# blyssprivacy/sdk

Hardware: AMD Instinct MI355X
Metric: PIR queries/sec (full answer path) on 2^20 items x 256 B (higher is better)
Workload: dtype u64; 1 GPU; spiral-rs process_query, c2 = {"db_item_size": 256, "instances": 1, "n": 2, "nu_1": 9, "nu_2": 11, "p": 256, "q2_bits": 20, "t_conv": 4, "t_exp_left": 8, "t_exp_right": 56, "t_gsw": 8}, encoded DB 64.0 GiB (56.0 GiB resident per GPU), unsharded, one query per step

## Files before the change

include/spiral_hip.h:

```cpp
#ifndef SPIRAL_HIP_H
#define SPIRAL_HIP_H

#include <stddef.h>
#include <stdint.h>

#ifdef __cplusplus
extern "C" {
#endif

#define SP_OK 0
#define SP_E_ARG (-1)
#define SP_E_HIP (-2)
#define SP_E_OOM (-3)
#define SP_E_STATE (-4)
#define SP_E_NOTFOUND (-5)

#define SP_MAX_ROW_SHARDS 8

typedef struct sp_params sp_params_t;
typedef struct sp_pp sp_pp_t;
typedef struct sp_ppc sp_ppc_t;
typedef struct sp_db sp_db_t;
typedef struct sp_query sp_query_t;

const char* sp_last_error(void);
uint64_t sp_paths_taken(int reset);
const char* sp_path_name(int bit);
int sp_debug_set(const char* name, long value);
int sp_device_count(void);
int sp_set_device(int device);

sp_params_t* sp_params_from_json(const char* json);
void sp_params_free(sp_params_t*);
uint64_t sp_params_get(const sp_params_t*, const char* name);
int sp_params_ntt_table(const sp_params_t*, int crt, int which, uint64_t* out_n);

sp_db_t* sp_db_create(const sp_params_t*, int shard, int num_shards);
sp_db_t* sp_db_create_columns(const sp_params_t*, int shard, int num_shards);
sp_db_t* sp_db_create_sparse(const sp_params_t*);
sp_db_t* sp_db_create_sparse_shard(const sp_params_t*, int shard, int num_shards);
size_t sp_db_sparse_items(const sp_db_t*);
sp_db_t* sp_db_create_planar(const sp_params_t*);
sp_db_t* sp_db_create_planar_shard(const sp_params_t*, int shard, int num_shards);
const char* sp_db_format(const sp_db_t*);
void sp_db_free(sp_db_t*);
int sp_db_load_plane(sp_db_t*, int plane, int z0, int nz, const uint64_t* words);
int sp_db_load(sp_db_t*, const uint64_t* words, size_t n_words);
int sp_db_load_items(sp_db_t*, const uint8_t* file, size_t file_len);
int sp_db_update_item(sp_db_t*, size_t item_idx, const uint8_t* data, size_t len);
int sp_db_update_items(sp_db_t*, const size_t* item_idx, const uint8_t* const* data, const size_t* lens, size_t n);
int sp_db_update_rows(sp_db_t*, const uint8_t* body, size_t body_len, size_t* applied, size_t* largest_update);
int sp_db_fill_synthetic(sp_db_t*, uint64_t seed);
int sp_db_prepare_batch(sp_db_t*, int* built);
uint64_t sp_synth_word(uint64_t seed, uint64_t ref_index);
int sp_db_read_ref(const sp_db_t*, int plane, int z, int ii, int j0, int count, uint64_t* out);
int sp_db_read_items(const sp_db_t*, size_t item0, size_t count, uint8_t* out, size_t out_cap,
                     uint8_t* present , size_t* undecodable );
size_t sp_db_export_rows_bound(const sp_db_t*, size_t count);
int sp_db_export_rows(const sp_db_t*, size_t item0, size_t count, uint8_t* body, size_t body_cap,
                      size_t* body_len, size_t* records);
int sp_db_copy_items(sp_db_t* dst, const sp_db_t* src, size_t item0, size_t count, size_t* copied );
#define SP_DIGEST_RESIDENT 0
#define SP_DIGEST_BATCH_COPY 1
int sp_db_digest(const sp_db_t*, uint64_t seed, int which, int plane0, int nplanes, uint64_t* out );
int sp_db_digest_ref_words(const sp_params_t*, uint64_t seed, int plane, int z0, int nz, const uint64_t* words, uint64_t acc[2]);
int sp_db_item_digests(const sp_db_t*, uint64_t seed, int which, int plane0, int nplanes, size_t item0, size_t count,
                       uint64_t* out , uint8_t* present );
int sp_db_item_digests_ref_words(const sp_params_t*, uint64_t seed, int plane, int z0, int nz, const uint64_t* words,
                                 uint64_t* acc );
size_t sp_db_device_bytes(const sp_db_t*);
size_t sp_db_batch_copy_bytes(const sp_db_t*);

sp_pp_t* sp_pp_deserialize(const sp_params_t*, const uint8_t* data, size_t len);
void sp_pp_free(sp_pp_t*);
int sp_pp_export(const sp_pp_t*, uint64_t* out, size_t cap_words, size_t* n_words);
size_t sp_pp_device_bytes(const sp_pp_t*);

sp_ppc_t* sp_pp_compact(const sp_params_t*, const uint8_t* data, size_t len);
void sp_ppc_free(sp_ppc_t*);
size_t sp_ppc_device_bytes(const sp_ppc_t*);
sp_pp_t* sp_pp_expand(const sp_ppc_t*);
int sp_pp_expand_into(const sp_ppc_t*, sp_pp_t* slot);

int sp_process_query(const sp_params_t*, const sp_pp_t*, const uint8_t* query, size_t query_len,
                     const sp_db_t*, uint8_t* out, size_t out_cap, size_t* out_len);
int sp_process_query_batch(const sp_params_t*, const sp_pp_t* const* pps, const uint8_t* const* queries,
                           const size_t* query_lens, int batch, const sp_db_t*, uint8_t* out,
                           size_t out_stride, size_t* out_len);

int sp_query_sweep_scatter(sp_query_t*, const sp_db_t*, int G);
int sp_query_sweep_scatter_plane(sp_query_t*, const sp_db_t*, int G, int plane);
int sp_query_sweep_scatter_group(sp_query_t* const* qs, int batch, const sp_db_t* shard, int G);
int sp_query_fold_local(sp_query_t*, const void* reduced_chunk_dev, int G);
int sp_query_fold_local_plane(sp_query_t*, const void* reduced_plane_chunk_dev, int G, int plane);
int sp_query_fold_local_join(sp_query_t*);
void* sp_query_stream2(sp_query_t*);
void* sp_query_local_cts_ptr(sp_query_t*);
size_t sp_query_local_cts_words(const sp_query_t*);
int sp_query_finish_gathered(sp_query_t*, const void* gathered_dev, int G, uint8_t* out, size_t out_cap, size_t* out_len);
sp_query_t* sp_query_begin(const sp_params_t*, const sp_pp_t*, const uint8_t* query, size_t query_len);
sp_query_t* sp_query_begin_for_db(const sp_params_t*, const sp_pp_t*, const uint8_t* query, size_t query_len,
                                  const sp_db_t* db);
int sp_query_sweep(sp_query_t*, const sp_db_t*);
void* sp_query_partial_ptr(sp_query_t*);
size_t sp_query_partial_words(const sp_query_t*);
int sp_query_sync(sp_query_t*);
int sp_query_finish(sp_query_t*, uint8_t* out, size_t out_cap, size_t* out_len);
void sp_query_free(sp_query_t*);
void* sp_query_stream(sp_query_t*);
int sp_query_timings(const sp_query_t*, float* ms4);

typedef struct sp_comm sp_comm_t;
#define SP_COMM_ID_BYTES 128
int sp_comm_unique_id(uint8_t* id128);
sp_comm_t* sp_comm_create(int rank, int world, const uint8_t* id128);
typedef struct sp_comm_ops {
  int (*reduce_scatter_u32)(void* user, const void* send, void* recv, size_t recv_count, void* hip_stream);
  int (*all_gather_u64)(void* user, const void* send, void* recv, size_t send_count, void* hip_stream);
  void* user;
} sp_comm_ops_t;
sp_comm_t* sp_comm_create_custom(int rank, int world, const sp_comm_ops_t* ops);
void sp_comm_free(sp_comm_t*);
int sp_comm_rank(const sp_comm_t*);
int sp_comm_world(const sp_comm_t*);
void* sp_comm_stream(sp_comm_t*);
int sp_comm_barrier(sp_comm_t*);
int sp_process_query_sharded(sp_comm_t*, const sp_params_t*, const sp_pp_t*, const uint8_t* query, size_t query_len,
                             const sp_db_t* shard, uint8_t* out, size_t out_cap, size_t* out_len);
int sp_process_queries_sharded(sp_comm_t*, const sp_params_t*, const sp_pp_t* const* pps, const uint8_t* const* queries,
                               const size_t* query_lens, int n, const sp_db_t* shard, uint8_t* out, size_t out_stride,
                               size_t* out_len);
int sp_process_queries_sharded_batched(sp_comm_t*, const sp_params_t*, const sp_pp_t* const* pps, const uint8_t* const* queries,
                                       const size_t* query_lens, int n, const sp_db_t* shard, int group, uint8_t* out,
                                       size_t out_stride, size_t* out_len);
int sp_comm_reserve_batch(sp_comm_t*, const sp_params_t* params, int group);
int sp_comm_reserve_batch_for(sp_comm_t*, const sp_params_t* params, const sp_db_t* shard, int group);
int sp_comm_reserve(sp_comm_t*, const sp_params_t* params);
int sp_comm_timings(const sp_comm_t*, float* ms3);
int sp_comm_describe(const sp_comm_t*, char* buf, size_t cap);

typedef struct sp_server sp_server_t;
sp_server_t* sp_server_create(const sp_params_t* params, const sp_db_t* db);
void sp_server_free(sp_server_t*);
size_t sp_server_clients(const sp_server_t*);
int sp_server_setup(sp_server_t*, const uint8_t* pp_bytes, size_t len, char* uuid_out37);
int sp_server_setup_json(sp_server_t*, const char* body, size_t body_len, char* out, size_t out_cap, size_t* out_len);
int sp_server_forget(sp_server_t*, const char* uuid);
int sp_server_private_read(sp_server_t*, const uint8_t* const* requests, const size_t* request_lens, int n, uint8_t* out,
                           size_t out_stride, size_t* out_lens);
int sp_server_private_read_json(sp_server_t*, const char* body, size_t body_len, char* out, size_t out_cap, size_t* out_len);
size_t sp_server_private_read_json_bound(const sp_server_t*, int n_queries);
int sp_server_update_row(sp_server_t*, sp_db_t* db, const uint8_t* body, size_t body_len, char* out, size_t out_cap, size_t* out_len);
int sp_server_replace_db(sp_server_t*, const sp_db_t* new_db);
int sp_server_set_expanded_clients(sp_server_t*, size_t max_expanded);
int sp_server_client_stats(const sp_server_t*, uint64_t out[7]);

int sp_sweep_launches(const sp_params_t*, const sp_db_t*);
int sp_bench_sweep(sp_query_t* q, const sp_db_t* db, int iters, float* ms_per_launch);
int sp_bench_sweep_ex(sp_query_t* q, const sp_db_t* db, int iters, int per_plane_launches, float* ms_per_launch);
int sp_bench_sweep_batch(sp_query_t* const* qs, int batch, const sp_db_t* db, int iters, float* ms_per_pass);
int sp_bench_sweep_scatter_group(sp_query_t* const* qs, int batch, const sp_db_t* shard, int G, int layout, int iters,
                                 float* ms_per_pass);

int sp_debug_cu_probe(int bit_lo, int bit_hi, int blocks, uint32_t* out2);
int sp_debug_resident_check(const sp_params_t* params, const sp_pp_t* pp, uint64_t* out, int cap);
int sp_debug_chacha20_u64(const uint8_t seed[32], uint64_t* out, size_t count);
int sp_debug_chacha20_u64_device(const sp_params_t*, const uint8_t seed[32], size_t first_word, uint64_t* out, size_t count);

int sp_bench_ntt(const sp_params_t*, int M, int blocks, int reps, float* ns_per_ntt);


int sp_ntt_forward(const sp_params_t*, uint64_t* data, size_t count);
int sp_ntt_inverse(const sp_params_t*, uint64_t* data, size_t count);
int sp_to_ntt(const sp_params_t*, const uint64_t* raw, uint64_t* out, size_t count);
int sp_from_ntt(const sp_params_t*, const uint64_t* ntt, uint64_t* out, size_t count);
int sp_multiply(const sp_params_t*, const uint64_t* a, size_t ar, size_t ac, const uint64_t* b, size_t bc,
                uint64_t* res);
int sp_add(const sp_params_t*, const uint64_t* a, const uint64_t* b, size_t count, uint64_t* res);
int sp_add_into(const sp_params_t*, uint64_t* res, const uint64_t* a, size_t count);
int sp_scalar_multiply(const sp_params_t*, const uint64_t* scalar, const uint64_t* b, size_t count, uint64_t* res);
int sp_automorph(const sp_params_t*, const uint64_t* a, size_t count, size_t t, uint64_t* res);
int sp_gadget_invert_rdim(const sp_params_t*, const uint64_t* inp, size_t rows_in, size_t cols, uint64_t* out,
                          size_t rows_out, size_t rdim);
int sp_reorient_reg_ciphertexts(const sp_params_t*, const uint64_t* v_reg, uint64_t* out);
int sp_multiply_reg_by_database(const sp_params_t*, const uint64_t* db, const uint64_t* v_firstdim, size_t dim0,
                                size_t num_per, uint64_t* out);
int sp_coefficient_expansion(const sp_params_t*, const sp_pp_t*, uint64_t* v, size_t g, size_t stop_round,
                             size_t max_bits_to_gen_right);
int sp_regev_to_gsw(const sp_params_t*, const sp_pp_t*, const uint64_t* v_inp, uint64_t* v_gsw, size_t num_gsw);
int sp_get_v_folding_neg(const sp_params_t*, const uint64_t* v_folding, uint64_t* out);
int sp_expand_query(const sp_params_t*, const sp_pp_t*, const uint8_t* query, size_t query_len,
                    uint64_t* v_reg_reoriented, uint64_t* v_folding);
int sp_fold_ciphertexts(const sp_params_t*, uint64_t* cts, size_t num_per, const uint64_t* v_folding,
                        const uint64_t* v_folding_neg);
int sp_fold_ciphertexts_fused(const sp_params_t*, uint64_t* cts, size_t num_per, const uint64_t* v_folding,
                              long fused_min_pairs);
int sp_pack(const sp_params_t*, const sp_pp_t*, const uint64_t* v_ct, uint64_t* out);
int sp_encode(const sp_params_t*, const uint64_t* v_packed, uint8_t* out, size_t out_cap, size_t* out_len);

#ifdef __cplusplus
}
#endif
#endif
```

rust/src/hip.rs:

```rust
#![allow(non_camel_case_types, clippy::missing_safety_doc, clippy::too_many_arguments)]

use std::ffi::{CStr, CString};
use std::os::raw::{c_char, c_int, c_long, c_void};

pub mod sys {
    use super::*;

    pub const SP_OK: c_int = 0;
    pub const SP_E_ARG: c_int = -1;
    pub const SP_E_HIP: c_int = -2;
    pub const SP_E_OOM: c_int = -3;
    pub const SP_E_STATE: c_int = -4;
    pub const SP_E_NOTFOUND: c_int = -5;
    pub const SP_MAX_ROW_SHARDS: c_int = 8;
    pub const SP_COMM_ID_BYTES: usize = 128;

    #[repr(C)]
    pub struct sp_params_t {
        _p: [u8; 0],
    }
    #[repr(C)]
    pub struct sp_pp_t {
        _p: [u8; 0],
    }
// ... 7 lines not shown
    }
    #[repr(C)]
    pub struct sp_query_t {
        _p: [u8; 0],
    }
    #[repr(C)]
    pub struct sp_comm_t {
        _p: [u8; 0],
    }
    #[repr(C)]
    pub struct sp_server_t {
        _p: [u8; 0],
    }
    #[repr(C)]
    pub struct sp_comm_ops_t {
        pub reduce_scatter_u32: Option<
            unsafe extern "C" fn(user: *mut c_void, send: *const c_void, recv: *mut c_void, recv_count: usize, hip_stream: *mut c_void) -> c_int,
        >,
        pub all_gather_u64: Option<
            unsafe extern "C" fn(user: *mut c_void, send: *const c_void, recv: *mut c_void, send_count: usize, hip_stream: *mut c_void) -> c_int,
        >,
        pub user: *mut c_void,
    }

    extern "C" {
        pub fn sp_last_error() -> *const c_char;
        pub fn sp_paths_taken(reset: c_int) -> u64;
        pub fn sp_path_name(bit: c_int) -> *const c_char;
        pub fn sp_debug_set(name: *const c_char, value: c_long) -> c_int;
        pub fn sp_device_count() -> c_int;
        pub fn sp_set_device(device: c_int) -> c_int;
        pub fn sp_params_from_json(json: *const c_char) -> *mut sp_params_t;
        pub fn sp_params_free(p: *mut sp_params_t);
        pub fn sp_params_get(p: *const sp_params_t, name: *const c_char) -> u64;
        pub fn sp_params_ntt_table(p: *const sp_params_t, crt: c_int, which: c_int, out_n: *mut u64) -> c_int;
        pub fn sp_db_create(p: *const sp_params_t, shard: c_int, num_shards: c_int) -> *mut sp_db_t;
        pub fn sp_db_create_columns(p: *const sp_params_t, shard: c_int, num_shards: c_int) -> *mut sp_db_t;
        pub fn sp_db_create_sparse(p: *const sp_params_t) -> *mut sp_db_t;
        pub fn sp_db_create_sparse_shard(p: *const sp_params_t, shard: c_int, num_shards: c_int) -> *mut sp_db_t;
        pub fn sp_db_create_planar(p: *const sp_params_t) -> *mut sp_db_t;
        pub fn sp_db_create_planar_shard(p: *const sp_params_t, shard: c_int, num_shards: c_int) -> *mut sp_db_t;
        pub fn sp_db_format(db: *const sp_db_t) -> *const c_char;
        pub fn sp_db_sparse_items(db: *const sp_db_t) -> usize;
        pub fn sp_db_free(db: *mut sp_db_t);
        pub fn sp_db_load_plane(db: *mut sp_db_t, plane: c_int, z0: c_int, nz: c_int, words: *const u64) -> c_int;
        pub fn sp_db_load(db: *mut sp_db_t, words: *const u64, n_words: usize) -> c_int;
        pub fn sp_db_load_items(db: *mut sp_db_t, file: *const u8, file_len: usize) -> c_int;
        pub fn sp_db_update_item(db: *mut sp_db_t, item_idx: usize, data: *const u8, len: usize) -> c_int;
        pub fn sp_db_update_items(db: *mut sp_db_t, item_idx: *const usize, data: *const *const u8, lens: *const usize, n: usize) -> c_int;
        pub fn sp_db_update_rows(db: *mut sp_db_t, body: *const u8, body_len: usize, applied: *mut usize, largest_update: *mut usize) -> c_int;
        pub fn sp_db_fill_synthetic(db: *mut sp_db_t, seed: u64) -> c_int;
        pub fn sp_db_prepare_batch(db: *mut sp_db_t, built: *mut c_int) -> c_int;
        pub fn sp_db_batch_copy_bytes(db: *const sp_db_t) -> usize;
        pub fn sp_synth_word(seed: u64, ref_index: u64) -> u64;
        pub fn sp_db_read_ref(db: *const sp_db_t, plane: c_int, z: c_int, ii: c_int, j0: c_int, count: c_int, out: *mut u64) -> c_int;
        pub fn sp_db_read_items(db: *const sp_db_t, item0: usize, count: usize, out: *mut u8, out_cap: usize, present: *mut u8, undecodable: *mut usize) -> c_int;
        pub fn sp_db_export_rows_bound(db: *const sp_db_t, count: usize) -> usize;
        pub fn sp_db_export_rows(db: *const sp_db_t, item0: usize, count: usize, body: *mut u8, body_cap: usize, body_len: *mut usize, records: *mut usize) -> c_int;
        pub fn sp_db_copy_items(dst: *mut sp_db_t, src: *const sp_db_t, item0: usize, count: usize, copied: *mut usize) -> c_int;
        pub fn sp_db_digest(db: *const sp_db_t, seed: u64, which: c_int, plane0: c_int, nplanes: c_int, out: *mut u64) -> c_int;
        pub fn sp_db_digest_ref_words(p: *const sp_params_t, seed: u64, plane: c_int, z0: c_int, nz: c_int, words: *const u64, acc: *mut u64) -> c_int;
        pub fn sp_db_item_digests(db: *const sp_db_t, seed: u64, which: c_int, plane0: c_int, nplanes: c_int, item0: usize, count: usize, out: *mut u64, present: *mut u8) -> c_int;
        pub fn sp_db_item_digests_ref_words(p: *const sp_params_t, seed: u64, plane: c_int, z0: c_int, nz: c_int, words: *const u64, acc: *mut u64) -> c_int;
        pub fn sp_db_device_bytes(db: *const sp_db_t) -> usize;
        pub fn sp_pp_deserialize(p: *const sp_params_t, data: *const u8, len: usize) -> *mut sp_pp_t;
        pub fn sp_pp_free(pp: *mut sp_pp_t);
        pub fn sp_pp_export(pp: *const sp_pp_t, out: *mut u64, cap_words: usize, n_words: *mut usize) -> c_int;
        pub fn sp_pp_device_bytes(pp: *const sp_pp_t) -> usize;
        pub fn sp_pp_compact(p: *const sp_params_t, data: *const u8, len: usize) -> *mut sp_ppc_t;
        pub fn sp_ppc_free(c: *mut sp_ppc_t);
        pub fn sp_ppc_device_bytes(c: *const sp_ppc_t) -> usize;
        pub fn sp_pp_expand(c: *const sp_ppc_t) -> *mut sp_pp_t;
        pub fn sp_pp_expand_into(c: *const sp_ppc_t, slot: *mut sp_pp_t) -> c_int;
        pub fn sp_process_query(p: *const sp_params_t, pp: *const sp_pp_t, query: *const u8, query_len: usize, db: *const sp_db_t,
                                out: *mut u8, out_cap: usize, out_len: *mut usize) -> c_int;
        pub fn sp_process_query_batch(p: *const sp_params_t, pps: *const *const sp_pp_t, queries: *const *const u8,
                                      query_lens: *const usize, batch: c_int, db: *const sp_db_t, out: *mut u8,
                                      out_stride: usize, out_len: *mut usize) -> c_int;
        pub fn sp_query_sweep_scatter(q: *mut sp_query_t, db: *const sp_db_t, g: c_int) -> c_int;
        pub fn sp_query_sweep_scatter_plane(q: *mut sp_query_t, db: *const sp_db_t, g: c_int, plane: c_int) -> c_int;
        pub fn sp_query_sweep_scatter_group(qs: *const *mut sp_query_t, batch: c_int, shard: *const sp_db_t, g: c_int) -> c_int;
        pub fn sp_query_fold_local(q: *mut sp_query_t, reduced_chunk_dev: *const c_void, g: c_int) -> c_int;
        pub fn sp_query_fold_local_plane(q: *mut sp_query_t, reduced_plane_chunk_dev: *const c_void, g: c_int, plane: c_int) -> c_int;
        pub fn sp_query_fold_local_join(q: *mut sp_query_t) -> c_int;
        pub fn sp_query_stream2(q: *mut sp_query_t) -> *mut c_void;
        pub fn sp_query_local_cts_ptr(q: *mut sp_query_t) -> *mut c_void;
        pub fn sp_query_local_cts_words(q: *const sp_query_t) -> usize;
        pub fn sp_query_finish_gathered(q: *mut sp_query_t, gathered_dev: *const c_void, g: c_int, out: *mut u8, out_cap: usize,
                                        out_len: *mut usize) -> c_int;
        pub fn sp_query_begin(p: *const sp_params_t, pp: *const sp_pp_t, query: *const u8, query_len: usize) -> *mut sp_query_t;
        pub fn sp_query_begin_for_db(p: *const sp_params_t, pp: *const sp_pp_t, query: *const u8, query_len: usize,
                                     db: *const sp_db_t) -> *mut sp_query_t;
        pub fn sp_query_sweep(q: *mut sp_query_t, db: *const sp_db_t) -> c_int;
        pub fn sp_query_partial_ptr(q: *mut sp_query_t) -> *mut c_void;
        pub fn sp_query_partial_words(q: *const sp_query_t) -> usize;
        pub fn sp_query_sync(q: *mut sp_query_t) -> c_int;
        pub fn sp_query_finish(q: *mut sp_query_t, out: *mut u8, out_cap: usize, out_len: *mut usize) -> c_int;
        pub fn sp_query_free(q: *mut sp_query_t);
        pub fn sp_query_stream(q: *mut sp_query_t) -> *mut c_void;
        pub fn sp_query_timings(q: *const sp_query_t, ms4: *mut f32) -> c_int;
        pub fn sp_comm_unique_id(id128: *mut u8) -> c_int;
        pub fn sp_comm_create(rank: c_int, world: c_int, id128: *const u8) -> *mut sp_comm_t;
        pub fn sp_comm_create_custom(rank: c_int, world: c_int, ops: *const sp_comm_ops_t) -> *mut sp_comm_t;
        pub fn sp_comm_free(c: *mut sp_comm_t);
        pub fn sp_comm_rank(c: *const sp_comm_t) -> c_int;
        pub fn sp_comm_world(c: *const sp_comm_t) -> c_int;
        pub fn sp_comm_stream(c: *mut sp_comm_t) -> *mut c_void;
        pub fn sp_comm_barrier(c: *mut sp_comm_t) -> c_int;
        pub fn sp_process_query_sharded(c: *mut sp_comm_t, p: *const sp_params_t, pp: *const sp_pp_t, query: *const u8,
                                        query_len: usize, shard: *const sp_db_t, out: *mut u8, out_cap: usize,
                                        out_len: *mut usize) -> c_int;
        pub fn sp_process_queries_sharded(c: *mut sp_comm_t, p: *const sp_params_t, pps: *const *const sp_pp_t, queries: *const *const u8,
                                          query_lens: *const usize, n: c_int, shard: *const sp_db_t, out: *mut u8, out_stride: usize,
                                          out_len: *mut usize) -> c_int;
        pub fn sp_comm_reserve(c: *mut sp_comm_t, p: *const sp_params_t) -> c_int;
        pub fn sp_comm_reserve_batch(c: *mut sp_comm_t, p: *const sp_params_t, group: c_int) -> c_int;
        pub fn sp_comm_reserve_batch_for(c: *mut sp_comm_t, p: *const sp_params_t, shard: *const sp_db_t, group: c_int) -> c_int;
        pub fn sp_process_queries_sharded_batched(c: *mut sp_comm_t, p: *const sp_params_t, pps: *const *const sp_pp_t,
                                                  queries: *const *const u8, query_lens: *const usize, n: c_int,
                                                  shard: *const sp_db_t, group: c_int, out: *mut u8, out_stride: usize,
                                                  out_len: *mut usize) -> c_int;
        pub fn sp_comm_timings(c: *const sp_comm_t, ms3: *mut f32) -> c_int;
        pub fn sp_comm_describe(c: *const sp_comm_t, buf: *mut c_char, cap: usize) -> c_int;
        pub fn sp_server_create(params: *const sp_params_t, db: *const sp_db_t) -> *mut sp_server_t;
        pub fn sp_server_free(s: *mut sp_server_t);
        pub fn sp_server_clients(s: *const sp_server_t) -> usize;
        pub fn sp_server_setup(s: *mut sp_server_t, pp_bytes: *const u8, len: usize, uuid_out37: *mut c_char) -> c_int;
        pub fn sp_server_setup_json(s: *mut sp_server_t, body: *const c_char, body_len: usize, out: *mut c_char, out_cap: usize,
                                    out_len: *mut usize) -> c_int;
        pub fn sp_server_forget(s: *mut sp_server_t, uuid: *const c_char) -> c_int;
        pub fn sp_server_set_expanded_clients(s: *mut sp_server_t, max_expanded: usize) -> c_int;
        pub fn sp_server_client_stats(s: *const sp_server_t, out7: *mut u64) -> c_int;
        pub fn sp_server_private_read(s: *mut sp_server_t, requests: *const *const u8, request_lens: *const usize, n: c_int,
                                      out: *mut u8, out_stride: usize, out_lens: *mut usize) -> c_int;
        pub fn sp_server_private_read_json(s: *mut sp_server_t, body: *const c_char, body_len: usize, out: *mut c_char,
                                           out_cap: usize, out_len: *mut usize) -> c_int;
        pub fn sp_server_private_read_json_bound(s: *const sp_server_t, n_queries: c_int) -> usize;
        pub fn sp_server_update_row(s: *mut sp_server_t, db: *mut sp_db_t, body: *const u8, body_len: usize, out: *mut c_char,
                                    out_cap: usize, out_len: *mut usize) -> c_int;
        pub fn sp_server_replace_db(s: *mut sp_server_t, new_db: *const sp_db_t) -> c_int;
        pub fn sp_sweep_launches(p: *const sp_params_t, db: *const sp_db_t) -> c_int;
        pub fn sp_bench_sweep(q: *mut sp_query_t, db: *const sp_db_t, iters: c_int, ms_per_launch: *mut f32) -> c_int;
        pub fn sp_bench_sweep_ex(q: *mut sp_query_t, db: *const sp_db_t, iters: c_int, per_plane_launches: c_int,
                                 ms_per_launch: *mut f32) -> c_int;
        pub fn sp_bench_sweep_batch(qs: *const *mut sp_query_t, batch: c_int, db: *const sp_db_t, iters: c_int,
                                    ms_per_pass: *mut f32) -> c_int;
        pub fn sp_bench_sweep_scatter_group(qs: *const *mut sp_query_t, batch: c_int, shard: *const sp_db_t, g: c_int,
                                            layout: c_int, iters: c_int, ms_per_pass: *mut f32) -> c_int;
        pub fn sp_debug_cu_probe(bit_lo: c_int, bit_hi: c_int, blocks: c_int, out2: *mut u32) -> c_int;
        pub fn sp_debug_resident_check(params: *const sp_params_t, pp: *const sp_pp_t, out: *mut u64, cap: c_int) -> c_int;
        pub fn sp_debug_chacha20_u64(seed: *const u8, out: *mut u64, count: usize) -> c_int;
        pub fn sp_debug_chacha20_u64_device(p: *const sp_params_t, seed: *const u8, first_word: usize, out: *mut u64,
                                            count: usize) -> c_int;
        pub fn sp_bench_ntt(p: *const sp_params_t, m: c_int, blocks: c_int, reps: c_int, ns_per_ntt: *mut f32) -> c_int;
        pub fn sp_ntt_forward(p: *const sp_params_t, data: *mut u64, count: usize) -> c_int;
        pub fn sp_ntt_inverse(p: *const sp_params_t, data: *mut u64, count: usize) -> c_int;
        pub fn sp_to_ntt(p: *const sp_params_t, raw: *const u64, out: *mut u64, count: usize) -> c_int;
        pub fn sp_from_ntt(p: *const sp_params_t, ntt: *const u64, out: *mut u64, count: usize) -> c_int;
        pub fn sp_multiply(p: *const sp_params_t, a: *const u64, ar: usize, ac: usize, b: *const u64, bc: usize, res: *mut u64) -> c_int;
        pub fn sp_add(p: *const sp_params_t, a: *const u64, b: *const u64, count: usize, res: *mut u64) -> c_int;
        pub fn sp_add_into(p: *const sp_params_t, res: *mut u64, a: *const u64, count: usize) -> c_int;
        pub fn sp_scalar_multiply(p: *const sp_params_t, scalar: *const u64, b: *const u64, count: usize, res: *mut u64) -> c_int;
        pub fn sp_automorph(p: *const sp_params_t, a: *const u64, count: usize, t: usize, res: *mut u64) -> c_int;
        pub fn sp_gadget_invert_rdim(p: *const sp_params_t, inp: *const u64, rows_in: usize, cols: usize, out: *mut u64,
                                     rows_out: usize, rdim: usize) -> c_int;
        pub fn sp_reorient_reg_ciphertexts(p: *const sp_params_t, v_reg: *const u64, out: *mut u64) -> c_int;
        pub fn sp_multiply_reg_by_database(p: *const sp_params_t, db: *const u64, v_firstdim: *const u64, dim0: usize,
                                           num_per: usize, out: *mut u64) -> c_int;
        pub fn sp_coefficient_expansion(p: *const sp_params_t, pp: *const sp_pp_t, v: *mut u64, g: usize, stop_round: usize,
                                        max_bits_to_gen_right: usize) -> c_int;
        pub fn sp_regev_to_gsw(p: *const sp_params_t, pp: *const sp_pp_t, v_inp: *const u64, v_gsw: *mut u64, num_gsw: usize) -> c_int;
        pub fn sp_get_v_folding_neg(p: *const sp_params_t, v_folding: *const u64, out: *mut u64) -> c_int;
        pub fn sp_expand_query(p: *const sp_params_t, pp: *const sp_pp_t, query: *const u8, query_len: usize,
                               v_reg_reoriented: *mut u64, v_folding: *mut u64) -> c_int;
        pub fn sp_fold_ciphertexts(p: *const sp_params_t, cts: *mut u64, num_per: usize, v_folding: *const u64,
                                   v_folding_neg: *const u64) -> c_int;
        pub fn sp_fold_ciphertexts_fused(p: *const sp_params_t, cts: *mut u64, num_per: usize, v_folding: *const u64,
                                         fused_min_pairs: c_long) -> c_int;
        pub fn sp_pack(p: *const sp_params_t, pp: *const sp_pp_t, v_ct: *const u64, out: *mut u64) -> c_int;
        pub fn sp_encode(p: *const sp_params_t, v_packed: *const u64, out: *mut u8, out_cap: usize, out_len: *mut usize) -> c_int;
    }
}

#[derive(Debug, Clone)]
pub struct HipError {
    pub code: c_int,
    pub message: String,
}
impl std::fmt::Display for HipError {
    fn fmt(&self, f: &mut std::fmt::Formatter<'_>) -> std::fmt::Result {
        write!(f, "spiral_hip rc={}: {}", self.code, self.message)
    }
}
impl std::error::Error for HipError {}

fn last_error() -> String {
    unsafe { CStr::from_ptr(sys::sp_last_error()) }.to_string_lossy().into_owned()
}
fn check(rc: c_int) -> Result<(), HipError> {
    if rc == sys::SP_OK {
        Ok(())
    } else {
        Err(HipError { code: rc, message: last_error() })
    }
}
fn must<T>(r: Result<T, HipError>) -> T {
    r.unwrap_or_else(|e| panic!("{}", e))
}

const N: usize = 2048;
const CRT: usize = 2;

pub struct Params(*mut sys::sp_params_t);
pub struct PublicParameters(*mut sys::sp_pp_t);
pub struct CompactPublicParameters(*mut sys::sp_ppc_t);
unsafe impl Send for CompactPublicParameters {}
unsafe impl Sync for CompactPublicParameters {}
pub struct Database(*mut sys::sp_db_t);
pub struct Comm(*mut sys::sp_comm_t);
unsafe impl Send for Params {}
unsafe impl Sync for Params {}
unsafe impl Send for PublicParameters {}
unsafe impl Sync for PublicParameters {}
unsafe impl Send for Database {}
unsafe impl Sync for Database {}
unsafe impl Send for Comm {}

impl Params {
    pub fn try_from_json(cfg: &str) -> Result<Self, HipError> {
        let c = CString::new(cfg).map_err(|_| HipError { code: sys::SP_E_ARG, message: "NUL in JSON".into() })?;
        let p = unsafe { sys::sp_params_from_json(c.as_ptr()) };
        if p.is_null() {
            Err(HipError { code: sys::SP_E_ARG, message: last_error() })
        } else {
            Ok(Params(p))
        }
    }
    pub fn from_json(cfg: &str) -> Self {
        must(Self::try_from_json(cfg))
    }
    pub fn get(&self, name: &str) -> u64 {
        let c = CString::new(name).unwrap();
        let v = unsafe { sys::sp_params_get(self.0, c.as_ptr()) };
        assert!(v != u64::MAX, "unknown Params field {}", name);
        v
    }
    pub fn setup_bytes(&self) -> usize { self.get("setup_bytes") as usize }
    pub fn query_bytes(&self) -> usize { self.get("query_bytes") as usize }
    pub fn num_items(&self) -> usize { self.get("num_items") as usize }
    pub fn response_bytes(&self) -> usize { self.get("response_bytes") as usize }
    pub fn db_words(&self) -> usize { self.get("db_words") as usize }
    pub fn dim0(&self) -> usize { 1usize << self.get("db_dim_1") }
    pub fn num_per(&self) -> usize { 1usize << self.get("db_dim_2") }
    pub fn planes(&self) -> usize { (self.get("instances") * self.get("n") * self.get("n")) as usize }
    pub fn t_gsw(&self) -> usize { self.get("t_gsw") as usize }
    pub fn n(&self) -> usize { self.get("n") as usize }
    pub fn as_ptr(&self) -> *const sys::sp_params_t { self.0 }
}
impl Drop for Params {
    fn drop(&mut self) {
        unsafe { sys::sp_params_free(self.0) }
    }
}

impl PublicParameters {
    pub fn try_deserialize(params: &Params, data: &[u8]) -> Result<Self, HipError> {
        let h = unsafe { sys::sp_pp_deserialize(params.0, data.as_ptr(), data.len()) };
        if h.is_null() {
            Err(HipError { code: sys::SP_E_ARG, message: last_error() })
        } else {
            Ok(PublicParameters(h))
        }
    }
    pub fn deserialize(params: &Params, data: &[u8]) -> Self {
        must(Self::try_deserialize(params, data))
    }
}
impl Drop for PublicParameters {
    fn drop(&mut self) {
        unsafe { sys::sp_pp_free(self.0) }
    }
}
impl PublicParameters {
    pub fn device_bytes(&self) -> usize {
        unsafe { sys::sp_pp_device_bytes(self.0) }
    }
}

impl CompactPublicParameters {
    pub fn try_new(params: &Params, data: &[u8]) -> Result<Self, HipError> {
        let h = unsafe { sys::sp_pp_compact(params.0, data.as_ptr(), data.len()) };
        if h.is_null() {
            Err(HipError { code: sys::SP_E_ARG, message: last_error() })
        } else {
            Ok(CompactPublicParameters(h))
        }
    }
    pub fn device_bytes(&self) -> usize {
        unsafe { sys::sp_ppc_device_bytes(self.0) }
    }
    pub fn expand(&self) -> Result<PublicParameters, HipError> {
        let h = unsafe { sys::sp_pp_expand(self.0) };
        if h.is_null() {
            Err(HipError { code: sys::SP_E_ARG, message: last_error() })
        } else {
            Ok(PublicParameters(h))
// ... 348 lines not shown
```

sdk_amd/csrc/capi.cpp:

```cpp
#include <cstdlib>
#include <new>

#include "capi_internal.hpp"

using namespace spiral;

static thread_local std::string g_last_error;
static thread_local int g_last_rc = SP_OK;
static thread_local int g_shard_split_hint = 1;
int spiral::guarded_status(int rc, const char* what) {
  if (rc != SP_OK) g_last_error = what;
  g_last_rc = rc;
  return rc;
}
int spiral::null_handle_rc() { return g_last_rc != SP_OK ? g_last_rc : SP_E_ARG; }

void spiral::check_device(int dev) {
  int cur = 0;
  HIP_CHECK(hipGetDevice(&cur));
  if (cur != dev) throw ArgError("handle belongs to HIP device " + std::to_string(dev) + " but the current device is " + std::to_string(cur));
}

void spiral::download_ntt(Workspace& W, const u32* src, size_t words, uint64_t* host, DevBuf<u64>& tmp) {
  tmp.ensure(words);
// ... 1259 lines not shown
    need_shard_count(q->params->p, G, db);
    need_row_shard(db);
    need_begun_for(q, db);
    check_device(db->device);
    Workspace& W = *q->ws;
    if (db->sparse) {
      sweep_sparse_scatter(q, db, G, 0, (int)q->params->p.planes(), false);
    } else if (db->planar_resident) {
      sp_query_t* one[1] = {q};
      planar_shard_pass(one, 1, db, G, 0, (int)q->params->p.planes(), true);
    } else {
      ScatterLayout scatter(W, G);
      run_sweep(W, *db);
    }
    HIP_CHECK(hipEventRecord(W.ev[2], W.stream));
    q->state = 2;
  });
}

int sp_query_sweep_scatter_plane(sp_query_t* q, const sp_db_t* db, int G, int plane) {
  return guarded([&] {
    need(q && db, "null argument");
    refuse_planar_unsharded(db, "sp_query_sweep_scatter_plane");
    need(db->params == q->params, "db was created for different params");
    need_rows_of(q, db);
    const Params& p = q->params->p;
    need_shard_count(p, G, db);
    need_row_shard(db);
    need_begun_for(q, db);
    need(plane >= 0 && (size_t)plane < p.planes(), "plane out of range");
    need(q->state == 1 && q->next_plane == plane, "sp_query_sweep_scatter_plane: planes must be swept in order after begin");
    check_device(db->device);
    Workspace& W = *q->ws;
    W.ensure_sweep();
    if (db->sparse) {
      sweep_sparse_scatter(q, db, G, plane, 1, true);
    } else if (db->planar_resident) {
      sp_query_t* one[1] = {q};
      planar_shard_pass(one, 1, db, G, plane, 1, false);
    } else {
      ScatterLayout scatter(W, G);
      launch_plane_sweep(W, *db, (size_t)plane);
    }
    q->next_plane = plane + 1;
    if ((size_t)q->next_plane == p.planes()) {
      HIP_CHECK(hipEventRecord(W.ev[2], W.stream));
      q->state = 2;
    }
  });
}

int sp_query_sweep_scatter_group(sp_query_t* const* qs, int batch, const sp_db_t* db, int G) {
  return guarded([&] {
    scatter_group_check(qs, batch, db, G);
    for (int i = 0; i < batch; i++)
      need(qs[i]->state == 1 && qs[i]->next_plane == 0, "sp_query_sweep_scatter_group: every query must be in 'begun' state, no plane swept");
    const size_t planes = db->params->p.planes();
    SweepBatchDesc d{};
    if (db->sparse) {
      const int group_min = sparse_group_min();
      bool shared = batch >= 2 && group_min != 0 && batch >= group_min;
      for (int i = 1; i < batch; i++) shared = shared && qs[i]->sparse_index == qs[0]->sparse_index;
      for (int i = 0; i < batch; i++) qs[i]->ws->ensure_sweep();
      if (shared) {
        Workspace* Ws[SPARSE_GROUP_MAX];
        for (int i = 0; i < batch; i++) Ws[i] = qs[i]->ws.get();
        const sp_db::SparseIndex& idx = *qs[0]->sparse_index;
        Workspace& W0 = group_pass_stream(qs, batch);
        run_sweep_sparse_scatter_group(Ws, batch, *db, idx.col_ptr.p, idx.col_rows.p, idx.col_slots.p, G, W0.stream);
        for (int i = 0; i < batch; i++) {
          group_pass_done(qs, i);
          qs[i]->ws->zero_shortcuts = true;
        }
      } else {
        for (int i = 0; i < batch; i++) {
          sweep_sparse_scatter(qs[i], db, G, 0, (int)planes, true);
          HIP_CHECK(hipEventRecord(qs[i]->ws->ev[2], qs[i]->ws->stream));
        }
      }
    } else if (db->planar_resident) {
      planar_shard_pass(qs, batch, db, G, 0, (int)planes, false);
      for (int i = 0; i < batch; i++) group_pass_done(qs, i);
    } else if (scatter_group_desc(qs, batch, db, G, d)) {
      Workspace& W0 = group_pass_stream(qs, batch);
      sweep_batch_prepare(W0.D->T, d, W0.stream);
      launch_sweep_batch_scatter(W0.D->T, d, G, W0.stream);
      for (int i = 0; i < batch; i++) group_pass_done(qs, i);
    } else {
      for (int i = 0; i < batch; i++) {
        Workspace& W = *qs[i]->ws;
        ScatterLayout scatter(W, G);
        for (size_t pl = 0; pl < planes; pl++) launch_plane_sweep(W, *db, pl);
        HIP_CHECK(hipEventRecord(W.ev[2], W.stream));
      }
    }
    for (int i = 0; i < batch; i++) {
      qs[i]->next_plane = (int)planes;
      qs[i]->state = 2;
    }
  });
}

int sp_query_fold_local(sp_query_t* q, const void* reduced_chunk, int G) {
  return guarded([&] {
    need(q && reduced_chunk, "null argument");
    need(q->state == 2, "sp_query_fold_local: sweep has not run");
    need_shard_count(q->params->p, G);
    run_fold_local(*q->ws, (const u32*)reduced_chunk, G);
    q->state = 4;
  });
}
int sp_query_fold_local_plane(sp_query_t* q, const void* reduced_plane_chunk, int G, int plane) {
  return guarded([&] {
    need(q && reduced_plane_chunk, "null argument");
    const Params& p = q->params->p;
    need_shard_count(p, G);
    need(plane >= 0 && (size_t)plane < p.planes(), "plane out of range");
    need((q->state == 1 && plane < q->next_plane) || q->state == 2, "sp_query_fold_local_plane: plane has not been swept");
    need(plane == q->next_fold_plane, "sp_query_fold_local_plane: planes must be folded in order");
    run_fold_local_plane(*q->ws, (const u32*)reduced_plane_chunk, G, plane);
    q->next_fold_plane = plane + 1;
  });
}

int sp_query_fold_local_join(sp_query_t* q) {
  return guarded([&] {
    need(q, "null argument");
    need(q->state == 2 && (size_t)q->next_fold_plane == q->params->p.planes(),
         "sp_query_fold_local_join: every plane must have been swept and folded");
    run_fold_local_join(*q->ws);
    q->state = 4;
  });
}

void* sp_query_stream2(sp_query_t* q) { return q && q->ws ? (void*)q->ws->stream2 : nullptr; }

void* sp_query_local_cts_ptr(sp_query_t* q) { return q && q->ws ? (void*)q->ws->final_cts.p : nullptr; }
size_t sp_query_local_cts_words(const sp_query_t* q) { return q ? q->params->p.planes() * 2 * POLY_LEN : 0; }

int sp_query_finish_gathered(sp_query_t* q, const void* gathered, int G, uint8_t* out, size_t out_cap, size_t* out_len) {
  return guarded([&] {
    need(q && gathered && out && out_len, "null argument");
    need(q->state == 4, "sp_query_finish_gathered: local fold has not run");
    const Params& p = q->params->p;
    need(out_cap >= p.response_bytes(), "output buffer smaller than response_bytes");
    run_finish_gathered(*q->ws, *q->pp, (const u64*)gathered, G);
    collect_response(q, out, out_len);
    q->state = 3;
  });
}

void* sp_query_partial_ptr(sp_query_t* q) {
  if (!q || !q->ws) return nullptr;
  if (guarded([&] { q->ws->ensure_sweep(); }) != SP_OK) return nullptr;
  return (void*)q->ws->sweep_out.p;
}
size_t sp_query_partial_words(const sp_query_t* q) {
  if (!q) return 0;
  const Params& p = q->params->p;
  return p.planes() * 4 * POLY_LEN * p.num_per();
}
void* sp_query_stream(sp_query_t* q) { return q && q->ws ? (void*)q->ws->stream : nullptr; }

int sp_query_sync(sp_query_t* q) {
  return guarded([&] {
    need(q && q->ws, "null query");
    HIP_CHECK(hipStreamSynchronize(q->ws->stream));
    HIP_CHECK(hipStreamSynchronize(q->ws->stream2));
  });
}

int sp_query_finish(sp_query_t* q, uint8_t* out, size_t out_cap, size_t* out_len) {
  return guarded([&] { finish_impl(q, true, out, out_cap, out_len); });
}

int sp_query_timings(const sp_query_t* q, float* ms4) {
  if (!q || !ms4 || q->state != 3) {
    g_last_error = "timings are available after sp_query_finish";
    return SP_E_STATE;
  }
  memcpy(ms4, q->ms, sizeof(q->ms));
  return SP_OK;
}
void sp_query_free(sp_query_t* q) { delete q; }

int sp_process_query(const sp_params_t* h, const sp_pp_t* pp, const uint8_t* query, size_t query_len,
                     const sp_db_t* db, uint8_t* out, size_t out_cap, size_t* out_len) {
  if (db && (db->num_shards != 1 || db->col_G != 1)) {
    g_last_error = "sp_process_query needs an unsharded db; use sp_query_begin/sweep/finish for shards";
    return SP_E_ARG;
  }
  sp_query_t* q = sp_query_begin_for_db(h, pp, query, query_len, db);
  if (!q) return null_handle_rc();
  int rc = sp_query_sweep(q, db);
  if (rc == SP_OK) rc = guarded([&] { finish_impl(q, false, out, out_cap, out_len); });
  sp_query_free(q);
  return rc;
}

}

#include "capi_readback.hpp"
#include "capi_copy.hpp"
#include "capi_digest.hpp"
#include "capi_item_digest.hpp"
#include "capi_compact.hpp"

#ifndef SPIRAL_CAPI_SPLIT
#include "capi_batch.cpp"
#include "capi_stage.cpp"
#endif
```

sdk_amd/csrc/capi_internal.hpp:

```cpp
#pragma once
#include <cstring>
#include <memory>
#include <string>

#include "../../include/spiral_hip.h"
#include "pipeline.hpp"

struct sp_query {
  sp_params* params = nullptr;
  const sp_pp* pp = nullptr;
  std::unique_ptr<spiral::Workspace> ws;
  int state = 0;
  int next_plane = 0;
  int next_fold_plane = 0;
  int rows_j0 = 0, rows_nj = 0;
  const sp_db* for_sparse = nullptr;
  std::shared_ptr<const sp_db::SparseIndex> sparse_index;
  std::shared_ptr<const spiral::DevBuf<spiral::u64>> planar;
  float ms[4] = {0, 0, 0, 0};
  bool streams_idle = false;
  ~sp_query() {
    if (ws && params) {
      if (!streams_idle) {
        (void)hipStreamSynchronize(ws->stream);
        (void)hipStreamSynchronize(ws->stream2);
      }
      ws->pipelined = false;
      ws->have_sweep_span = false;
      ws->zero_shortcuts = false;
      ws->out_G = 1;
      params->release_ws(std::move(ws));
    }
  }
};

extern "C" void sp_set_last_error_(const char* msg);

namespace spiral {

int guarded_status(int rc, const char* what);
int null_handle_rc();

template <typename F>
int guarded(F&& f) {
  tunables_new_call();
  try {
    f();
    return guarded_status(SP_OK, nullptr);
  } catch (const ArgError& e) {
    return guarded_status(SP_E_ARG, e.what());
  } catch (const OomError& e) {
    return guarded_status(SP_E_OOM, e.what());
  } catch (const HipError& e) {
    return guarded_status(SP_E_HIP, e.what());
  } catch (const std::bad_alloc&) {
    return guarded_status(SP_E_OOM, "host allocation failed");
  } catch (const std::exception& e) {
    return guarded_status(SP_E_ARG, e.what());
  }
}
template <typename F>
auto guarded_handle(F&& make) -> decltype(make().release()) {
  decltype(make()) h;
  return guarded([&] { h = make(); }) == SP_OK ? h.release() : nullptr;
}

inline void need(bool c, const char* msg) {
  if (!c) throw ArgError(msg);
}
void check_device(int dev);

struct Scoped {
  sp_params* P;
  std::unique_ptr<Workspace> ws;
  explicit Scoped(const sp_params* p) : P(const_cast<sp_params*>(p)), ws(P->acquire_ws()) {}
  ~Scoped() {
    (void)hipStreamSynchronize(ws->stream);
    P->release_ws(std::move(ws));
  }
  Workspace& operator*() { return *ws; }
  Workspace* operator->() { return ws.get(); }
};
void download_ntt(Workspace& W, const u32* src, size_t words, uint64_t* host, DevBuf<u64>& tmp);

struct TimingEvents {
  hipEvent_t a = nullptr, b = nullptr;
  TimingEvents() {
    HIP_CHECK(hipEventCreate(&a));
    if (hipEventCreate(&b) != hipSuccess) {
      (void)hipEventDestroy(a);
      throw HipError("hipEventCreate failed");
    }
  }
  ~TimingEvents() {
    (void)hipEventDestroy(a);
    (void)hipEventDestroy(b);
  }
  TimingEvents(const TimingEvents&) = delete;
  TimingEvents& operator=(const TimingEvents&) = delete;
};
template <typename F>
float timed_reps(hipStream_t s, int iters, F&& once, float launches_per_rep = 1.0f) {
  struct Drain {
    hipStream_t s;
    ~Drain() { (void)hipStreamSynchronize(s); }
  } drain{s};
  TimingEvents ev;
  once();
  HIP_CHECK(hipEventRecord(ev.a, s));
  for (int i = 0; i < iters; i++) once();
  HIP_CHECK(hipEventRecord(ev.b, s));
  HIP_CHECK(hipStreamSynchronize(s));
  float t = 0;
  HIP_CHECK(hipEventElapsedTime(&t, ev.a, ev.b));
  return t / ((float)iters * launches_per_rep);
}

sp_query_t* query_open(const sp_params_t* h, const sp_pp_t* pp);
sp_query_t* query_open_sparse(const sp_params_t* h, const sp_pp_t* pp, const sp_db_t* db, std::shared_ptr<const sp_db::SparseIndex> snapshot);
void query_begin_opened(sp_query_t* q, const uint8_t* query, size_t query_len, const sp_db_t* db);
void finish_impl(sp_query_t* q, bool premod, uint8_t* out, size_t out_cap, size_t* out_len);

size_t group_ws_bytes(const Params& p, int np_local);

using PlanarPin = std::shared_ptr<const DevBuf<u64>>;
SweepBatchDesc group_pass(const sp_db& db, sp_query_t* const* qs, int B, bool use_planar, PlanarPin& pin);
void group_pass_launch(const sp_db& db, const DevTables& T, SweepBatchDesc& d, hipStream_t s);
void refuse_planar_resident(const sp_db_t* db, const char* what);
Workspace& group_pass_stream(sp_query_t* const* qs, int B);
void group_pass_done(sp_query_t* const* qs, int i);

void sparse_group_pass(const sp_db& db, sp_query_t* const* qs, int B, hipStream_t s);

void scatter_group_check(sp_query_t* const* qs, int batch, const sp_db_t* db, int G);
bool scatter_group_desc(sp_query_t* const* qs, int batch, const sp_db_t* db, int G, SweepBatchDesc& d);

}
```

sdk_amd/csrc/capi_stage.cpp:

```cpp
#include "capi_internal.hpp"

using namespace spiral;

namespace {

void upload_ntt(Workspace& W, const uint64_t* host, size_t words, DevBuf<u32>& dst, DevBuf<u64>& tmp) {
  tmp.ensure(words);
  dst.ensure(words);
  HIP_CHECK(hipMemcpyAsync(tmp.p, host, words * 8, hipMemcpyHostToDevice, W.stream));
  launch_u64_to_u32(dst.p, tmp.p, (long)words, W.stream);
}
void upload_raw(Workspace& W, const uint64_t* host, size_t words, DevBuf<u64>& dst) {
  dst.ensure(words);
  HIP_CHECK(hipMemcpyAsync(dst.p, host, words * 8, hipMemcpyHostToDevice, W.stream));
}
void download_raw(Workspace& W, const u64* src, size_t words, uint64_t* host) {
  HIP_CHECK(hipMemcpyAsync(host, src, words * 8, hipMemcpyDeviceToHost, W.stream));
  HIP_CHECK(hipStreamSynchronize(W.stream));
}

void ensure_stage_fold(Workspace& W, size_t num_per, size_t further) {
  const size_t two_t = 2 * W.P->t_gsw;
  W.ensure_expand();
  W.foldX.ensure(num_per * 2 * POLY_LEN);
  W.foldY.ensure(std::max<size_t>(num_per / 2, 1) * 2 * POLY_LEN);
  W.fold_dig.ensure(num_per * two_t * 2 * POLY_LEN);
  W.fold_ntt.ensure(std::max<size_t>(num_per / 2, 1) * 2 * 2 * POLY_LEN);
  W.fold_mats.ensure(further * 2 * 2 * two_t * 2 * POLY_LEN);
}

enum MatsCopy { TO_MATS, FROM_MATS };
void copy_mats_half(Workspace& W, MatsCopy dir, int half, size_t levels, u32* dense) {
  const size_t row = 2 * W.P->t_gsw * 2 * POLY_LEN;
  for (size_t k = 0; k < levels * 2; k++) {
    u32 *m = W.fold_mats.p + (k * 2 + half) * row, *d = dense + k * row;
    HIP_CHECK(hipMemcpyAsync(dir == TO_MATS ? m : d, dir == TO_MATS ? d : m, row * sizeof(u32), hipMemcpyDeviceToDevice, W.stream));
  }
}
size_t mats_half_words(const Params& p, size_t levels) { return levels * 2 * 2 * p.t_gsw * 2 * POLY_LEN; }

template <typename F>
void stage_fold(const sp_params_t* h, uint64_t* cts, size_t num_per, const uint64_t* v_folding, F&& prepare) {
  need(num_per >= 1 && (num_per & (num_per - 1)) == 0, "num_per must be a power of two");
  size_t further = 0;
  while (((size_t)1 << further) < num_per) further++;
  if (further == 0) return;
  Scoped W(h);
  ensure_stage_fold(*W, num_per, further);
  DevBuf<u64> tmp, tmp2;
  DevBuf<u32> dF, left;
  upload_ntt(*W, v_folding, mats_half_words(h->p, further), dF, tmp);
  copy_mats_half(*W, TO_MATS, 1, further, dF.p);
  const FoldOpts o = prepare(*W, further, left, tmp2);
  HIP_CHECK(hipMemcpyAsync(W->foldX.p, cts, num_per * 2 * POLY_LEN * 8, hipMemcpyHostToDevice, W->stream));
  u64* res = run_fold(*W, o, W->foldX.p, W->foldY.p, 1, (int)num_per, -1);
  download_raw(*W, res, 2 * POLY_LEN, cts);
}

}

extern "C" {

int sp_bench_sweep(sp_query_t* q, const sp_db_t* db, int iters, float* ms_per_launch) {
  return sp_bench_sweep_ex(q, db, iters, -1, ms_per_launch);
}

int sp_bench_sweep_ex(sp_query_t* q, const sp_db_t* db, int iters, int per_plane_launches, float* ms_per_launch) {
  return guarded([&] {
    need(q && db && ms_per_launch && iters > 0, "bad argument");
    refuse_planar_resident(db, "sp_bench_sweep");
    need(q->state >= 1, "query not begun");
    check_device(db->device);
    Workspace& W = *q->ws;
    const Params& p = q->params->p;
    const bool per_plane = per_plane_launches < 0 ? sweep_is_pipelined(p, *db) : per_plane_launches != 0;
    need(!per_plane || db->col_G == 1, "per-plane launches need a row-sharded or unsharded db");
    auto sweep_once = [&] {
      if (!per_plane) return run_sweep(W, *db);
      W.ensure_sweep();
      for (size_t pl = 0; pl < p.planes(); pl++) launch_plane_sweep(W, *db, pl);
    };
    *ms_per_launch = timed_reps(W.stream, iters, sweep_once, per_plane ? (float)p.planes() : 1.0f);
  });
}

int sp_bench_sweep_batch(sp_query_t* const* qs, int batch, const sp_db_t* db, int iters, float* ms_per_pass) {
  return guarded([&] {
    if (qs && db && db->sparse) {
      need(ms_per_pass && iters > 0 && batch >= 1 && batch <= SPARSE_GROUP_MAX, "bad argument");
      check_device(db->device);
      for (int i = 0; i < batch; i++) {
        need(qs[i] && qs[i]->state >= 1, "query not begun");
        need(qs[i]->params == db->params, "query and db were created for different params");
        qs[i]->ws->ensure_sweep();
        HIP_CHECK(hipStreamSynchronize(qs[i]->ws->stream));
        HIP_CHECK(hipStreamSynchronize(qs[i]->ws->stream2));
      }
      hipStream_t s = qs[0]->ws->stream;
      *ms_per_pass = timed_reps(s, iters, [&] { sparse_group_pass(*db, qs, batch, s); });
      return;
    }
    const int group_max = !db ? 0 : db->planar_resident ? planar_resident_group_max(db->nj) : sweep_batch_group_max(db->np_local, db->nj);
    need(qs && db && ms_per_pass && iters > 0 && batch >= 1 && batch <= group_max, "bad argument");
    const bool narrow = !db->packed && db->num_shards == 1 && db->col_G == 1 && batch >= 2 && sweep_narrow_batch_shape_ok(db->np_local, db->nj);
    need(narrow || (db->planar_resident && db->num_shards == 1) || (db->packed && db->num_shards == 1 && db->col_G == 1),
         "the batched pass needs an unsharded PACKED database");
    check_device(db->device);
    for (int i = 0; i < batch; i++) {
      need(qs[i] && qs[i]->state >= 1, "query not begun");
      need(qs[i]->params == db->params, "query and db were created for different params");
    }
    Workspace& W0 = *qs[0]->ws;
    for (int i = 0; i < batch; i++) {
      qs[i]->ws->ensure_sweep();
      HIP_CHECK(hipStreamSynchronize(qs[i]->ws->stream));
      HIP_CHECK(hipStreamSynchronize(qs[i]->ws->stream2));
    }
    PlanarPin pin;
    SweepBatchDesc d = group_pass(*db, qs, batch, true, pin);
    *ms_per_pass = timed_reps(W0.stream, iters, [&] { group_pass_launch(*db, W0.D->T, d, W0.stream); });
  });
}

int sp_bench_sweep_scatter_group(sp_query_t* const* qs, int batch, const sp_db_t* db, int G, int layout, int iters, float* ms_per_pass) {
  return guarded([&] {
    need(ms_per_pass && iters > 0 && (layout == 0 || layout == 1), "bad argument");
    scatter_group_check(qs, batch, db, G);
    for (int i = 0; i < batch; i++) {
      need(qs[i]->state >= 1, "query not begun");
      HIP_CHECK(hipStreamSynchronize(qs[i]->ws->stream));
      HIP_CHECK(hipStreamSynchronize(qs[i]->ws->stream2));
    }
    if (db->sparse) {
      Workspace* Ws[SPARSE_GROUP_MAX];
      for (int i = 0; i < batch; i++) {
        need(qs[i]->sparse_index == qs[0]->sparse_index, "the queries of a sparse bucket's group must have been begun on one snapshot of its index");
        qs[i]->ws->ensure_sweep();
        Ws[i] = qs[i]->ws.get();
      }
      const sp_db::SparseIndex& idx = *qs[0]->sparse_index;
      Workspace& W0 = *qs[0]->ws;
      const int planes = (int)db->params->p.planes();
      *ms_per_pass = timed_reps(W0.stream, iters, [&] {
        if (batch == 1 && layout == 1)
          run_sweep_sparse_scatter(W0, *db, idx.col_ptr.p, idx.col_rows.p, idx.col_slots.p, G, 0, planes, true);
        else if (batch == 1)
          run_sweep_sparse(W0, *db, idx.col_ptr.p, idx.col_rows.p, idx.col_slots.p);
        else if (layout == 1)
          run_sweep_sparse_scatter_group(Ws, batch, *db, idx.col_ptr.p, idx.col_rows.p, idx.col_slots.p, G, W0.stream);
        else
          run_sweep_sparse_group(Ws, batch, *db, idx.col_ptr.p, idx.col_rows.p, idx.col_slots.p, W0.stream);
      });
      return;
    }
    if (db->planar_resident) {
      need(layout == 1, "a planar row shard has the scatter-form pass only (layout 1)");
      for (int i = 0; i < batch; i++) qs[i]->ws->ensure_sweep();
      PlanarPin none;
      SweepBatchDesc pd = group_pass(*db, qs, batch, false, none);
      Workspace& Wp = *qs[0]->ws;
      const int planes = (int)db->params->p.planes();
      *ms_per_pass = timed_reps(Wp.stream, iters, [&] {
        sweep_planar_resident_prepare(Wp.D->T, pd, Wp.stream);
        launch_sweep_planar_scatter(Wp.D->T, pd, G, 0, planes, false, Wp.stream);
      });
      return;
    }
    SweepBatchDesc d{};
    need(scatter_group_desc(qs, batch, db, G, d), "this group / shard does not take the scatter-form pass (sp_query_sweep_scatter_group would sweep per query)");
    Workspace& W0 = *qs[0]->ws;
    *ms_per_pass = timed_reps(W0.stream, iters, [&] {
      sweep_batch_prepare(W0.D->T, d, W0.stream);
      if (layout == 1)
        launch_sweep_batch_scatter(W0.D->T, d, G, W0.stream);
      else
        launch_sweep_batch(W0.D->T, d, W0.stream);
    });
  });
}

int sp_sweep_launches(const sp_params_t* h, const sp_db_t* db) {
  if (!h || !db) return 0;
  return sweep_is_pipelined(h->p, *db) ? (int)h->p.planes() : 1;
}

int sp_debug_cu_probe(int bit_lo, int bit_hi, int blocks, uint32_t* out2) {
  return guarded([&] {
    need(out2 && blocks > 0 && blocks <= 65536, "bad argument");
    hipStream_t s = nullptr;
    if (bit_hi > bit_lo) {
      hipDeviceProp_t prop;
      int dev = 0;
      HIP_CHECK(hipGetDevice(&dev));
      HIP_CHECK(hipGetDeviceProperties(&prop, dev));
      std::vector<uint32_t> m((prop.multiProcessorCount + 31) / 32, 0u);
      for (int k = bit_lo; k < bit_hi && k < prop.multiProcessorCount; k++) m[k / 32] |= 1u << (k % 32);
      HIP_CHECK(hipExtStreamCreateWithCUMask(&s, (uint32_t)m.size(), m.data()));
    } else {
      HIP_CHECK(hipStreamCreateWithFlags(&s, hipStreamNonBlocking));
    }
    DevBuf<u32> d((size_t)blocks * 2);
    launch_cu_probe(d.p, blocks, s);
    HIP_CHECK(hipMemcpyAsync(out2, d.p, (size_t)blocks * 8, hipMemcpyDeviceToHost, s));
    HIP_CHECK(hipStreamSynchronize(s));
    (void)hipStreamDestroy(s);
  });
}

int sp_debug_chacha20_u64(const uint8_t seed[32], uint64_t* out, size_t count) {
  if (!seed || (!out && count)) {
    sp_set_last_error_("null argument");
    return SP_E_ARG;
  }
  chacha20_keystream_u64(seed, out, count);
  return SP_OK;
}

int sp_debug_resident_check(const sp_params_t* h, const sp_pp_t* pp, uint64_t* out, int cap) {
  return guarded([&] {
    need(h && pp && out && cap >= 24, "bad argument");
    DeviceState& D = const_cast<sp_params*>(h)->device_state();
    struct Item { const u32* p; size_t n; const u32* host; };
    const Item items[6] = {{D.tw.p, D.tw.n, h->p.ntt_tables.data()}, {D.neg1.p, D.neg1.n, nullptr},
                           {D.gadget_gsw.p, D.gadget_gsw.n, nullptr}, {(const u32*)D.lists.p, D.lists.n, nullptr},
                           {pp->all.p, pp->all.n, nullptr}, {pp->pack_cat.p, pp->pack_cat.n, nullptr}};
    hipStream_t s = nullptr;
    HIP_CHECK(hipStreamCreateWithFlags(&s, hipStreamNonBlocking));
    DevBuf<unsigned long long> acc(12);
    DevBuf<u32> sink(1);
    auto host_sum = [](const u32* p, size_t n) {
      unsigned long long a = 0;
      for (size_t i = 0; i < n; i++) a += (unsigned long long)p[i] * (unsigned long long)((i << 1) | 1);
      return a;
    };
    HIP_CHECK(hipMemsetAsync(acc.p, 0, 12 * 8, s));
    for (int i = 0; i < 6; i++) launch_checksum(items[i].p, items[i].n, acc.p + i, s);
    launch_cache_sync(sink.p, s);
    for (int i = 0; i < 6; i++) launch_checksum(items[i].p, items[i].n, acc.p + 6 + i, s);
    unsigned long long k[12];
    HIP_CHECK(hipMemcpyAsync(k, acc.p, sizeof(k), hipMemcpyDeviceToHost, s));
    HIP_CHECK(hipStreamSynchronize(s));
    for (int i = 0; i < 6; i++) {
      std::vector<u32> hostcopy(items[i].n);
      if (items[i].n) HIP_CHECK(hipMemcpy(hostcopy.data(), items[i].p, items[i].n * 4, hipMemcpyDeviceToHost));
      out[4 * i + 0] = k[i];
      out[4 * i + 1] = host_sum(hostcopy.data(), items[i].n);
      out[4 * i + 2] = k[6 + i];
      out[4 * i + 3] = items[i].host ? host_sum(items[i].host, items[i].n) : 0;
    }
    (void)hipStreamDestroy(s);
  });
}

int sp_bench_ntt(const sp_params_t* h, int M, int blocks, int reps, float* ns_per_ntt) {
  return guarded([&] {
    need(h && ns_per_ntt && blocks > 0 && reps > 0, "bad argument");
    Scoped W(h);
    DevBuf<u32> scratch((size_t)blocks * 256);
    const float ms = bench_ntt_core(W->D->T, M, blocks, reps, scratch.p, W->stream);
    *ns_per_ntt = ms * 1e6f / ((float)blocks * reps * (M == 1 || M == 2 ? M : 4));
  });
}

int sp_to_ntt(const sp_params_t* h, const uint64_t* raw, uint64_t* out, size_t count) {
  return guarded([&] {
    need(h && raw && out, "null argument");
    if (count == 0) return;
    Scoped W(h);
    DevBuf<u64> d_raw, tmp;
    DevBuf<u32> d_ntt(count * 2 * POLY_LEN);
    upload_raw(*W, raw, count * POLY_LEN, d_raw);
    FwdDesc f{d_raw.p, nullptr, d_ntt.p, (int)count, 1, 1, 1, 64, 1, 0, 1};
    launch_ntt_fwd(W->D->T, f, W->stream);
    download_ntt(*W, d_ntt.p, count * 2 * POLY_LEN, out, tmp);
  });
}

int sp_from_ntt(const sp_params_t* h, const uint64_t* ntt, uint64_t* out, size_t count) {
  return guarded([&] {
    need(h && ntt && out, "null argument");
    if (count == 0) return;
    Scoped W(h);
    DevBuf<u64> tmp, d_raw(count * POLY_LEN);
    DevBuf<u32> d_ntt;
    upload_ntt(*W, ntt, count * 2 * POLY_LEN, d_ntt, tmp);
    InvDesc inv{};
    inv.src = d_ntt.p;
    inv.poly_stride = 2 * POLY_LEN;
    inv.crt_stride = POLY_LEN;
    inv.z_stride = 1;
    inv.dst = d_raw.p;
    inv.n_polys = (int)count;
    launch_ntt_inv(W->D->T, inv, W->stream);
    download_raw(*W, d_raw.p, count * POLY_LEN, out);
  });
}

int sp_ntt_forward(const sp_params_t* h, uint64_t* data, size_t count) {
  return guarded([&] {
    need(h && data, "null argument");
    if (count == 0) return;
    std::vector<u64> full(count * 2 * 2 * POLY_LEN);
    int rc = sp_to_ntt(h, data, full.data(), count * 2);
    if (rc != SP_OK) throw HipError(sp_last_error());
    for (size_t i = 0; i < count; i++)
      for (size_t c = 0; c < 2; c++)
        memcpy(data + (i * 2 + c) * POLY_LEN, full.data() + ((i * 2 + c) * 2 + c) * POLY_LEN, POLY_LEN * 8);
  });
}

int sp_ntt_inverse(const sp_params_t* h, uint64_t* data, size_t count) {
  return guarded([&] {
    need(h && data, "null argument");
    if (count == 0) return;
    std::vector<u64> raw(count * POLY_LEN);
    int rc = sp_from_ntt(h, data, raw.data(), count);
    if (rc != SP_OK) throw HipError(sp_last_error());
    for (size_t i = 0; i < count; i++)
      for (size_t z = 0; z < POLY_LEN; z++) {
        data[(i * 2 + 0) * POLY_LEN + z] = raw[i * POLY_LEN + z] % h->p.moduli[0];
        data[(i * 2 + 1) * POLY_LEN + z] = raw[i * POLY_LEN + z] % h->p.moduli[1];
      }
  });
}

int sp_multiply(const sp_params_t* h, const uint64_t* a, size_t ar, size_t ac, const uint64_t* b, size_t bc,
                uint64_t* res) {
  return guarded([&] {
    need(h && a && b && res && ar && ac && bc, "bad argument");
    Scoped W(h);
    DevBuf<u64> tmp;
    DevBuf<u32> dA, dBt, dR(ar * bc * 2 * POLY_LEN);
    upload_ntt(*W, a, ar * ac * 2 * POLY_LEN, dA, tmp);
    std::vector<u64> bt(ac * bc * 2 * POLY_LEN);
    for (size_t k = 0; k < ac; k++)
      for (size_t j = 0; j < bc; j++)
        memcpy(bt.data() + (j * ac + k) * 2 * POLY_LEN, b + (k * bc + j) * 2 * POLY_LEN, 2 * POLY_LEN * 8);
    DevBuf<u64> tmp2;
    upload_ntt(*W, bt.data(), bt.size(), dBt, tmp2);
    MacDesc m{};
    m.A = dA.p;
    m.B = dBt.p;
    m.out = dR.p;
    m.R = (int)ar;
    m.K = (int)ac;
    m.batch_inner = (int)bc;
    m.batch_outer = 1;
    m.B_inner_stride = (long)ac;
    m.split_k = (int)ac;
    m.out_batch_stride = 1;
    m.out_row_stride = (int)bc;
    launch_mac(W->D->T, m, W->stream);
    download_ntt(*W, dR.p, ar * bc * 2 * POLY_LEN, res, tmp);
  });
}

int sp_add(const sp_params_t* h, const uint64_t* a, const uint64_t* b, size_t count, uint64_t* res) {
  return guarded([&] {
    need(h && a && b && res && count, "bad argument");
    Scoped W(h);
    DevBuf<u64> tmp, tmp2;
    DevBuf<u32> dA, dB, dR(count * 2 * POLY_LEN);
    upload_ntt(*W, a, count * 2 * POLY_LEN, dA, tmp);
    upload_ntt(*W, b, count * 2 * POLY_LEN, dB, tmp2);
    launch_add(W->D->T, dR.p, dA.p, dB.p, (int)count, W->stream);
    download_ntt(*W, dR.p, count * 2 * POLY_LEN, res, tmp);
  });
}
// ... 223 lines not shown
```

sdk_amd/csrc/db.hip:

```cpp
#include "device_common.hpp"

namespace spiral {

__global__ __launch_bounds__(256) void k_db_relayout(u64* dst_plane, const u64* src, int z0, int num_per, int dim0,
                                                     int j0, int nj, ColMap cm) {
  __shared__ u64 tile[32][33];
  const int zl = blockIdx.z;
  const int tx = threadIdx.x & 31, ty = threadIdx.x >> 5;
  const int jt = blockIdx.x * 32, it = blockIdx.y * 32;
  const u64* s = src + (size_t)zl * cm.np_global * dim0;
  u64* dpl = dst_plane + (size_t)(z0 + zl) * nj * num_per;
#pragma unroll
  for (int i = 0; i < 4; i++) {
    int ii = it + ty + 8 * i, j = jt + tx;
    if (ii < num_per && j < nj) tile[ty + 8 * i][tx] = canon_word(s[(size_t)(cm.off + cm.stride * ii) * dim0 + j0 + j]);
  }
  __syncthreads();
#pragma unroll
  for (int i = 0; i < 4; i++) {
    int j = jt + ty + 8 * i, ii = it + tx;
    if (ii < num_per && j < nj) dpl[(size_t)j * num_per + ii] = tile[tx][ty + 8 * i];
  }
}
__global__ __launch_bounds__(256) void k_db_relayout_packed(u32* dst, int plane, const u64* src, int z0, int nz,
// ... 184 lines not shown
  for (int k = 0; k < 8; k++) {
    const int z = 8 * tau + k;
    if (d.packed) {
      const int chunks = d.num_per >> 7, npairs = d.nj >> 1;
      u32* unit = reinterpret_cast<u32*>(d.db) +
                  packed_unit_offset((size_t)plane * N + z, jp, ii0 >> 7, npairs, chunks);
      pack_unit_lane(unit, (ii0 & 127) >> 1, w[0][k], w[1][k], w[2][k], w[3][k]);
    } else {
#pragma unroll
      for (int ab = 0; ab < 4; ab++) {
        const int jl = jl0 + (ab >> 1), ii = ii0 + (ab & 1);
        if (jl < d.nj && ii < d.num_per) d.db[(((size_t)plane * N + z) * d.nj + jl) * d.num_per + ii] = w[ab][k];
      }
    }
  }
}
void launch_db_encode(const DevTables& T, const DbEncodeDesc& d, hipStream_t s) {
  if (d.njp <= 0) return;
  const unsigned gx = d.only_item >= 0 ? 1u : (unsigned)((d.num_per + 1) / 2);
  hipLaunchKernelGGL(k_db_encode, dim3(gx * (unsigned)d.njp, 1, d.planes), dim3(256), 0, s, T, d);
  launched(0, "k_db_encode");
}

__device__ __forceinline__ u32 quad_item_coeff(const DbEncodeDesc& d, const uint8_t* bytes, int len, int chunk_idx, int z) {
  const int pos = chunk_idx * d.bytes_per_chunk;
  if (pos >= d.db_item_size) return 0u;
  const int avail = d.db_item_size - pos;
  const int bytes_read = avail < d.bytes_per_chunk ? avail : d.bytes_per_chunk;
  const int words_read = (bytes_read * 8 + d.logp - 1) / d.logp;
  if (z >= words_read) return 0u;
  const int bit = z * d.logp;
  const int b0 = bit >> 3, sh = bit & 7;
  u64 acc = 0;
  const int nb = (sh + d.logp + 7) >> 3;
  for (int i = 0; i < nb; i++) {
    const int bi = b0 + i;
    const u64 byte = (bi < bytes_read && pos + bi < len) ? (u64)bytes[pos + bi] : 0ULL;
    acc |= byte << (8 * i);
  }
  return (u32)((acc >> sh) & ((1ULL << d.logp) - 1ULL));
}
__global__ __launch_bounds__(256) void k_db_encode_quads(DevTables T, DbEncodeDesc d, const DbQuadRec* quads) {
  __shared__ u32 lds0[LDS_WORDS];
  __shared__ u32 lds1[LDS_WORDS];
  const int tau = threadIdx.x;
  const int plane = (int)(blockIdx.x % (unsigned)d.planes);
  const DbQuadRec* qr = quads + blockIdx.x / (unsigned)d.planes;
  const int jp = qr->jp, qd = qr->q;
  const int chunks = d.num_per >> 7, npairs = d.nj >> 1;
  u64 w[4][8];
#pragma unroll
  for (int t = 0; t < 4; t++)
#pragma unroll
    for (int k = 0; k < 8; k++) w[t][k] = 0;
  u32* la = lds0;
  u32* lb = lds1;
#pragma unroll 1
  for (int ab = 0; ab < 4; ab++) {
    const int a = ab >> 1, b = ab & 1;
    const int jl = 2 * jp + a, ii = 2 * qd + b;
    const bool valid = jl < d.nj && ii < d.num_per;
    const long long src = qr->src[ab];
    u64 cur[8];
    if (src < 0 || !valid) {
#pragma unroll
      for (int k = 0; k < 8; k++) {
        cur[k] = 0;
        if (valid && d.packed) {
          const u32* unit = reinterpret_cast<const u32*>(d.db) + packed_unit_offset((size_t)plane * N + 8 * tau + k, jp, ii >> 7, npairs, chunks);
          cur[k] = unpack_word(unit, (ii & 127) >> 1, ab);
        }
      }
    } else {
      const uint8_t* bytes = d.win + src;
      const int len = qr->len[ab];
      u32 lo[8];
#pragma unroll 1
      for (int c = 0; c < 2; c++) {
        const ModConst m = T.c.mod[c];
        u32 v[8];
#pragma unroll
        for (int k = 0; k < 8; k++) {
          const u32 x = quad_item_coeff(d, bytes, len, plane, tau + 256 * k);
          v[k] = x > d.pt_modulus / 2 ? m.q - (d.pt_modulus - x) : x;
        }
        const u32* fw = T.tw + (size_t)c * 4 * N;
        ntt_fwd_block(v, tau, la, lb, fw, fw + N, m.q, m.two_q);
        {
          u32* tmp = la;
          la = lb;
          lb = tmp;
        }
#pragma unroll
        for (int k = 0; k < 8; k++) {
          if (c == 0)
            lo[k] = v[k];
          else
            cur[k] = (u64)lo[k] | ((u64)v[k] << 32);
        }
      }
    }
#pragma unroll
    for (int t = 0; t < 4; t++)
#pragma unroll
      for (int k = 0; k < 8; k++) w[t][k] = t == ab ? cur[k] : w[t][k];
  }
  const int jl0 = 2 * jp, ii0 = 2 * qd;
#pragma unroll
  for (int k = 0; k < 8; k++) {
    const int z = 8 * tau + k;
    if (d.packed) {
      u32* unit = reinterpret_cast<u32*>(d.db) + packed_unit_offset((size_t)plane * N + z, jp, ii0 >> 7, npairs, chunks);
      pack_unit_lane(unit, (ii0 & 127) >> 1, w[0][k], w[1][k], w[2][k], w[3][k]);
    } else {
#pragma unroll
      for (int ab = 0; ab < 4; ab++) {
        const int jl = jl0 + (ab >> 1), ii = ii0 + (ab & 1);
        if (qr->src[ab] >= 0 && jl < d.nj && ii < d.num_per) d.db[(((size_t)plane * N + z) * d.nj + jl) * d.num_per + ii] = w[ab][k];
      }
    }
  }
}
void launch_db_encode_quads(const DevTables& T, const DbEncodeDesc& d, const DbQuadRec* quads, size_t n_quads, hipStream_t s) {
  if (n_quads == 0) return;
  hipLaunchKernelGGL(k_db_encode_quads, dim3((unsigned)(n_quads * (size_t)d.planes)), dim3(256), 0, s, T, d, quads);
  launched(0, "k_db_encode_quads");
}

__global__ __launch_bounds__(256) void k_canon_words(u64* w, size_t total) {
  const size_t i = (size_t)blockIdx.x * 256 + threadIdx.x;
  if (i < total) w[i] = canon_word(w[i]);
}
void launch_canon_words(u64* w, size_t total, hipStream_t s) {
  if (total == 0) return;
  hipLaunchKernelGGL(k_canon_words, dim3((unsigned)((total + 255) / 256)), dim3(256), 0, s, w, total);
  launched(0, "k_canon_words");
}

__global__ __launch_bounds__(256) void k_sweep_out_to_ref(u64* out, const u32* in, int num_per) {
  size_t i = (size_t)blockIdx.x * 256 + threadIdx.x;
  size_t total = (size_t)4 * N * num_per;
  if (i >= total) return;
  size_t z = i & (N - 1);
  size_t rc = (i >> POLY_LEN_LOG2) & 3;
  size_t ii = i >> (POLY_LEN_LOG2 + 2);
  out[i] = (u64)in[(rc * N + z) * num_per + ii];
}
void launch_sweep_out_to_ref(u64* out, const u32* in, int num_per, hipStream_t s) {
  size_t total = (size_t)4 * N * num_per;
  hipLaunchKernelGGL(k_sweep_out_to_ref, dim3((unsigned)((total + 255) / 256)), dim3(256), 0, s, out, in, num_per);
  launched(0, "k_sweep_out_to_ref");
}

}

#include "item_readback.hpp"
#include "db_digest.hpp"
#include "db_item_digest.hpp"
#include "db_copy.hpp"
```

sdk_amd/csrc/kernels.hpp:

```cpp
#pragma once
#include <hip/hip_runtime.h>

#include <vector>

#include "params.hpp"

namespace spiral {

constexpr int N = (int)POLY_LEN;

struct DevTables {
  const u32* tw;
  DevConsts c;
};
__host__ __device__ inline const u32* inv_tables(const u32* tw, int c) { return tw + (size_t)8 * N + (size_t)c * 2 * N; }
__host__ __device__ inline const u32* wave_fwd_image(const u32* tw, int c) { return tw + (size_t)12 * N + (size_t)c * 2 * N; }
__host__ __device__ inline int wtw_phys(int idx) {
  if (idx >= 1024) {
    const int L = (idx - 1024) >> 4, r = (idx - 1024) & 15;
    return 1024 + 16 * L + 4 * (((r >> 2) + (L >> 2)) & 3) + (r & 3);
  }
  if (idx >= 512) {
    const int L = (idx - 512) >> 3, r = (idx - 512) & 7;
    return 512 + 8 * L + 4 * (((r >> 2) + (L >> 3)) & 1) + (r & 3);
  }
  return idx;
}

enum PathBit : u64 {
  PATH_SWEEP_PERSIST = 1ull << 0,
  PATH_SWEEP_PACKED = 1ull << 1,
  PATH_SWEEP_WIDE = 1ull << 2,
  PATH_SWEEP_NARROW = 1ull << 3,
  PATH_SWEEP_BATCH = 1ull << 4,
  PATH_FROM_SWEEP4 = 1ull << 5,
  PATH_FROM_SWEEP1 = 1ull << 6,
  PATH_FOLD_FUSED = 1ull << 7,
  PATH_FOLD_TAIL = 1ull << 8,
  PATH_FOLD_TAIL_LITERAL = 1ull << 9,
  PATH_PIPELINED = 1ull << 10,
  PATH_EXPAND_PRUNED = 1ull << 11,
  PATH_PACK_V1 = 1ull << 12,
  PATH_DIRECT_UPLOAD = 1ull << 13,
  PATH_SCATTER_OUT = 1ull << 14,
  PATH_SWEEP_XCD_FROM = 1ull << 15,
  PATH_FOLD_TAIL_PERSIST = 1ull << 16,
  PATH_EXPAND_FUSED = 1ull << 17,
  PATH_SWEEP_SPARSE = 1ull << 18,
  PATH_RCCL = 1ull << 19,
  PATH_FOLD_WAVE = 1ull << 20,
  PATH_CU_SPLIT = 1ull << 21,
  PATH_EXPAND_SPLIT = 1ull << 22,
  PATH_PIPE_CLASS_SPLIT = 1ull << 23,
  PATH_SWEEP_MFMA = 1ull << 24,
  PATH_CUSTOM_TRANSPORT = 1ull << 25,
  PATH_FROM_SWEEP_WAVE = 1ull << 26,
  PATH_FOLD_TAIL_BATCHED = 1ull << 27,
  PATH_SWEEP_RING = 1ull << 28,
  PATH_SWEEP_MFMA2 = 1ull << 29,
  PATH_FOLD_WAVE8 = 1ull << 30,
  PATH_SWEEP_PLANAR = 1ull << 31,
  PATH_EXPAND_GROUP = 1ull << 32,
  PATH_EXPAND_WAVE = 1ull << 33,
  PATH_SWEEP_BATCH_SCATTER = 1ull << 34,
  PATH_SWEEP_SPARSE_GROUP = 1ull << 35,
  PATH_SWEEP_NARROW_GROUP = 1ull << 36
};
long tunable(const char* name, long dflt);
void launched(u64 path_bits, const char* kernel);
void note_path(u64 path_bits);
void launch_checksum(const u32* p, size_t n_words, unsigned long long* out, hipStream_t s);
void launch_cache_sync(u32* sink, hipStream_t s);
void launch_copy_words(u32* dst, const u32* src, size_t n_words, hipStream_t s);
void debug_stage(int stage);

struct FwdDesc {
  const u64* src;
  const int* src_idx;
  u32* dst;
  int n_out;
  int rdim, cols, t, bits;
  int src_batch_stride;
  int src_row0, src_cols;
  long delta_off;
  int delta_inner, delta_outer_stride;
};
void launch_ntt_fwd(const DevTables& T, const FwdDesc& d, hipStream_t s);
void launch_ntt_fwd3(const DevTables& T, const FwdDesc& d0, const FwdDesc& d1, const FwdDesc& d2, hipStream_t s);

float bench_ntt_core(const DevTables& T, int M, int blocks, int reps, u32* scratch, hipStream_t s);

struct InvDesc {
  const u32* src;
  const int* idx;
  int polys_per_idx;
  long idx_stride, poly_stride, crt_stride, z_stride;
  u64* dst;
  int n_polys;
  int premod;
  int sweep_np;
  int automorph_t;
  const u32* scal;
  u32* scal_dst;
  int scal_thresh;
  const int* scal_only_idx;
  int n_scalar_only;
  const u64* addend;
  int add_inner2, add_outer_stride;
};
void launch_ntt_inv(const DevTables& T, const InvDesc& d, hipStream_t s);
void launch_from_sweep4(const DevTables& T, const u32* src, int np, int n_planes, int premod, u64* dst, hipStream_t s);

struct MacDesc {
  const u32* A;
  const u32* B;
  u32* out;
  const u32* addend;
  const int* out_idx;
  int R, K;
  int A_row_stride;
  int batch_inner, batch_outer;
  long B_inner_stride, B_outer_stride;
  int split_k;
  long split_off;
  int out_batch_stride, out_row_stride;
  const u32* extra;
  const int* extra_idx;
  int extra_row;
};
void launch_mac(const DevTables& T, const MacDesc& d, hipStream_t s);
void launch_mac2(const DevTables& T, const MacDesc& d0, const MacDesc& d1, hipStream_t s);

struct ExpandSideDesc {
  const u64* raw;
  const int* pos;
  const int* out_idx;
  const u32* A;
  u32* v;
  int cnt, t, bits;
};
void launch_expand_round(const DevTables& T, const ExpandSideDesc& left, const ExpandSideDesc& right, hipStream_t s);
constexpr long EXPAND_ROUND_MIN_DEFAULT = 2048;

constexpr int GROUP_MAX = 16;
struct GroupOff {
  long long v[GROUP_MAX], raw[GROUP_MAX], dig[GROUP_MAX], ct1[GROUP_MAX], pp[GROUP_MAX];
};
void launch_ntt_inv_group(const DevTables& T, const InvDesc& d, const GroupOff& g, int B, hipStream_t s);
void launch_ntt_fwd3_group(const DevTables& T, const FwdDesc& d0, const FwdDesc& d1, const FwdDesc& d2, const GroupOff& g, int B,
                           hipStream_t s);
void launch_mac2_group(const DevTables& T, const MacDesc& d0, const MacDesc& d1, const GroupOff& g, int B, hipStream_t s);
void launch_expand_round_group(const DevTables& T, const ExpandSideDesc& left, const ExpandSideDesc& right, const GroupOff& g, int B,
                               hipStream_t s);
void launch_reorient_group(u64* out, const u32* v, int first, int step, int dim0, const GroupOff& g, int B, hipStream_t s);
void launch_copy_polys_group(u32* dst, const int* dst_idx, int dst_row_stride, const u32* src, const int* src_idx, int src_row_stride,
                             int R, int batch, const GroupOff& g, int B, hipStream_t s);
void launch_folding_neg_group(const DevTables& T, u32* mats, const u32* gadget_ntt, int nu2, int two_t, const GroupOff& g, int B,
                              hipStream_t s);
void launch_mats_to_wave_group(u32* dst, const u32* src, size_t n_words, int half_polys, const GroupOff& g, int B, hipStream_t s);
struct ExpandWaveDesc {
  const u64* raw;
  const int* pos;
  const int* out_idx;
  const u32* A_w;
  const u32* const_w;
  u32* v;
  int cnt, t, bits;
};
void launch_expand_wave(const DevTables& T, const ExpandWaveDesc& d, const GroupOff& g, int B, hipStream_t s);
constexpr long EXPAND_WAVE_MIN_DIGITS_DEFAULT = 16;
constexpr long EXPAND_GROUP_ROUND_MIN_DEFAULT = 4096;

struct FoldDesc {
  const u64* X;
  u64* Y;
  const u32* mats;
  int cur, half, planes;
  int t, bits;
  int t_live;
  int zero_shortcuts;
  const u32* mats_w;
};
void launch_mats_to_wave(u32* dst, const u32* src, size_t n_words, hipStream_t s, int half_polys = 0);
constexpr long FOLD_VARIANT_DEFAULT = 5;
void launch_fold_fused(const DevTables& T, const FoldDesc& d, hipStream_t s);

void launch_add_poly_into(const DevTables& T, u32* dst, const int* idx, const u32* src, int batch, hipStream_t s);
void launch_scalar_mul(const DevTables& T, u32* base, long dst_off, long src_off, const u32* scalar, int n_polys,
                       hipStream_t s);
void launch_add_polys_idx(const DevTables& T, u32* dst, const int* di, const u32* a, const int* ai, const u32* b,
                          const int* bi, int count, hipStream_t s);
void launch_interleave_query(u64* qv, const u32* row0_ntt, const u64* wire, int dim0, hipStream_t s);
void launch_copy_polys(u32* dst, const int* dst_idx, int dst_row_stride, const u32* src, const int* src_idx,
                       int src_row_stride, int R, int batch, hipStream_t s);
void launch_folding_neg(const DevTables& T, u32* mats, const u32* gadget_ntt, int nu2, int two_t, hipStream_t s);
void launch_add(const DevTables& T, u32* out, const u32* a, const u32* b, int n_polys, hipStream_t s);
void launch_invert_raw(const DevTables& T, u64* out, const u64* a, long n_words, hipStream_t s);
void launch_automorph(const DevTables& T, u64* out, const u64* a, int n_polys, int t, hipStream_t s);
void launch_gadget_raw(u64* out, const u64* inp, int rows_in, int cols, int rows_out, int rdim, int bits,
                       hipStream_t s);
void launch_u64_to_u32(u32* out, const u64* in, long n, hipStream_t s);
void launch_u32_to_u64(u64* out, const u32* in, long n, hipStream_t s);

void launch_cu_probe(u32* out, int blocks, hipStream_t s);

struct EncodeDesc {
  const u64* packed;
  unsigned long long* out;
  int instances, n;
  u64 Q, q1, q2;
  int q1_bits, q2_bits;
};
void launch_encode(const EncodeDesc& d, hipStream_t s);

void launch_reorient(u64* out, const u32* v, int first, int step, int dim0, hipStream_t s);

struct CopyPolysDesc {
  u32* dst;
  const int* dst_idx;
  int dst_row_stride;
  const u32* src;
  const int* src_idx;
  int src_row_stride, R, batch;
};
struct FoldingNegDesc {
  u32* mats;
  const u32* gadget_ntt;
  int two_t, nu2;
};
struct ReorientDesc {
  u64* out;
  const u32* v;
  int first, step, dim0;
};
struct MatsToWaveDesc {
  u32* dst;
  const u32* src;
  size_t n_words;
  int half_polys;
};
struct AddPolyIntoDesc {
  u32* dst;
  const int* idx;
  const u32* src;
  int batch;
};
struct CopyWordsDesc {
  u32* dst;
  const u32* src;
  size_t n_words;
};
constexpr u64 PP_RAW_WIRE = 1ull << 63;
struct PpRawDesc {
  u64* dst;
  const u64* wire;
  const u64* table;
  u64 n_words;
  u64 modulus, modulus_inv;
};
void launch_pp_raw_image(const PpRawDesc& d, int n_polys, hipStream_t s);

struct SweepDesc {
  const u64* db;
  const u64* qv;
  u32* out;
  int planes, num_per, dim0, j0, nj;
  int packed;
  int out_G;
  int nt_store;
};
struct ColMap {
  int off = 0, stride = 1, np_global = 0;
};
inline bool db_can_pack(int num_per, int nj) { return num_per >= 128 && (nj % 2) == 0; }
inline size_t db_bytes(int planes, int num_per, int nj, bool packed) {
  return (size_t)planes * N * nj * num_per * (packed ? 7 : 8);
}
void launch_sweep(const DevTables& T, const SweepDesc& d, hipStream_t s);
void launch_sweep_persist(const DevTables& T, const SweepDesc& d, int wgs_per_cu, hipStream_t s, int n_cus = 256);
constexpr int SWEEP_BATCH_MAX = 8;
constexpr int SWEEP_GROUP_MAX = 16;
struct SweepBatchDesc {
  const u64* db;
  const u64* qv[SWEEP_GROUP_MAX];
  u32* out[SWEEP_GROUP_MAX];
  int batch;
  int planes, num_per, dim0, j0, nj;
  u32* rq;
  int use_mfma;
  const unsigned char* planar;
  int narrow;
  int fold_every;
};
bool sweep_narrow_batch_shape_ok(int num_per, int nj);
constexpr long NARROW_BATCH_MIN_DEFAULT = 0;
void launch_sweep_narrow_batch(const DevTables& T, const SweepBatchDesc& d, hipStream_t s);
bool sweep_planar_shape_ok(int num_per, int nj);
size_t sweep_planar_bytes(int planes, int num_per, int nj);
void launch_packed_to_planar(unsigned char* planar, const u64* packed, int planes, int num_per, int nj, hipStream_t s);
void launch_planar_patch_item(unsigned char* planar, const u64* packed, int planes, int num_per, int nj, int j, int ii, hipStream_t s);
constexpr size_t UPSERT_MAX_GROUP_PLANES = (size_t)1 << 23;
struct PlanarPatchCell {
  int j, ii;
};
void launch_planar_patch_items(unsigned char* planar, const u64* packed, int planes, int num_per, int nj, const PlanarPatchCell* cells,
                               size_t n_cells, hipStream_t s);
void launch_sweep_planar(const DevTables& T, const SweepBatchDesc& d, hipStream_t s);
bool planar_resident_shape_ok(int num_per, int nj);
int planar_resident_group_max(int nj);
struct PlanarShardShape {
  int dim0 = 0;
  int j0 = 0;
  int G = 1;
};
void launch_planar_from_ref(unsigned char* planar, const u64* src, int plane, int z0, int nz, int num_per, int nj, PlanarShardShape sh,
                            hipStream_t s);
void launch_planar_synth(unsigned char* planar, u64 seed, int planes, int num_per, int nj, PlanarShardShape sh, hipStream_t s);
void launch_planar_from_stage(unsigned char* planar, const u64* stage, int planes, int jg, int ii0, int ncols, int num_per, int nj,
                              PlanarShardShape sh, hipStream_t s);
void launch_planar_put_items(unsigned char* planar, const u64* stage, int planes, size_t np_s, const PlanarPatchCell* cells, size_t n_items,
                             int num_per, int nj, PlanarShardShape sh, hipStream_t s);
void launch_planar_read(u64* out, const unsigned char* planar, int plane, int z, int ii, int jl0, int count, int num_per, int nj,
                        PlanarShardShape sh, hipStream_t s);
void sweep_planar_resident_prepare(const DevTables& T, SweepBatchDesc& d, hipStream_t s);
void launch_sweep_planar_resident(const DevTables& T, const SweepBatchDesc& d, hipStream_t s);
void launch_sweep_planar_scatter(const DevTables& T, const SweepBatchDesc& d, int G, int plane0, int total_planes, bool all_planes,
                                 hipStream_t s);
bool sweep_batch_wants_mfma(const SweepBatchDesc& d);
int sweep_batch_group_max(int num_per, int nj);
inline int sweep_batch_tiles(int batch) { return batch > SWEEP_BATCH_MAX ? 2 : 1; }
inline size_t sweep_batch_rq_words(int nj, int tiles = 1) {
  return (size_t)tiles * ((size_t)N * (size_t)(nj / 16) * 128 * 4 + (size_t)N * 32);
}
void sweep_batch_prepare(const DevTables& T, SweepBatchDesc& d, hipStream_t s);
void launch_sweep_batch(const DevTables& T, const SweepBatchDesc& d, hipStream_t s);
constexpr long BATCH_SCATTER_STORE_DEFAULT = 2;
constexpr long BATCH_SCATTER_MAX_G_DEFAULT = 8;
bool sweep_batch_scatter_ok(const SweepBatchDesc& d, int G);
void launch_sweep_batch_scatter(const DevTables& T, const SweepBatchDesc& d, int G, hipStream_t s);
void launch_db_relayout(u64* dst, int plane, const u64* src, int z0, int nz, int num_per, int dim0, int j0, int nj,
                        int packed, ColMap cm, hipStream_t s);
void launch_canon_words(u64* w, size_t total, hipStream_t s);
void launch_db_synth(u64* dst, u64 seed, int planes, int num_per, int dim0, int j0, int nj, int packed, ColMap cm,
                     hipStream_t s);
void launch_db_read(u64* out, const u64* db, int plane, int z, int ii, int jl0, int count, int num_per, int nj,
                    int packed, hipStream_t s);
struct DbEncodeDesc {
  const uint8_t* win;
  size_t win_item0;
  size_t win_bytes;
  size_t file_len;
  u64* db;
  int db_item_size, bytes_per_chunk, logp;
  u32 pt_modulus;
  int planes, num_per, dim0, j0, nj, packed;
  int jp0, njp;
  long only_item;
  int only_q;
  ColMap cm;
};
void launch_db_encode(const DevTables& T, const DbEncodeDesc& d, hipStream_t s);
struct DbQuadRec {
  int jp, q;
  int len[4];
  long long src[4];
};
void launch_db_encode_quads(const DevTables& T, const DbEncodeDesc& d, const DbQuadRec* quads, size_t n_quads, hipStream_t s);

void launch_items_gather(u64* dst, const u64* db, size_t L0, size_t nL, int np_local, int nj, int planes, int packed, hipStream_t s);
void launch_planar_gather(u64* dst, const unsigned char* planar, size_t L0, size_t nL, int num_per, int nj, int planes, PlanarShardShape sh,
                          hipStream_t s);
struct ItemDecodeRec {
  int src, pos;
};
struct ItemDecodeDesc {
  const u64* src;
  const ItemDecodeRec* list;
  uint8_t* out;
  unsigned long long* undecodable;
  int planes, db_item_size, bytes_per_chunk, logp;
  u32 pt_modulus;
};
void launch_items_decode(const DevTables& T, const ItemDecodeDesc& d, size_t n_items, hipStream_t s);

void launch_items_scatter_words8(u64* db, const u64* stage, const int* src_of, size_t D0, size_t nD, int np_local, int nj, int planes,
                                 hipStream_t s);
struct CopyQuadRec {
  int jp, q;
  int src[4];
};
void launch_items_scatter_packed(u64* db, const u64* stage, const CopyQuadRec* quads, size_t n_quads, int np_local, int nj, int planes,
                                 hipStream_t s);
struct CopyCellRec {
  int j, ii;
  int src[16];
};
void launch_planar_scatter_items(unsigned char* planar, const u64* stage, const CopyCellRec* cells, size_t n_cells, int num_per, int nj,
                                 int planes, PlanarShardShape sh, hipStream_t s);
struct CopySlotRec {
  int src, slot;
};
void launch_items_copy_slots(u64* polys, const u64* stage, const CopySlotRec* recs, size_t n_recs, int planes, hipStream_t s);

void launch_sparse_item_encode(const DevTables& T, const uint8_t* bytes, int item_bytes, int bytes_per_chunk, int logp,
                               u32 pt_modulus, u64* slot_polys, int planes, hipStream_t s);
struct SparseItemRec {
  unsigned long long off;
  int len, slot;
};
void launch_sparse_items_encode(const DevTables& T, const uint8_t* win, const SparseItemRec* items, size_t n_items, int item_bytes,
                                int bytes_per_chunk, int logp, u32 pt_modulus, u64* polys, int planes, hipStream_t s);
void launch_sweep_sparse(const DevTables& T, const int* col_ptr, const int* col_rows, const int* col_slots, const u64* polys,
                         int planes, const u32* v, int first, int step, u32* out, int num_per, hipStream_t s);
constexpr int SPARSE_GROUP_MAX = 8;
constexpr long SPARSE_BATCH_MIN_DEFAULT = 2;
struct SparseGroup {
  const u32* v[SPARSE_GROUP_MAX];
  u32* out[SPARSE_GROUP_MAX];
};
void launch_sweep_sparse_batch(const DevTables& T, const int* col_ptr, const int* col_rows, const int* col_slots, const u64* polys,
                               int planes, const SparseGroup& members, int nq, int first, int step, int num_per, hipStream_t s);
void launch_sweep_sparse_scatter(const DevTables& T, const int* col_ptr, const int* col_rows, const int* col_slots, const u64* polys,
                                 int planes, int plane0, int n_planes, const u32* v, int first, int step, u32* out, int num_per, int G,
                                 bool per_plane, hipStream_t s);
void launch_sweep_sparse_scatter_batch(const DevTables& T, const int* col_ptr, const int* col_rows, const int* col_slots, const u64* polys,
                                       int planes, const SparseGroup& members, int nq, int first, int step, int num_per, int G,
                                       hipStream_t s);

void launch_sweep_out_to_ref(u64* out, const u32* in, int num_per, hipStream_t s);

__host__ __device__ inline u64 synth_word(u64 seed, u64 idx) {
  u64 z = seed + 0x9E3779B97F4A7C15ULL * (idx + 1);
  z = (z ^ (z >> 30)) * 0xBF58476D1CE4E5B9ULL;
  z = (z ^ (z >> 27)) * 0x94D049BB133111EBULL;
  z ^= z >> 31;
  u64 lo = (u32)z % (u32)MODULUS_0;
  u64 hi = (u32)(z >> 32) % (u32)MODULUS_1;
  return lo | (hi << 32);
}

__host__ __device__ inline u64 digest_mix(u64 x) {
  x += 0x9E3779B97F4A7C15ULL;
  x = (x ^ (x >> 30)) * 0xBF58476D1CE4E5B9ULL;
  x = (x ^ (x >> 27)) * 0x94D049BB133111EBULL;
  return x ^ (x >> 31);
}
__host__ __device__ inline u64 digest_col_key(u64 s, u64 c) { return digest_mix(s ^ c) | 1ULL; }
__host__ __device__ inline u64 digest_row_key(u64 s, u64 j) { return digest_mix(~s ^ j) | 1ULL; }
constexpr int DIGEST_ROWS = 1024;
struct DigestDesc {
  unsigned long long* sums;
  const u64* R;
  u64 s[2];
  int plane0, nplanes;
  int num_per;
  int nj;
};
void launch_digest_keys(unsigned long long* sums, u64* R, u64 seed, int nplanes, int j0, int nj, hipStream_t s);
void launch_digest_words(const DigestDesc& d, const u64* db, int np_local, int packed, ColMap cm, hipStream_t s);
struct DigestSlotRec {
  unsigned long long slot, item;
};
void launch_digest_sparse(const DigestDesc& d, const u64* polys, int planes, const DigestSlotRec* list, size_t n, hipStream_t s);
void launch_digest_planar(const DigestDesc& d, const unsigned char* planar, PlanarShardShape sh, hipStream_t s);

constexpr int ITEM_DIGEST_Z = 64;
struct ItemDigestDesc {
  unsigned long long* table;
  const u64* R;
  u64 s[2];
  int plane0, nplanes;
  int num_per;
  int nj;
  int jl0, nrows;
};
void launch_item_digest_words(const ItemDigestDesc& d, const u64* db, int np_local, int packed, ColMap cm, hipStream_t s);
void launch_item_digest_sparse(const ItemDigestDesc& d, const u64* polys, int planes, const DigestSlotRec* list, size_t n,
                               unsigned long long item_base, uint8_t* present, hipStream_t s);
void launch_item_digest_planar(const ItemDigestDesc& d, const unsigned char* planar, PlanarShardShape sh, hipStream_t s);

}
```

sdk_amd/csrc/ntt.hip:

```cpp
#include "device_common.hpp"
#include "bodies.hpp"

namespace spiral {

template <int M>
__global__ __launch_bounds__(256) void k_ntt_core_bench(DevTables T, u32* out, int reps) {
  __shared__ u32 lds0[M * LDS_WORDS];
  __shared__ u32 lds1[M * LDS_WORDS];
  const int tau = threadIdx.x;
  const ModConst m = T.c.mod[blockIdx.x & 1];
  const u32* fw = T.tw + (size_t)(blockIdx.x & 1) * 4 * N;
  u32 v[M][8];
#pragma unroll
  for (int mm = 0; mm < M; mm++)
#pragma unroll
    for (int k = 0; k < 8; k++) v[mm][k] = (tau * 2654435761u + k * 40503u + mm + blockIdx.x) % m.q;
  u32* la = lds0;
  u32* lb = lds1;
  for (int r = 0; r < reps; r++) {
    const u32* fwk = fw;
    int tk = tau;
    asm volatile("" : "+s"(fwk));
    asm volatile("" : "+v"(tk));
    ntt_fwd_block_m<M>(v, tk, la, lb, fwk, fwk + N, m.q, m.two_q);
    u32* t = la;
    la = lb;
    lb = t;
  }
  u32 acc = 0;
#pragma unroll
  for (int mm = 0; mm < M; mm++)
#pragma unroll
    for (int k = 0; k < 8; k++) acc ^= v[mm][k];
  out[blockIdx.x * 256 + tau] = acc;
}
float bench_ntt_core(const DevTables& T, int M, int blocks, int reps, u32* scratch, hipStream_t s) {
  hipEvent_t a, b;
  (void)hipEventCreate(&a);
  (void)hipEventCreate(&b);
  auto go = [&] {
    switch (M) {
      case 1: hipLaunchKernelGGL(k_ntt_core_bench<1>, dim3(blocks), dim3(256), 0, s, T, scratch, reps); break;
      case 2: hipLaunchKernelGGL(k_ntt_core_bench<2>, dim3(blocks), dim3(256), 0, s, T, scratch, reps); break;
      default: hipLaunchKernelGGL(k_ntt_core_bench<4>, dim3(blocks), dim3(256), 0, s, T, scratch, reps); break;
    }
  };
  go();
  (void)hipEventRecord(a, s);
  go();
  (void)hipEventRecord(b, s);
  (void)hipEventSynchronize(b);
  float ms = 0;
  (void)hipEventElapsedTime(&ms, a, b);
  (void)hipEventDestroy(a);
  (void)hipEventDestroy(b);
  return ms;
}

__global__ __launch_bounds__(256) void k_ntt_fwd(DevTables T, FwdDesc d) {
  __shared__ u32 ldsA[LDS_WORDS];
  __shared__ u32 ldsB[LDS_WORDS];
  ntt_fwd_body(T, d, blockIdx.x, blockIdx.y, ldsA, ldsB);
}
__global__ __launch_bounds__(256) void k_ntt_fwd3(DevTables T, FwdDesc d0, FwdDesc d1, FwdDesc d2) {
  __shared__ u32 ldsA[LDS_WORDS];
  __shared__ u32 ldsB[LDS_WORDS];
  int o = blockIdx.x;
  if (o < d0.n_out) {
    ntt_fwd_body(T, d0, o, blockIdx.y, ldsA, ldsB);
  } else if (o < d0.n_out + d1.n_out) {
    ntt_fwd_body(T, d1, o - d0.n_out, blockIdx.y, ldsA, ldsB);
  } else {
    ntt_fwd_body(T, d2, o - d0.n_out - d1.n_out, blockIdx.y, ldsA, ldsB);
  }
}
__global__ __launch_bounds__(256) void k_ntt_fwd3_group(DevTables T, FwdDesc d0, FwdDesc d1, FwdDesc d2, GroupOff g) {
  __shared__ u32 ldsA[LDS_WORDS];
  __shared__ u32 ldsB[LDS_WORDS];
  const int qi = blockIdx.z;
  int o = blockIdx.x;
  FwdDesc d = d0;
  long long dst_off = g.dig[qi];
  if (o >= d0.n_out + d1.n_out) {
    d = d2;
    o -= d0.n_out + d1.n_out;
    dst_off = g.ct1[qi];
  } else if (o >= d0.n_out) {
    d = d1;
    o -= d0.n_out;
  }
  d.src = group_rebase(d.src, g.raw[qi]);
  d.dst = group_rebase(d.dst, dst_off);
  ntt_fwd_body(T, d, o, blockIdx.y, ldsA, ldsB);
}
void launch_ntt_fwd3_group(const DevTables& T, const FwdDesc& d0, const FwdDesc& d1, const FwdDesc& d2, const GroupOff& g, int B,
                           hipStream_t s) {
  const int total = std::max(d0.n_out, 0) + std::max(d1.n_out, 0) + std::max(d2.n_out, 0);
  if (total <= 0 || B <= 0) return;
  FwdDesc a = d0, b = d1, c = d2;
  a.n_out = std::max(a.n_out, 0);
  b.n_out = std::max(b.n_out, 0);
  c.n_out = std::max(c.n_out, 0);
  hipLaunchKernelGGL(k_ntt_fwd3_group, dim3(total, 2, B), dim3(256), 0, s, T, a, b, c, g);
  launched(PATH_EXPAND_GROUP, "k_ntt_fwd3_group");
}
void launch_ntt_fwd(const DevTables& T, const FwdDesc& d, hipStream_t s) {
  if (d.n_out <= 0) return;
  hipLaunchKernelGGL(k_ntt_fwd, dim3(d.n_out, 2), dim3(256), 0, s, T, d);
  launched(0, "k_ntt_fwd");
}
void launch_ntt_fwd3(const DevTables& T, const FwdDesc& d0, const FwdDesc& d1, const FwdDesc& d2, hipStream_t s) {
  const int total = std::max(d0.n_out, 0) + std::max(d1.n_out, 0) + std::max(d2.n_out, 0);
  if (total <= 0) return;
  FwdDesc a = d0, b = d1, c = d2;
  a.n_out = std::max(a.n_out, 0);
  b.n_out = std::max(b.n_out, 0);
  c.n_out = std::max(c.n_out, 0);
  hipLaunchKernelGGL(k_ntt_fwd3, dim3(total, 2), dim3(256), 0, s, T, a, b, c);
  launched(0, "k_ntt_fwd3");
}

constexpr int EXPAND_GD = 4;
static __device__ __forceinline__ void expand_round_body(const DevTables& T, const ExpandSideDesc& d, int b, int c, u32* lds0, u32* lds1) {
  constexpr int GD = EXPAND_GD;
  const int tau = threadIdx.x;
  const ModConst m = T.c.mod[c];
  const u32* fw = T.tw + (size_t)c * 4 * N;
  const u64* src = d.raw + (size_t)d.pos[b] * 2 * N;
  u64 x[8];
#pragma unroll
  for (int k = 0; k < 8; k++) x[k] = src[tau + 256 * k];
  const u64 mask = (1ULL << d.bits) - 1ULL;
  u64 acc0[8], acc1[8];
#pragma unroll
  for (int k = 0; k < 8; k++) acc0[k] = acc1[k] = 0;
#pragma unroll 1
  for (int k0 = 0; k0 < d.t; k0 += GD) {
    u32 v[GD][8];
#pragma unroll
    for (int mm = 0; mm < GD; mm++) {
      const int sh = (k0 + mm) * d.bits;
      const bool live = k0 + mm < d.t && sh < 64;
#pragma unroll
      for (int k = 0; k < 8; k++) v[mm][k] = live ? (u32)((x[k] >> (sh & 63)) & mask) : 0u;
    }
    int tk = tau;
    const u32* fwk = fw;
    asm volatile("" : "+v"(tk));
    asm volatile("" : "+s"(fwk));
    ntt_fwd_block_m<GD>(v, tk, lds0, lds1, fwk, fwk + N, m.q, m.two_q);
#pragma unroll
    for (int mm = 0; mm < GD; mm++) {
      const int kk = k0 + mm;
      if (kk < d.t) {
        const uint4* a0 = reinterpret_cast<const uint4*>(d.A + ((size_t)kk * 2 + c) * N + 8 * tk);
        const uint4* a1 = reinterpret_cast<const uint4*>(d.A + ((size_t)(d.t + kk) * 2 + c) * N + 8 * tk);
        const uint4 p0 = a0[0], p1 = a0[1], r0 = a1[0], r1 = a1[1];
        acc0[0] += (u64)p0.x * v[mm][0]; acc0[1] += (u64)p0.y * v[mm][1]; acc0[2] += (u64)p0.z * v[mm][2]; acc0[3] += (u64)p0.w * v[mm][3];
        acc0[4] += (u64)p1.x * v[mm][4]; acc0[5] += (u64)p1.y * v[mm][5]; acc0[6] += (u64)p1.z * v[mm][6]; acc0[7] += (u64)p1.w * v[mm][7];
        acc1[0] += (u64)r0.x * v[mm][0]; acc1[1] += (u64)r0.y * v[mm][1]; acc1[2] += (u64)r0.z * v[mm][2]; acc1[3] += (u64)r0.w * v[mm][3];
        acc1[4] += (u64)r1.x * v[mm][4]; acc1[5] += (u64)r1.y * v[mm][5]; acc1[6] += (u64)r1.z * v[mm][6]; acc1[7] += (u64)r1.w * v[mm][7];
      }
    }
    if (((k0 / GD) & 7) == 7) {
#pragma unroll
      for (int k = 0; k < 8; k++) {
        acc0[k] = reduce64(acc0[k], m);
        acc1[k] = reduce64(acc1[k], m);
      }
    }
    __syncthreads();
  }
  u32 e1[8];
#pragma unroll
  for (int k = 0; k < 8; k++) e1[k] = reduce64(src[(size_t)N + tau + 256 * k], m);
  ntt_fwd_block(e1, tau, lds0, lds1, fw, fw + N, m.q, m.two_q);
  u32* o0 = d.v + ((size_t)d.out_idx[b] * 2 + c) * N + 8 * tau;
  u32* o1 = o0 + (size_t)2 * N;
  const uint4 g0 = reinterpret_cast<const uint4*>(o0)[0], g1 = reinterpret_cast<const uint4*>(o0)[1];
  const uint4 h0 = reinterpret_cast<const uint4*>(o1)[0], h1 = reinterpret_cast<const uint4*>(o1)[1];
  const u32 ga[8] = {g0.x, g0.y, g0.z, g0.w, g1.x, g1.y, g1.z, g1.w};
  const u32 ha[8] = {h0.x, h0.y, h0.z, h0.w, h1.x, h1.y, h1.z, h1.w};
  u32 w0[8], w1[8];
#pragma unroll
  for (int k = 0; k < 8; k++) {
    w0[k] = reduce64(acc0[k] + ga[k], m);
    w1[k] = reduce64(acc1[k] + (u64)ha[k] + e1[k], m);
  }
  reinterpret_cast<uint4*>(o0)[0] = make_uint4(w0[0], w0[1], w0[2], w0[3]);
  reinterpret_cast<uint4*>(o0)[1] = make_uint4(w0[4], w0[5], w0[6], w0[7]);
  reinterpret_cast<uint4*>(o1)[0] = make_uint4(w1[0], w1[1], w1[2], w1[3]);
  reinterpret_cast<uint4*>(o1)[1] = make_uint4(w1[4], w1[5], w1[6], w1[7]);
}
__global__ __launch_bounds__(256) void k_expand_round(DevTables T, ExpandSideDesc dl, ExpandSideDesc dr) {
  __shared__ u32 lds0[EXPAND_GD * LDS_WORDS];
  __shared__ u32 lds1[EXPAND_GD * LDS_WORDS];
  const bool right = (int)blockIdx.x >= dl.cnt;
  expand_round_body(T, right ? dr : dl, (int)blockIdx.x - (right ? dl.cnt : 0), blockIdx.y, lds0, lds1);
}
__global__ __launch_bounds__(256) void k_expand_round_group(DevTables T, ExpandSideDesc dl, ExpandSideDesc dr, GroupOff g) {
  __shared__ u32 lds0[EXPAND_GD * LDS_WORDS];
  __shared__ u32 lds1[EXPAND_GD * LDS_WORDS];
  const int qi = blockIdx.z;
  const bool right = (int)blockIdx.x < dr.cnt;
  ExpandSideDesc d = right ? dr : dl;
  d.raw = group_rebase(d.raw, g.raw[qi]);
  d.A = group_rebase(d.A, g.pp[qi]);
  d.v = group_rebase(d.v, g.v[qi]);
  expand_round_body(T, d, (int)blockIdx.x - (right ? 0 : dr.cnt), blockIdx.y, lds0, lds1);
}
void launch_expand_round_group(const DevTables& T, const ExpandSideDesc& left, const ExpandSideDesc& right, const GroupOff& g, int B,
                               hipStream_t s) {
  const int total = std::max(left.cnt, 0) + std::max(right.cnt, 0);
  if (total <= 0 || B <= 0) return;
  ExpandSideDesc a = left, b = right;
  a.cnt = std::max(a.cnt, 0);
  b.cnt = std::max(b.cnt, 0);
  hipLaunchKernelGGL(k_expand_round_group, dim3(total, 2, B), dim3(256), 0, s, T, a, b, g);
  launched(PATH_EXPAND_FUSED | PATH_EXPAND_GROUP, "k_expand_round_group");
}
void launch_expand_round(const DevTables& T, const ExpandSideDesc& left, const ExpandSideDesc& right, hipStream_t s) {
  const int total = std::max(left.cnt, 0) + std::max(right.cnt, 0);
  if (total <= 0) return;
  ExpandSideDesc a = left, b = right;
  a.cnt = std::max(a.cnt, 0);
  b.cnt = std::max(b.cnt, 0);
  hipLaunchKernelGGL(k_expand_round, dim3(total, 2), dim3(256), 0, s, T, a, b);
  launched(PATH_EXPAND_FUSED, "k_expand_round");
}

__global__ __launch_bounds__(256) void k_ntt_inv(DevTables T, InvDesc d) {
  __shared__ u32 ldsA[LDS_WORDS];
  __shared__ u32 ldsB[LDS_WORDS];
  ntt_inv_body(T, d, blockIdx.x, ldsA, ldsB);
}
__global__ __launch_bounds__(256) void k_ntt_inv_group(DevTables T, InvDesc d, GroupOff g) {
  __shared__ u32 ldsA[LDS_WORDS];
  __shared__ u32 ldsB[LDS_WORDS];
  const int qi = blockIdx.y;
  d.src = group_rebase(d.src, g.v[qi]);
  d.scal_dst = group_rebase(d.scal_dst, g.v[qi]);
  d.dst = group_rebase(d.dst, g.raw[qi]);
  ntt_inv_body(T, d, blockIdx.x, ldsA, ldsB);
}
void launch_ntt_inv_group(const DevTables& T, const InvDesc& d, const GroupOff& g, int B, hipStream_t s) {
  const int blocks = d.n_polys + (d.scal ? 2 * d.n_scalar_only : 0);
  if (blocks <= 0 || B <= 0) return;
  hipLaunchKernelGGL(k_ntt_inv_group, dim3(blocks, B), dim3(256), 0, s, T, d, g);
  launched(PATH_EXPAND_GROUP, "k_ntt_inv_group");
}
void launch_ntt_inv(const DevTables& T, const InvDesc& d, hipStream_t s) {
  const int blocks = d.n_polys + (d.scal ? 2 * d.n_scalar_only : 0);
  if (blocks <= 0) return;
  hipLaunchKernelGGL(k_ntt_inv, dim3(blocks), dim3(256), 0, s, T, d);
  launched(d.sweep_np > 0 ? PATH_FROM_SWEEP1 : 0, "k_ntt_inv");
}

__global__ __launch_bounds__(256, 2) void k_from_sweep4(DevTables T, const u32* src, int np, int premod, u64* dst, int xcd_map) {
  __shared__ u32 lds0[4 * LDS_WORDS];
  __shared__ u32 lds1[4 * LDS_WORDS];
  const int tau = threadIdx.x;
  int g = blockIdx.x;
  if (xcd_map & 1) {
    const int xcd = g & 7, t = g >> 3;
    g = ((t >> 3) * 8 + xcd) * 8 + (t & 7);
  }
  const int gpr = np / 4;
  const int groups_per_plane = gpr * 2;
  const int plane = g / groups_per_plane, rem = g % groups_per_plane;
  const int r = rem / gpr, gl = rem % gpr;
  const int ii0 = gl * 4;
  const size_t base = ((size_t)plane * 4 + r * 2) * N * np + ii0;
  u32 res0[4][8];
  uint4 xin[2][8];
#pragma unroll
  for (int c = 0; c < 2; c++)
#pragma unroll
    for (int k = 0; k < 8; k++)
      xin[c][k] = *reinterpret_cast<const uint4*>(src + base + (size_t)c * N * np + (size_t)(8 * tau + k) * np);
#pragma unroll
  for (int c = 0; c < 2; c++) {
    const ModConst m = T.c.mod[c];
    u32 v[4][8];
#pragma unroll
    for (int k = 0; k < 8; k++) {
      uint4 x = xin[c][k];
      if (premod) {
        x.x %= m.q; x.y %= m.q; x.z %= m.q; x.w %= m.q;
      }
      v[0][k] = x.x; v[1][k] = x.y; v[2][k] = x.z; v[3][k] = x.w;
    }
    const u32* iw = inv_tables(T.tw, c);
    if (c == 1) __syncthreads();
    ntt_inv_block_m<4>(v, tau, lds0, lds1, iw, iw + N, m.q, m.two_q);
    if (c == 0) {
#pragma unroll
      for (int mm = 0; mm < 4; mm++)
#pragma unroll
        for (int k = 0; k < 8; k++) res0[mm][k] = v[mm][k];
    } else {
      const u32 q0 = T.c.mod[0].q, q1 = T.c.mod[1].q;
#pragma unroll
      for (int mm = 0; mm < 4; mm++) {
        u64* out = dst + (((size_t)plane * np + ii0 + mm) * 2 + r) * N;
#pragma unroll
        for (int k = 0; k < 8; k++) {
          u32 x = res0[mm][k], y = v[mm][k];
          u32 xm = x >= q1 ? x - q1 : x;
          u32 dd = y >= xm ? y - xm : y + q1 - xm;
          u32 qt = __umulhi(dd, T.c.q0_inv_q1_sh);
          u32 e = dd * T.c.q0_inv_q1 - qt * q1;
          e = e >= q1 ? e - q1 : e;
          const u64 val = (u64)x + (u64)q0 * (u64)e;
          out[tau + 256 * k] = val;
        }
      }
    }
  }
}
void launch_from_sweep4(const DevTables& T, const u32* src, int np, int n_planes, int premod, u64* dst, hipStream_t s) {
  if (n_planes <= 0) return;
  const unsigned groups = (unsigned)((np / 4) * 2 * n_planes);
  const int xcd_map = tunable("from_sweep_xcd", 1) != 0 && (np % 32) == 0 && (groups % 64) == 0;
  hipLaunchKernelGGL(k_from_sweep4, dim3(groups), dim3(256), 0, s, T, src, np, premod, dst, xcd_map);
  launched(PATH_FROM_SWEEP4 | (xcd_map ? PATH_SWEEP_XCD_FROM : 0), "k_from_sweep4");
}

}
```

sdk_amd/csrc/pipeline.hpp:

```cpp
#pragma once
#include <vector>

#include "server.hpp"

namespace spiral {

struct Workspace {
  const Params* P;
  DeviceState* D;
  int device = -1;
  hipStream_t stream = nullptr;
  hipStream_t stream2 = nullptr;
  std::vector<hipEvent_t> ev_plane;
  hipEvent_t ev_fold = nullptr;
  hipEvent_t ev_round0 = nullptr, ev_right = nullptr;
  bool right_pending = false;
  bool long_sweep_follows = false;
  hipEvent_t ev_sw[2] = {nullptr, nullptr};
  bool have_sweep_span = false;
  bool pipelined = false;
  hipEvent_t ev[5] = {nullptr, nullptr, nullptr, nullptr, nullptr};
  DevBuf<u64> q_raw;
  DevBuf<u32> v;
  DevBuf<u64> exp_raw;
  DevBuf<u32> exp_dig;
  DevBuf<u32> exp_ct1;
  DevBuf<u64> exp_raw_r;
  DevBuf<u32> exp_dig_r, exp_ct1_r;
  DevBuf<u64> qv;
  DevBuf<u32> fold_mats;
  DevBuf<u32> fold_mats_w;
  bool mats_w_ready = false;
  DevBuf<u64> gsw_raw;
  DevBuf<u32> gsw_dig;
  DevBuf<u32> sweep_out;
  DevBuf<u64> fold_tail;
  DevBuf<u32> batch_rq;
  DevBuf<u64> foldX, foldY, final_cts, pack_raw;
  DevBuf<u32> fold_dig, fold_ntt, pack_dig, pack_ct2, pack_res, pack_v1_P, pack_v1_P2;
  DevBuf<u64> pack_v1_raw, du_raw, du_wire;
  DevBuf<u32> du_ntt;
  u64* h_query = nullptr;
  u64* h_group_query = nullptr;
  DevBuf<u64> group_q_raw;
  u64* h_packed = nullptr;
  size_t h_packed_words = 0;
  DevBuf<u64> enc_out;
  uint8_t* h_response = nullptr;
  bool host_pinned = true;
  int out_G = 1;
  bool zero_shortcuts = false;
  long fused_min_pairs = 256;

  Workspace(const Params& P, DeviceState& D);
  ~Workspace();
  Workspace(const Workspace&) = delete;
  Workspace& operator=(const Workspace&) = delete;
  void ensure_expand();
  void ensure_sweep();
  void ensure_finish();
  size_t plane_group() const;
};

void run_coefficient_expansion(Workspace& W, const sp_pp& pp, size_t g_rounds, const DeviceState::PrunedPlan* plan = nullptr,
                               int tree = 0, size_t r_begin = 0);
void join_right(Workspace& W);
void run_regev_to_gsw(Workspace& W, const sp_pp& pp, const u32* v_src, const int* src_ct, const int* src_poly);
void run_folding_neg(Workspace& W);
void run_mats_to_wave(Workspace& W, size_t levels, bool c_only = false);
void run_fold_operands(Workspace& W);
void run_begin_direct(Workspace& W, const uint8_t* query);
void run_begin_group(Workspace* const* Ws, const sp_pp* const* pps, const uint8_t* const* queries, const size_t* query_lens, int B);
void run_begin(Workspace& W, const sp_pp& pp, const uint8_t* query, size_t query_len, int j0 = 0, int nj = 0,
               const DeviceState::PrunedPlan* plan = nullptr);
void run_sweep_sparse(Workspace& W, const sp_db& db, const int* col_ptr, const int* col_rows, const int* col_slots);
void run_sweep_sparse_group(Workspace* const* Ws, int B, const sp_db& db, const int* col_ptr, const int* col_rows, const int* col_slots,
                            hipStream_t s);
void run_sweep_sparse_scatter(Workspace& W, const sp_db& db, const int* col_ptr, const int* col_rows, const int* col_slots, int G,
                              int plane0, int n_planes, bool per_plane);
void run_sweep_sparse_scatter_group(Workspace* const* Ws, int B, const sp_db& db, const int* col_ptr, const int* col_rows,
                                    const int* col_slots, int G, hipStream_t s);
std::unique_ptr<DeviceState::PrunedPlan> build_pruned_plan_rows(const Params& P, const std::vector<char>& rows);
void run_sweep(Workspace& W, const sp_db& db);
void run_sweep_pipelined(Workspace& W, const sp_db& db);
bool sweep_is_pipelined(const Params& p, const sp_db& db);
void launch_plane_sweep(Workspace& W, const sp_db& db, size_t plane);
bool fused_fold_supported(const Params& p);
struct FoldOpts {
  long fused_min_pairs;
  bool delta_tail;
  bool inputs_below_q;
};
u64* run_fold(Workspace& W, const FoldOpts& o, u64* X, u64* Y, int np, int num_cts, int top, int d_begin = 0, int d_end = -1);
void run_fold_local(Workspace& W, const u32* reduced_chunk, int G);
void run_fold_local_plane(Workspace& W, const u32* reduced_plane_chunk, int G, int plane);
void run_fold_local_join(Workspace& W);
void run_finish_gathered(Workspace& W, const sp_pp& pp, const u64* gathered, int G);
void run_fold_all(Workspace& W, bool premod);
void run_pack(Workspace& W, const sp_pp& pp);
void run_finish(Workspace& W, const sp_pp& pp, bool premod);
size_t encode_response(const Params& p, const u64* packed, uint8_t* out);
void run_encode_device(Workspace& W);

}
```

sdk_amd/csrc/server.cpp:

```cpp
#include "server.hpp"

#include <algorithm>
#include <atomic>
#include <cstdlib>
#include <cstring>
#include <functional>

#include "pipeline.hpp"

namespace spiral {

void hip_check(hipError_t e, const char* what, const char* file, int line) {
  if (e != hipSuccess) {
    (void)hipGetLastError();
    throw HipError(std::string(what) + " failed at " + file + ":" + std::to_string(line) + ": " + hipGetErrorString(e));
  }
}

static std::mutex g_tun_mu;
static std::vector<std::pair<std::string, long>> g_tun;
static std::atomic<unsigned> g_tun_epoch{1};
static std::atomic<long> g_fresh_allocs{0};
void tunables_new_call() { g_tun_epoch.fetch_add(1, std::memory_order_relaxed); }
void set_tunable(const char* name, long v) {
// ... 968 lines not shown
    const long long dv = off(W.v.p, W0.v.p), dm = off(W.fold_mats.p, W0.fold_mats.p);
    g_reo.v[i] = dv;   g_reo.raw[i] = off(W.qv.p, W0.qv.p);
    g_copy.v[i] = dv;  g_copy.raw[i] = dm;
    g_inv.v[i] = dv;   g_inv.raw[i] = off(W.gsw_raw.p, W0.gsw_raw.p);
    g_fwd.raw[i] = g_inv.raw[i];  g_fwd.dig[i] = off(W.gsw_dig.p, W0.gsw_dig.p);
    g_mac.pp[i] = off(pps[i]->all.p, pps[0]->all.p);  g_mac.dig[i] = g_fwd.dig[i];  g_mac.v[i] = dm;
    g_neg.v[i] = dm;
    g_wave.v[i] = dm;  g_wave.raw[i] = off(W.fold_mats_w.p, W0.fold_mats_w.p);
    if (pps[i]->off_conv != pps[0]->off_conv) throw ArgError("a group's public parameters must have one layout");
  }
  launch_reorient_group(W0.qv.p, W0.v.p, 0, 2, (int)p.dim0(), g_reo, B, s);
  if (nb > 0) {
    launch_copy_polys_group(W0.fold_mats.p, L + D.gsw_out_odd, four_t, W0.v.p, L + D.gsw_src_poly, 1, 2, nb, g_copy, B, s);
    InvDesc inv{};
    inv.src = W0.v.p;
    inv.idx = L + D.gsw_src_ct;
    inv.polys_per_idx = 2;
    inv.idx_stride = 4 * POLY_LEN;
    inv.poly_stride = 2 * POLY_LEN;
    inv.crt_stride = POLY_LEN;
    inv.z_stride = 1;
    inv.dst = W0.gsw_raw.p;
    inv.n_polys = nb * 2;
    launch_ntt_inv_group(D.T, inv, g_inv, B, s);
    FwdDesc f{};
    f.src = W0.gsw_raw.p;
    f.dst = W0.gsw_dig.p;
    f.n_out = nb * 2 * (int)p.t_conv;
    f.rdim = 2;
    f.cols = 1;
    f.t = (int)p.t_conv;
    f.bits = (int)p.bits_per(p.t_conv);
    f.src_batch_stride = 2;
    f.src_row0 = 0;
    f.src_cols = 1;
    FwdDesc none{};
    launch_ntt_fwd3_group(D.T, f, none, none, g_fwd, B, s);
    MacDesc m{};
    m.A = pps[0]->all.p + pps[0]->off_conv * 2 * POLY_LEN;
    m.B = W0.gsw_dig.p;
    m.out = W0.fold_mats.p;
    m.out_idx = L + D.gsw_out_even;
    m.R = 2;
    m.K = 2 * (int)p.t_conv;
    m.batch_inner = nb;
    m.batch_outer = 1;
    m.B_inner_stride = 2 * p.t_conv;
    m.split_k = m.K;
    m.out_row_stride = four_t;
    MacDesc none_m{};
    launch_mac2_group(D.T, m, none_m, g_mac, B, s);
  }
  const bool neg = tunable("fold_neg_materialise", 0) != 0;
  if (neg) launch_folding_neg_group(D.T, W0.fold_mats.p, D.gadget_gsw.p, (int)p.db_dim_2, (int)(2 * p.t_gsw), g_neg, B, s);
  launch_mats_to_wave_group(W0.fold_mats_w.p, W0.fold_mats.p, mats_words, neg ? 0 : (int)(2 * p.t_gsw), g_wave, B, s);
  for (int i = 0; i < B; i++) Ws[i]->mats_w_ready = true;
}

void run_begin_group(Workspace* const* Ws, const sp_pp* const* pps, const uint8_t* const* queries, const size_t* query_lens, int B) {
  Workspace& W0 = *Ws[0];
  const Params& p = *W0.P;
  if (!p.expand_queries) throw ArgError("run_begin_group: direct-upload queries have no expansion to share");
  if (!W0.h_group_query) {
    if (W0.host_pinned)
      HIP_CHECK(hipHostMalloc((void**)&W0.h_group_query, (size_t)GROUP_MAX * 2 * POLY_LEN * sizeof(u64), hipHostMallocDefault));
    else if (!(W0.h_group_query = (u64*)malloc((size_t)GROUP_MAX * 2 * POLY_LEN * sizeof(u64))))
      throw OomError("host staging allocation failed");
  }
  W0.group_q_raw.ensure((size_t)GROUP_MAX * 2 * POLY_LEN);
  GroupOff gq{};
  for (int i = 0; i < B; i++) {
    Workspace& W = *Ws[i];
    query_ct_host(W, queries[i], query_lens[i], W0.h_group_query + (size_t)i * 2 * POLY_LEN);
    W.ensure_expand();
    if (W.right_pending) {
      HIP_CHECK(hipStreamWaitEvent(W0.stream, W.ev_right, 0));
      W.right_pending = false;
    }
    gq.raw[i] = (long long)((size_t)i * 2 * POLY_LEN * sizeof(u64));
    gq.dig[i] = (long long)((uintptr_t)W.v.p - (uintptr_t)W0.v.p);
  }
  HIP_CHECK(hipMemcpyAsync(W0.group_q_raw.p, W0.h_group_query, (size_t)B * 2 * POLY_LEN * sizeof(u64), hipMemcpyHostToDevice, W0.stream));
  {
    FwdDesc f{W0.group_q_raw.p, nullptr, W0.v.p, 2, 1, 1, 1, 64, 1, 0, 1};
    FwdDesc none{};
    launch_ntt_fwd3_group(W0.D->T, f, none, none, gq, B, W0.stream);
  }
  note_path(PATH_EXPAND_GROUP);
  run_group_expansion(Ws, pps, B, p.g());
  if (tunable("expand_group_tail", 1) != 0 && fused_fold_supported(p) && tunable("fold_variant", FOLD_VARIANT_DEFAULT) == 5 && p.db_dim_2 > 0)
    run_group_after_rounds(Ws, pps, B);
  else
    for (int i = 0; i < B; i++) {
      Workspace& W = *Ws[i];
      hipStream_t own = W.stream;
      W.stream = W0.stream;
      try {
        run_begin_after_rounds(W, *pps[i]);
      } catch (...) {
        W.stream = own;
        throw;
      }
      W.stream = own;
    }
  HIP_CHECK(hipEventRecord(W0.ev_round0, W0.stream));
  for (int i = 1; i < B; i++) HIP_CHECK(hipStreamWaitEvent(Ws[i]->stream, W0.ev_round0, 0));
}

void run_begin(Workspace& W, const sp_pp& pp, const uint8_t* query, size_t query_len, int j0, int nj,
               const DeviceState::PrunedPlan* plan) {
  const Params& p = *W.P;
  DeviceState& D = *W.D;
  if (query_len != p.query_bytes()) throw ArgError("query length " + std::to_string(query_len) + " != query_bytes " + std::to_string(p.query_bytes()));
  if (!p.expand_queries) {
    run_begin_direct(W, query);
    return;
  }
  run_begin_query_ct(W, query, query_len);
  hipStream_t s = W.stream;
  const size_t g = p.g();
  const bool prune = p.db_dim_2 > 0 && nj > 0 && (j0 != 0 || nj != (int)p.dim0());
  if (prune || (plan && p.db_dim_2 > 0)) note_path(PATH_EXPAND_PRUNED);
  const DeviceState::PrunedPlan* pl = plan && p.db_dim_2 > 0 ? plan : (prune ? &D.pruned_plan(p, j0, nj) : nullptr);
  const int* L = D.lists.p;
  const long split_mode = tunable("expand_split", -1);
  if (p.db_dim_2 > 0 && g >= 2 && (split_mode > 0 || (split_mode < 0 && W.long_sweep_follows))) {
    note_path(PATH_EXPAND_SPLIT);
    run_coefficient_expansion(W, pp, 1, pl, 0, 0);
    HIP_CHECK(hipEventRecord(W.ev_round0, s));
    HIP_CHECK(hipStreamWaitEvent(W.stream2, W.ev_round0, 0));
    on_stream(W, W.stream2, [&] {
      run_coefficient_expansion(W, pp, g, pl, 2, 1);
      run_regev_to_gsw(W, pp, W.v.p, L + D.gsw_src_ct, L + D.gsw_src_poly);
      run_fold_operands(W);
    });
    HIP_CHECK(hipEventRecord(W.ev_right, W.stream2));
    W.right_pending = true;
    run_coefficient_expansion(W, pp, g, pl, 1, 1);
    launch_reorient(W.qv.p, W.v.p, 0, 2, (int)p.dim0(), s);
    return;
  }
  run_coefficient_expansion(W, pp, g, pl);
  run_begin_after_rounds(W, pp);
}

void join_right(Workspace& W) {
  if (W.right_pending) HIP_CHECK(hipStreamWaitEvent(W.stream, W.ev_right, 0));
}

void run_sweep(Workspace& W, const sp_db& db) {
  if (db.planar_resident) throw ArgError("the single-query sweep kernels do not read a planar-resident database (sp_db_create_planar)");
  const Params& p = *W.P;
  W.ensure_sweep();
  SweepDesc d{db.words.p, W.qv.p, W.sweep_out.p, (int)p.planes(), db.np_local, (int)p.dim0(), db.j0, db.nj, db.packed, W.out_G};
  d.nt_store = (int)tunable("sweep_nt_store", 1);
  launch_sweep(W.D->T, d, W.stream);
}

void run_sweep_sparse(Workspace& W, const sp_db& db, const int* col_ptr, const int* col_rows, const int* col_slots) {
  const Params& p = *W.P;
  W.ensure_sweep();
  launch_sweep_sparse(W.D->T, col_ptr, col_rows, col_slots, db.polys.p, (int)p.planes(), W.v.p, 0,
                      p.db_dim_2 > 0 ? 2 : 1, W.sweep_out.p, (int)p.num_per(), W.stream);
}

void run_sweep_sparse_group(Workspace* const* Ws, int B, const sp_db& db, const int* col_ptr, const int* col_rows, const int* col_slots,
                            hipStream_t s) {
  const Params& p = *Ws[0]->P;
  SparseGroup g{};
  for (int b = 0; b < B; b++) {
    Ws[b]->ensure_sweep();
    g.v[b] = Ws[b]->v.p;
    g.out[b] = Ws[b]->sweep_out.p;
  }
  launch_sweep_sparse_batch(Ws[0]->D->T, col_ptr, col_rows, col_slots, db.polys.p, (int)p.planes(), g, B, 0, p.db_dim_2 > 0 ? 2 : 1,
                            (int)p.num_per(), s);
}

void run_sweep_sparse_scatter(Workspace& W, const sp_db& db, const int* col_ptr, const int* col_rows, const int* col_slots, int G,
                              int plane0, int n_planes, bool per_plane) {
  const Params& p = *W.P;
  W.ensure_sweep();
  launch_sweep_sparse_scatter(W.D->T, col_ptr, col_rows, col_slots, db.polys.p, (int)p.planes(), plane0, n_planes, W.v.p, 0,
                              p.db_dim_2 > 0 ? 2 : 1, W.sweep_out.p, (int)p.num_per(), G, per_plane, W.stream);
}
void run_sweep_sparse_scatter_group(Workspace* const* Ws, int B, const sp_db& db, const int* col_ptr, const int* col_rows,
                                    const int* col_slots, int G, hipStream_t s) {
  const Params& p = *Ws[0]->P;
  SparseGroup g{};
  for (int b = 0; b < B; b++) {
    Ws[b]->ensure_sweep();
    g.v[b] = Ws[b]->v.p;
    g.out[b] = Ws[b]->sweep_out.p;
  }
  launch_sweep_sparse_scatter_batch(Ws[0]->D->T, col_ptr, col_rows, col_slots, db.polys.p, (int)p.planes(), g, B, 0,
                                    p.db_dim_2 > 0 ? 2 : 1, (int)p.num_per(), G, s);
}

static FoldOpts query_fold_opts(const Workspace& W, bool below_q) {
  return FoldOpts{std::min(W.fused_min_pairs, tunable("fused_min_pairs_cap", 1L << 62)), true, below_q};
}

static void fold_planes(Workspace& W, size_t pg0, int np, bool premod) {
  const Params& p = *W.P;
  DeviceState& D = *W.D;
  hipStream_t s = W.stream;
  if (p.num_per() % 4 == 0 && !tunable("from_sweep1", 0)) {
    launch_from_sweep4(D.T, W.sweep_out.p + pg0 * 4 * POLY_LEN * p.num_per(), (int)p.num_per(), np, premod ? 1 : 0,
                       W.foldX.p, s);
  } else {
    InvDesc inv{};
    inv.src = W.sweep_out.p + pg0 * 4 * POLY_LEN * p.num_per();
    inv.sweep_np = (int)p.num_per();
    inv.dst = W.foldX.p;
    inv.n_polys = np * (int)p.num_per() * 2;
    inv.premod = premod ? 1 : 0;
    launch_ntt_inv(D.T, inv, s);
  }
  u64* res = run_fold(W, query_fold_opts(W, true), W.foldX.p, W.foldY.p, np, (int)p.num_per(), -1);
  HIP_CHECK(hipMemcpyAsync(W.final_cts.p + pg0 * 2 * POLY_LEN, res, (size_t)np * 2 * POLY_LEN * sizeof(u64), hipMemcpyDeviceToDevice, s));
}

static int tail_defer_levels(const Params& p, long stop) {
  if (stop <= 0 || !fused_fold_supported(p) || p.planes() < 2) return 0;
  int lv = 0;
  size_t cur = p.num_per();
  while (cur > (size_t)stop && cur / 2 >= 1 && (cur & 1) == 0) { cur >>= 1; lv++; }
  return cur == (size_t)stop && lv > 0 && stop >= 2 ? lv : 0;
}
static void fold_plane_head(Workspace& W, size_t pl, int levels) {
  const Params& p = *W.P;
  launch_from_sweep4(W.D->T, W.sweep_out.p + pl * 4 * POLY_LEN * p.num_per(), (int)p.num_per(), 1, 0, W.foldX.p, W.stream);
  u64* res = run_fold(W, query_fold_opts(W, true), W.foldX.p, W.foldY.p, 1, (int)p.num_per(), -1, 0, levels);
  const size_t cts = p.num_per() >> levels;
  HIP_CHECK(hipMemcpyAsync(W.fold_tail.p + pl * cts * 2 * POLY_LEN, res, cts * 2 * POLY_LEN * sizeof(u64), hipMemcpyDeviceToDevice, W.stream));
}
static void fold_tails(Workspace& W, int levels) {
  const Params& p = *W.P;
  const size_t cts = p.num_per() >> levels;
  u64* other = W.fold_tail.p + p.planes() * cts * 2 * POLY_LEN;
  u64* res = run_fold(W, query_fold_opts(W, true), W.fold_tail.p, other, (int)p.planes(), (int)p.num_per(), -1, levels, -1);
  HIP_CHECK(hipMemcpyAsync(W.final_cts.p, res, p.planes() * 2 * POLY_LEN * sizeof(u64), hipMemcpyDeviceToDevice, W.stream));
}

bool sweep_is_pipelined(const Params& p, const sp_db& db) {
  const bool enabled = tunable("pipeline", 1) != 0;
  return enabled && db.packed && db.num_shards == 1 && db.col_G == 1 && p.planes() > 1 && p.num_per() >= 1024;
}

void launch_plane_sweep(Workspace& W, const sp_db& db, size_t pl) {
  if (db.planar_resident) throw ArgError("the single-query sweep kernels do not read a planar-resident database (sp_db_create_planar)");
  const Params& p = *W.P;
  const size_t np_ = (size_t)db.np_local;
  const size_t plane_db_words = db_bytes(1, db.np_local, db.nj, db.packed) / 8;
  SweepDesc d{db.words.p + pl * plane_db_words, W.qv.p, W.sweep_out.p + pl * 4 * POLY_LEN * np_, 1, db.np_local,
              (int)p.dim0(), db.j0, db.nj, db.packed, W.out_G};
  d.nt_store = (int)tunable("sweep_nt_store", 1);
  const int wgs = (int)tunable("pipe_wgs", 4);
  if (db.packed && wgs > 0)
    launch_sweep_persist(W.D->T, d, wgs, W.stream);
  else
    launch_sweep(W.D->T, d, W.stream);
}

void run_sweep_pipelined(Workspace& W, const sp_db& db) {
  const Params& p = *W.P;
  W.ensure_sweep();
  W.ensure_finish();
  const size_t planes = p.planes();
  HIP_CHECK(hipEventRecord(W.ev_sw[0], W.stream));
  const int defer_levels = tail_defer_levels(p, tunable("pipe_tail_defer", 256));
  if (defer_levels > 0) {
    W.fold_tail.ensure(2 * planes * (p.num_per() >> defer_levels) * 2 * POLY_LEN);
    note_path(PATH_FOLD_TAIL_BATCHED);
  }
  for (size_t pl = 0; pl < planes; pl++) {
    launch_plane_sweep(W, db, pl);
    HIP_CHECK(hipEventRecord(W.ev_plane[pl], W.stream));
    HIP_CHECK(hipStreamWaitEvent(W.stream2, W.ev_plane[pl], 0));
    if (defer_levels > 0) {
      on_stream(W, W.stream2, [&] {
        fold_plane_head(W, pl, defer_levels);
        if (pl + 1 == planes) fold_tails(W, defer_levels);
      });
      continue;
    }
    on_stream(W, W.stream2, [&] { fold_planes(W, pl, 1, false); });
  }
  HIP_CHECK(hipEventRecord(W.ev_sw[1], W.stream));
  HIP_CHECK(hipEventRecord(W.ev_fold, W.stream2));
  W.have_sweep_span = true;
  W.pipelined = true;
  note_path(PATH_PIPELINED);
}

bool fused_fold_supported(const Params& p) { return 4 * p.t_gsw <= 128 && p.bits_per(p.t_gsw) <= 28; }

u64* run_fold(Workspace& W, const FoldOpts& o, u64* X, u64* Y, int np, int num_cts, int top, int d_begin, int d_end) {
  const Params& p = *W.P;
  DeviceState& D = *W.D;
  hipStream_t s = W.stream;
  const int two_t = (int)(2 * p.t_gsw);
  join_right(W);
  int further = 0;
  while (((int)1 << further) < num_cts) further++;
  const int top_idx = top < 0 ? further - 1 : top;
  if (d_end < 0) d_end = further;
  int cur = num_cts >> d_begin;
  for (int d = d_begin; d < d_end; d++) {
    const int half = cur / 2;
    if (W.zero_shortcuts && !fused_fold_supported(p))
      throw ArgError("sparse buckets need gadget parameters the fused fold supports (3 <= t_gsw <= 32)");
    if (W.zero_shortcuts || ((long)np * half >= o.fused_min_pairs && fused_fold_supported(p))) {
      FoldDesc fd{};
      fd.zero_shortcuts = W.zero_shortcuts ? 1 : 0;
      fd.mats_w = W.mats_w_ready ? W.fold_mats_w.p + (size_t)(top_idx - d) * 2 * 2 * two_t * 2 * POLY_LEN : nullptr;
      fd.X = X;
      fd.Y = Y;
      fd.mats = W.fold_mats.p + (size_t)(top_idx - d) * 2 * 2 * two_t * 2 * POLY_LEN;
      fd.cur = cur;
      fd.half = half;
      fd.planes = np;
      fd.t = (int)p.t_gsw;
      fd.bits = (int)p.bits_per(p.t_gsw);
      fd.t_live = o.inputs_below_q && tunable("fold_skip_dead_digits", 1)
                      ? (int)std::min<size_t>(p.t_gsw, (p.modulus_log2 + fd.bits - 1) / fd.bits) : fd.t;
      launch_fold_fused(D.T, fd, s);
      std::swap(X, Y);
      cur = half;
      continue;
    }
    if (o.delta_tail) {
      FwdDesc f{};
      f.src = X;
      f.dst = W.fold_dig.p;
      f.n_out = np * half * two_t;
      f.rdim = 2;
      f.cols = 1;
      f.t = (int)p.t_gsw;
      f.bits = (int)p.bits_per(p.t_gsw);
      f.src_batch_stride = 2;
      f.src_row0 = 0;
      f.src_cols = 1;
      f.delta_off = (long)half * 2;
      f.delta_inner = half;
      f.delta_outer_stride = cur;
      launch_ntt_fwd(D.T, f, s);
      MacDesc m{};
      m.A = W.fold_mats.p + ((size_t)(top_idx - d) * 2 * 2 * two_t + two_t) * 2 * POLY_LEN;
      m.A_row_stride = 2 * two_t;
      m.B = W.fold_dig.p;
      m.out = W.fold_ntt.p;
      m.R = 2;
      m.K = two_t;
      m.batch_inner = np * half;
      m.batch_outer = 1;
      m.B_inner_stride = two_t;
      m.split_k = two_t;
      m.out_batch_stride = 2;
      m.out_row_stride = 1;
      launch_mac(D.T, m, s);
      InvDesc inv{};
      inv.src = W.fold_ntt.p;
      inv.poly_stride = 2 * POLY_LEN;
      inv.crt_stride = POLY_LEN;
      inv.z_stride = 1;
      inv.dst = Y;
      inv.n_polys = np * half * 2;
      inv.addend = X;
      inv.add_inner2 = half * 2;
      inv.add_outer_stride = cur * 2;
      launch_ntt_inv(D.T, inv, s);
      note_path(PATH_FOLD_TAIL);
      std::swap(X, Y);
      cur = half;
      continue;
    }
    FwdDesc f{};
    f.src = X;
    f.dst = W.fold_dig.p;
    f.n_out = np * cur * two_t;
    f.rdim = 2;
    f.cols = 1;
    f.t = (int)p.t_gsw;
    f.bits = (int)p.bits_per(p.t_gsw);
    f.src_batch_stride = 2;
    f.src_row0 = 0;
    f.src_cols = 1;
    launch_ntt_fwd(D.T, f, s);
    MacDesc m{};
    m.A = W.fold_mats.p + (size_t)(top_idx - d) * 2 * 2 * two_t * 2 * POLY_LEN;
    m.B = W.fold_dig.p;
    m.out = W.fold_ntt.p;
    m.R = 2;
    m.K = 2 * two_t;
    m.batch_inner = half;
    m.batch_outer = np;
    m.B_inner_stride = two_t;
    m.B_outer_stride = (long)cur * two_t;
    m.split_k = two_t;
    m.split_off = (long)half * two_t;
    m.out_batch_stride = 2;
    m.out_row_stride = 1;
    launch_mac(D.T, m, s);
    InvDesc inv{};
    inv.src = W.fold_ntt.p;
    inv.poly_stride = 2 * POLY_LEN;
    inv.crt_stride = POLY_LEN;
    inv.z_stride = 1;
    inv.dst = Y;
    inv.n_polys = np * half * 2;
    launch_ntt_inv(D.T, inv, s);
    note_path(PATH_FOLD_TAIL_LITERAL);
    std::swap(X, Y);
    cur = half;
  }
  return X;
}

static void run_pack_v1(Workspace& W, const sp_pp& pp) {
  const Params& p = *W.P;
  DeviceState& D = *W.D;
  hipStream_t s = W.stream;
  const int* L = D.lists.p;
  const int tc = (int)p.t_conv;
  note_path(PATH_PACK_V1);
  const int nb = (int)p.planes();
  const int ne = (int)p.instances * 2;
  const size_t PW = 2 * POLY_LEN;
  W.pack_v1_P.ensure((size_t)nb * 3 * PW);
  W.pack_v1_P2.ensure((size_t)ne * 3 * PW);
  W.pack_v1_raw.ensure((size_t)ne * POLY_LEN);
  const u32* w_key = pp.all.p + (pp.off_packing + 0 * 3 * tc) * PW;
  const u32* w_shift = pp.all.p + (pp.off_packing + 1 * 3 * tc) * PW;
  FwdDesc f{};
  f.src = W.final_cts.p;
  f.src_idx = L + D.pack_src_ct;
  f.dst = W.pack_dig.p;
  f.n_out = nb * tc;
  f.rdim = 1; f.cols = 1; f.t = tc; f.bits = (int)p.bits_per(tc);
// ... 242 lines not shown
```

sdk_amd/csrc/sweep.hip:

```cpp
#include "device_common.hpp"
#include "sweep_mfma.hpp"
#include "server.hpp"

namespace spiral {

__device__ __forceinline__ size_t sweep_out_index(const SweepDesc& d, int plane, int rc, int z, int ii) {
  const int G = d.out_G > 1 ? d.out_G : 1;
  const int npl = d.num_per / G;
  const size_t chunk_words = (size_t)d.planes * 4 * N * npl;
  return (size_t)(ii % G) * chunk_words + (((size_t)plane * 4 + rc) * N + z) * npl + (ii / G);
}
__device__ __forceinline__ void sweep_store_pair(const SweepDesc& d, int plane, int z, int ii0, u32 r0c0_a, u32 r0c0_b,
                                                 u32 r0c1_a, u32 r0c1_b, u32 r1c0_a, u32 r1c0_b, u32 r1c1_a,
                                                 u32 r1c1_b) {
  if (d.out_G <= 1 && d.nt_store) {
    const size_t rc = (size_t)N * d.num_per;
    u32* o = d.out + (size_t)plane * 4 * rc + (size_t)z * d.num_per + ii0;
    __builtin_nontemporal_store(mf_u32x2_t{r0c0_a, r0c0_b}, reinterpret_cast<mf_u32x2_t*>(o + 0 * rc));
    __builtin_nontemporal_store(mf_u32x2_t{r0c1_a, r0c1_b}, reinterpret_cast<mf_u32x2_t*>(o + 1 * rc));
    __builtin_nontemporal_store(mf_u32x2_t{r1c0_a, r1c0_b}, reinterpret_cast<mf_u32x2_t*>(o + 2 * rc));
    __builtin_nontemporal_store(mf_u32x2_t{r1c1_a, r1c1_b}, reinterpret_cast<mf_u32x2_t*>(o + 3 * rc));
  } else if (d.out_G <= 1) {
    const size_t rc = (size_t)N * d.num_per;
    u32* o = d.out + (size_t)plane * 4 * rc + (size_t)z * d.num_per + ii0;
    *reinterpret_cast<uint2*>(o + 0 * rc) = make_uint2(r0c0_a, r0c0_b);
    *reinterpret_cast<uint2*>(o + 1 * rc) = make_uint2(r0c1_a, r0c1_b);
    *reinterpret_cast<uint2*>(o + 2 * rc) = make_uint2(r1c0_a, r1c0_b);
    *reinterpret_cast<uint2*>(o + 3 * rc) = make_uint2(r1c1_a, r1c1_b);
  } else {
    d.out[sweep_out_index(d, plane, 0, z, ii0)] = r0c0_a;
    d.out[sweep_out_index(d, plane, 0, z, ii0 + 1)] = r0c0_b;
    d.out[sweep_out_index(d, plane, 1, z, ii0)] = r0c1_a;
    d.out[sweep_out_index(d, plane, 1, z, ii0 + 1)] = r0c1_b;
    d.out[sweep_out_index(d, plane, 2, z, ii0)] = r1c0_a;
    d.out[sweep_out_index(d, plane, 2, z, ii0 + 1)] = r1c0_b;
    d.out[sweep_out_index(d, plane, 3, z, ii0)] = r1c1_a;
    d.out[sweep_out_index(d, plane, 3, z, ii0 + 1)] = r1c1_b;
  }
}

__global__ __launch_bounds__(256) void k_sweep_wide(DevTables T, SweepDesc d) {
  const int lane = threadIdx.x & 63;
  const int unit = __builtin_amdgcn_readfirstlane(blockIdx.x * 4 + (threadIdx.x >> 6));
  const int chunks = d.num_per >> 7;
  const int chunk = unit % chunks;
  const int zp = unit / chunks;
  const int z = zp & (N - 1);
  const int plane = zp >> POLY_LEN_LOG2;
  if (plane >= d.planes) return;
  const ulonglong2* p =
      reinterpret_cast<const ulonglong2*>(d.db + ((size_t)zp * d.nj) * d.num_per + (size_t)chunk * 128) + lane;
  const size_t stride = (size_t)(d.num_per >> 1);
  const uint4* __restrict__ qrow = reinterpret_cast<const uint4*>(d.qv) + ((size_t)z * d.dim0 + d.j0);
  const ModConst m0 = T.c.mod[0], m1 = T.c.mod[1];

  u64 a00 = 0, a01 = 0, a02 = 0, a03 = 0;
  u64 a10 = 0, a11 = 0, a12 = 0, a13 = 0;
  for (int jb = 0; jb < d.nj; jb += 256) {
    const int je = min(jb + 256, d.nj);
    for (int j = jb; j < je; j++) {
      const ulonglong2* a = p + (size_t)j * stride;
      ulonglong2 w;
      w.x = __builtin_nontemporal_load(&a->x);
      w.y = __builtin_nontemporal_load(&a->y);
      const uint4 qa = qrow[j];
      const u32 b0l = (u32)w.x, b0h = (u32)(w.x >> 32);
      const u32 b1l = (u32)w.y, b1h = (u32)(w.y >> 32);
      a00 += (u64)qa.x * b0l;
      a01 += (u64)qa.z * b0l;
      a02 += (u64)qa.y * b0h;
      a03 += (u64)qa.w * b0h;
      a10 += (u64)qa.x * b1l;
      a11 += (u64)qa.z * b1l;
      a12 += (u64)qa.y * b1h;
      a13 += (u64)qa.w * b1h;
    }
    a00 = reduce64(a00, m0);
    a01 = reduce64(a01, m0);
    a02 = reduce64(a02, m1);
    a03 = reduce64(a03, m1);
    a10 = reduce64(a10, m0);
    a11 = reduce64(a11, m0);
    a12 = reduce64(a12, m1);
    a13 = reduce64(a13, m1);
  }
  sweep_store_pair(d, plane, z, chunk * 128 + 2 * lane, (u32)a00, (u32)a10, (u32)a02, (u32)a12, (u32)a01, (u32)a11,
                   (u32)a03, (u32)a13);
}

typedef u32 u32x4_t __attribute__((ext_vector_type(4)));
typedef u32 u32x3_t __attribute__((ext_vector_type(3), aligned(4)));

__global__ __launch_bounds__(256) void k_sweep_packed_persist(DevTables T, SweepDesc d, int units, int hi_prio) {
  if (hi_prio) __builtin_amdgcn_s_setprio(3);
  constexpr int U = 4;
  const int lane = threadIdx.x & 63;
  const int wave0 = __builtin_amdgcn_readfirstlane(blockIdx.x * 4 + (threadIdx.x >> 6));
  const int nwaves = gridDim.x * 4;
  const int chunks = d.num_per >> 7;
  const int npairs = d.nj >> 1;
  const size_t ustride = 448;
  const ModConst m0 = T.c.mod[0], m1 = T.c.mod[1];
  const u32 M = 0x0FFFFFFFu;
  for (int unit = wave0; unit < units; unit += nwaves) {
    const int chunk = unit % chunks;
    const int zp = unit / chunks;
    const int z = zp & (N - 1);
    const int plane = zp >> POLY_LEN_LOG2;
    const u32* base = reinterpret_cast<const u32*>(d.db) + packed_unit_offset((size_t)zp, 0, chunk, npairs, chunks);
    const uint4* __restrict__ qrow = reinterpret_cast<const uint4*>(d.qv) + ((size_t)z * d.dim0 + d.j0);
    u64 a00 = 0, a01 = 0, a02 = 0, a03 = 0, a10 = 0, a11 = 0, a12 = 0, a13 = 0;
    for (int jb = 0; jb < npairs; jb += 128) {
      const int je = min(jb + 128, npairs);
      for (int jp0 = jb; jp0 < je; jp0 += U) {
        u32x4_t va[U];
        u32x3_t vb[U];
#pragma unroll
        for (int u = 0; u < U; u++) {
          const int jp = min(jp0 + u, je - 1);
          const u32* uu = base + (size_t)jp * ustride;
          va[u] = __builtin_nontemporal_load(reinterpret_cast<const u32x4_t*>(uu + lane * 4));
          vb[u] = __builtin_nontemporal_load(reinterpret_cast<const u32x3_t*>(uu + 256 + lane * 3));
        }
#pragma unroll
        for (int u = 0; u < U; u++) {
          const int jp = jp0 + u;
          if (jp < je) {
            const u32 d0 = va[u].x, d1 = va[u].y, d2 = va[u].z, d3 = va[u].w, d4 = vb[u].x, d5 = vb[u].y, d6 = vb[u].z;
            const uint4 qa = qrow[2 * jp];
            const uint4 qb = qrow[2 * jp + 1];
            const u32 f0 = d0 & M;
            const u32 f1 = __builtin_amdgcn_alignbit(d1, d0, 28) & M;
            const u32 f2 = __builtin_amdgcn_alignbit(d2, d1, 24) & M;
            const u32 f3 = __builtin_amdgcn_alignbit(d3, d2, 20) & M;
            const u32 f4 = __builtin_amdgcn_alignbit(d4, d3, 16) & M;
            const u32 f5 = __builtin_amdgcn_alignbit(d5, d4, 12) & M;
            const u32 f6 = __builtin_amdgcn_alignbit(d6, d5, 8) & M;
            const u32 f7 = d6 >> 4;
            a00 += (u64)qa.x * f0; a01 += (u64)qa.z * f0; a02 += (u64)qa.y * f1; a03 += (u64)qa.w * f1;
            a10 += (u64)qa.x * f2; a11 += (u64)qa.z * f2; a12 += (u64)qa.y * f3; a13 += (u64)qa.w * f3;
            a00 += (u64)qb.x * f4; a01 += (u64)qb.z * f4; a02 += (u64)qb.y * f5; a03 += (u64)qb.w * f5;
            a10 += (u64)qb.x * f6; a11 += (u64)qb.z * f6; a12 += (u64)qb.y * f7; a13 += (u64)qb.w * f7;
          }
        }
      }
      a00 = reduce64(a00, m0); a01 = reduce64(a01, m0); a02 = reduce64(a02, m1); a03 = reduce64(a03, m1);
      a10 = reduce64(a10, m0); a11 = reduce64(a11, m0); a12 = reduce64(a12, m1); a13 = reduce64(a13, m1);
    }
    sweep_store_pair(d, plane, z, chunk * 128 + 2 * lane, (u32)a00, (u32)a10, (u32)a02, (u32)a12, (u32)a01, (u32)a11,
                     (u32)a03, (u32)a13);
  }
}
typedef __attribute__((address_space(4))) const u32x4_t sweep_const_uint4;
template <int U>
__global__ __launch_bounds__(256) void k_sweep_packed_ring(DevTables T, SweepDesc d, int units, int hi_prio) {
  if (hi_prio) __builtin_amdgcn_s_setprio(3);
  const int lane = threadIdx.x & 63;
  const int wave0 = __builtin_amdgcn_readfirstlane(blockIdx.x * 4 + (threadIdx.x >> 6));
  const int nwaves = gridDim.x * 4;
  const int chunks = d.num_per >> 7;
  const int npairs = d.nj >> 1;
  const size_t ustride = 448;
  const ModConst m0 = T.c.mod[0], m1 = T.c.mod[1];
  const u32 M = 0x0FFFFFFFu;
  if (wave0 >= units) return;
  u32x4_t va[U], na[U];
  u32x3_t vb[U], nb[U];
#define SPR_BASE(UNIT) \
  (reinterpret_cast<const u32*>(d.db) + packed_unit_offset((size_t)((UNIT) / chunks), 0, (UNIT) % chunks, npairs, chunks))
#define SPR_LOAD(VA, VB, BASE, JP0)                                                                       \
  _Pragma("unroll") for (int uu = 0; uu < U; uu++) {                                                      \
    const u32* u = (BASE) + (size_t)((JP0) + uu) * ustride;                                               \
    VA[uu] = __builtin_nontemporal_load(reinterpret_cast<const u32x4_t*>(u + lane * 4));                  \
    VB[uu] = __builtin_nontemporal_load(reinterpret_cast<const u32x3_t*>(u + 256 + lane * 3));            \
  }
#define SPR_MAC(VA, VB, JP0)                                                                                              \
  _Pragma("unroll") for (int uu = 0; uu < U; uu++) {                                                                      \
    const int jp = (JP0) + uu;                                                                                            \
    const u32 d0 = VA[uu].x, d1 = VA[uu].y, d2 = VA[uu].z, d3 = VA[uu].w, d4 = VB[uu].x, d5 = VB[uu].y, d6 = VB[uu].z;    \
    const u32x4_t qa = qrow[2 * jp];                                                                                      \
    const u32x4_t qb = qrow[2 * jp + 1];                                                                                  \
    const u32 f0 = d0 & M;                                                                                                \
    const u32 f1 = __builtin_amdgcn_alignbit(d1, d0, 28) & M;                                                             \
    const u32 f2 = __builtin_amdgcn_alignbit(d2, d1, 24) & M;                                                             \
    const u32 f3 = __builtin_amdgcn_alignbit(d3, d2, 20) & M;                                                             \
    const u32 f4 = __builtin_amdgcn_alignbit(d4, d3, 16) & M;                                                             \
    const u32 f5 = __builtin_amdgcn_alignbit(d5, d4, 12) & M;                                                             \
    const u32 f6 = __builtin_amdgcn_alignbit(d6, d5, 8) & M;                                                              \
    const u32 f7 = d6 >> 4;                                                                                               \
    a00 += (u64)qa.x * f0; a01 += (u64)qa.z * f0; a02 += (u64)qa.y * f1; a03 += (u64)qa.w * f1;                           \
    a10 += (u64)qa.x * f2; a11 += (u64)qa.z * f2; a12 += (u64)qa.y * f3; a13 += (u64)qa.w * f3;                           \
    a00 += (u64)qb.x * f4; a01 += (u64)qb.z * f4; a02 += (u64)qb.y * f5; a03 += (u64)qb.w * f5;                           \
    a10 += (u64)qb.x * f6; a11 += (u64)qb.z * f6; a12 += (u64)qb.y * f7; a13 += (u64)qb.w * f7;                           \
  }
#define SPR_FOLD                                                                                          \
  a00 = reduce64(a00, m0); a01 = reduce64(a01, m0); a02 = reduce64(a02, m1); a03 = reduce64(a03, m1);     \
  a10 = reduce64(a10, m0); a11 = reduce64(a11, m0); a12 = reduce64(a12, m1); a13 = reduce64(a13, m1);
  const u32* base = SPR_BASE(wave0);
  SPR_LOAD(va, vb, base, 0)
  for (int unit = wave0; unit < units;) {
    const int chunk = unit % chunks;
    const int zp = unit / chunks;
    const int z = zp & (N - 1);
    const int plane = zp >> POLY_LEN_LOG2;
    const sweep_const_uint4* qrow =
        (const sweep_const_uint4*)(uintptr_t)(reinterpret_cast<const uint4*>(d.qv) + ((size_t)z * d.dim0 + d.j0));
    u64 a00 = 0, a01 = 0, a02 = 0, a03 = 0, a10 = 0, a11 = 0, a12 = 0, a13 = 0;
    int next_unit = units;
    const u32* next_base = base;
    for (int jb = 0; jb < npairs; jb += 128) {
      const int len = min(128, npairs - jb);
      int j = jb;
      for (; j + 2 * U < jb + len; j += 2 * U) {
        SPR_LOAD(na, nb, base, j + U)
        __builtin_amdgcn_sched_barrier(0);
        SPR_MAC(va, vb, j)
        SPR_LOAD(va, vb, base, j + 2 * U)
        __builtin_amdgcn_sched_barrier(0);
        SPR_MAC(na, nb, j + U)
      }
      SPR_LOAD(na, nb, base, j + U)
      __builtin_amdgcn_sched_barrier(0);
      SPR_MAC(va, vb, j)
      const bool more = jb + 128 < npairs;
      next_unit = unit + nwaves;
      next_base = next_unit < units ? SPR_BASE(next_unit) : base;
      const u32* nb_base = more ? base : next_base;
      const int nb_jp = more ? jb + 128 : 0;
      SPR_LOAD(va, vb, nb_base, nb_jp)
      __builtin_amdgcn_sched_barrier(0);
      SPR_MAC(na, nb, j + U)
      SPR_FOLD
    }
    sweep_store_pair(d, plane, z, chunk * 128 + 2 * lane, (u32)a00, (u32)a10, (u32)a02, (u32)a12, (u32)a01, (u32)a11,
                     (u32)a03, (u32)a13);
    base = next_base;
    unit = next_unit;
  }
#undef SPR_BASE
#undef SPR_LOAD
#undef SPR_MAC
#undef SPR_FOLD
}
void launch_sweep_persist(const DevTables& T, const SweepDesc& d, int wgs_per_cu, hipStream_t s, int n_cus) {
  const int units = d.planes * N * (d.num_per >> 7);
  const int prio = (int)tunable("sweep_prio", 1);
  const int npairs = d.nj >> 1;
  long ring = tunable("pipe_ring", 8);
  while (ring > 1 && (npairs % (2 * ring) != 0 || (ring != 2 && ring != 4 && ring != 8))) ring >>= 1;
  if (ring >= 2) {
    const int ring_wgs = (int)std::max(1L, tunable("pipe_ring_wgs", 1));
    const dim3 rgrid((unsigned)std::min(n_cus * ring_wgs, (units + 3) / 4));
    switch (ring) {
      case 2: hipLaunchKernelGGL(k_sweep_packed_ring<2>, rgrid, dim3(256), 0, s, T, d, units, prio); break;
      case 8: hipLaunchKernelGGL(k_sweep_packed_ring<8>, rgrid, dim3(256), 0, s, T, d, units, prio); break;
      default: hipLaunchKernelGGL(k_sweep_packed_ring<4>, rgrid, dim3(256), 0, s, T, d, units, prio); break;
    }
    launched(PATH_SWEEP_PERSIST | PATH_SWEEP_RING | (d.out_G > 1 ? PATH_SCATTER_OUT : 0), "k_sweep_packed_ring");
    return;
  }
  const dim3 grid((unsigned)std::min(n_cus * wgs_per_cu, (units + 3) / 4));
  hipLaunchKernelGGL(k_sweep_packed_persist, grid, dim3(256), 0, s, T, d, units, prio);
  launched(PATH_SWEEP_PERSIST | (d.out_G > 1 ? PATH_SCATTER_OUT : 0), "k_sweep_packed_persist");
}

constexpr int QLDS_ROWS = 512;
template <int B, int U, bool QLDS>
__global__ __launch_bounds__(256, 2) void k_sweep_packed_batch(DevTables T, SweepBatchDesc d) {
  extern __shared__ __attribute__((aligned(16))) unsigned char smem_q[];
  const int lane = threadIdx.x & 63;
  const int unit = __builtin_amdgcn_readfirstlane(blockIdx.x * 4 + (threadIdx.x >> 6));
  const int chunks = d.num_per >> 7;
  const int chunk = unit % chunks;
  const int zp = unit / chunks;
  const int z = zp & (N - 1);
  const int plane = zp >> POLY_LEN_LOG2;
  const uint4* qs = reinterpret_cast<const uint4*>(smem_q);
  if (QLDS) {
    const int zp0 = (blockIdx.x * 4) / chunks;
    const int z0 = zp0 & (N - 1);
    uint4* qw = reinterpret_cast<uint4*>(smem_q);
#pragma unroll
    for (int b = 0; b < B; b++) {
      const uint4* src = reinterpret_cast<const uint4*>(d.qv[b]) + ((size_t)z0 * d.dim0 + d.j0);
      for (int j = threadIdx.x; j < d.nj; j += 256) qw[b * QLDS_ROWS + j] = src[j];
    }
    __syncthreads();
  }
  if (plane >= d.planes) return;
  const int npairs = d.nj >> 1;
  const u32* base = reinterpret_cast<const u32*>(d.db) + packed_unit_offset((size_t)zp, 0, chunk, npairs, chunks);
  const size_t ustride = 448;
  const size_t qoff = (size_t)z * d.dim0 + d.j0;
  const ModConst m0 = T.c.mod[0], m1 = T.c.mod[1];
  const u32 M = 0x0FFFFFFFu;
  u64 acc[B][8];
#pragma unroll
  for (int b = 0; b < B; b++)
#pragma unroll
    for (int k = 0; k < 8; k++) acc[b][k] = 0;
  u32x4_t va[U], na[U];
  u32x3_t vb[U], nb[U];
#define SP_BATCH_LOAD(VA, VB, JP0)                                                                        \
  _Pragma("unroll") for (int uu = 0; uu < U; uu++) {                                                      \
    const u32* u = base + (size_t)((JP0) + uu) * ustride;                                                 \
    VA[uu] = __builtin_nontemporal_load(reinterpret_cast<const u32x4_t*>(u + lane * 4));                  \
    VB[uu] = __builtin_nontemporal_load(reinterpret_cast<const u32x3_t*>(u + 256 + lane * 3));            \
  }
#define SP_BATCH_MAC16(QA, QB, b)                                                                                        \
  acc[b][0] += (u64)QA.x * f0; acc[b][1] += (u64)QA.z * f0; acc[b][2] += (u64)QA.y * f1; acc[b][3] += (u64)QA.w * f1;     \
  acc[b][4] += (u64)QA.x * f2; acc[b][5] += (u64)QA.z * f2; acc[b][6] += (u64)QA.y * f3; acc[b][7] += (u64)QA.w * f3;     \
  acc[b][0] += (u64)QB.x * f4; acc[b][1] += (u64)QB.z * f4; acc[b][2] += (u64)QB.y * f5; acc[b][3] += (u64)QB.w * f5;     \
  acc[b][4] += (u64)QB.x * f6; acc[b][5] += (u64)QB.z * f6; acc[b][6] += (u64)QB.y * f7; acc[b][7] += (u64)QB.w * f7;
#define SP_BATCH_MAC(VA, VB, JP0)                                                                                         \
  _Pragma("unroll") for (int uu = 0; uu < U; uu++) {                                                                      \
    const int jp = (JP0) + uu;                                                                                            \
    const u32 d0 = VA[uu].x, d1 = VA[uu].y, d2 = VA[uu].z, d3 = VA[uu].w, d4 = VB[uu].x, d5 = VB[uu].y, d6 = VB[uu].z;    \
    const u32 f0 = d0 & M;                                                                                                \
    const u32 f1 = __builtin_amdgcn_alignbit(d1, d0, 28) & M;                                                             \
    const u32 f2 = __builtin_amdgcn_alignbit(d2, d1, 24) & M;                                                             \
    const u32 f3 = __builtin_amdgcn_alignbit(d3, d2, 20) & M;                                                             \
    const u32 f4 = __builtin_amdgcn_alignbit(d4, d3, 16) & M;                                                             \
    const u32 f5 = __builtin_amdgcn_alignbit(d5, d4, 12) & M;                                                             \
    const u32 f6 = __builtin_amdgcn_alignbit(d6, d5, 8) & M;                                                              \
    const u32 f7 = d6 >> 4;                                                                                               \
    if (QLDS) {                                                                                                           \
      uint4 qa_n = qs[2 * jp], qb_n = qs[2 * jp + 1];                                                                     \
      _Pragma("unroll") for (int b = 0; b < B; b++) {                                                                     \
        const uint4 qa = qa_n, qb = qb_n;                                                                                 \
        if (b + 1 < B) {                                                                                                  \
          qa_n = qs[(b + 1) * QLDS_ROWS + 2 * jp];                                                                        \
          qb_n = qs[(b + 1) * QLDS_ROWS + 2 * jp + 1];                                                                    \
        }                                                                                                                 \
        __builtin_amdgcn_sched_barrier(0);                                                                                \
        SP_BATCH_MAC16(qa, qb, b)                                                                                         \
      }                                                                                                                   \
    } else {                                                                                                              \
      _Pragma("unroll") for (int b = 0; b < B; b++) {                                                                     \
        const uint4* __restrict__ qrow = reinterpret_cast<const uint4*>(d.qv[b]) + qoff;                                  \
        const uint4 qa = qrow[2 * jp];                                                                                    \
        const uint4 qb = qrow[2 * jp + 1];                                                                                \
        SP_BATCH_MAC16(qa, qb, b)                                                                                         \
      }                                                                                                                   \
    }                                                                                                                     \
    __builtin_amdgcn_sched_barrier(0);                                                                                    \
  }
#define SP_BATCH_FOLD                                                                                     \
  _Pragma("unroll") for (int b = 0; b < B; b++) {                                                         \
    acc[b][0] = reduce64(acc[b][0], m0); acc[b][1] = reduce64(acc[b][1], m0);                             \
    acc[b][2] = reduce64(acc[b][2], m1); acc[b][3] = reduce64(acc[b][3], m1);                             \
    acc[b][4] = reduce64(acc[b][4], m0); acc[b][5] = reduce64(acc[b][5], m0);                             \
    acc[b][6] = reduce64(acc[b][6], m1); acc[b][7] = reduce64(acc[b][7], m1);                             \
  }
  if (U > 1 || (npairs & 1) == 0) {
    SP_BATCH_LOAD(va, vb, 0)
    int jp0 = 0;
    for (; jp0 + 2 * U < npairs; jp0 += 2 * U) {
      SP_BATCH_LOAD(na, nb, jp0 + U)
      __builtin_amdgcn_sched_barrier(0);
      SP_BATCH_MAC(va, vb, jp0)
      SP_BATCH_LOAD(va, vb, jp0 + 2 * U)
      __builtin_amdgcn_sched_barrier(0);
      SP_BATCH_MAC(na, nb, jp0 + U)
      if (((jp0 + 2 * U) & 127) == 0) SP_BATCH_FOLD
    }
    SP_BATCH_LOAD(na, nb, jp0 + U)
    __builtin_amdgcn_sched_barrier(0);
    SP_BATCH_MAC(va, vb, jp0)
    SP_BATCH_MAC(na, nb, jp0 + U)
    SP_BATCH_FOLD
  } else {
    for (int jp0 = 0; jp0 < npairs; jp0++) {
      SP_BATCH_LOAD(va, vb, jp0)
      SP_BATCH_MAC(va, vb, jp0)
      if (((jp0 + 1) & 127) == 0 || jp0 + 1 >= npairs) SP_BATCH_FOLD
    }
  }
#undef SP_BATCH_LOAD
#undef SP_BATCH_MAC
#undef SP_BATCH_MAC16
#undef SP_BATCH_FOLD
  const size_t rc = (size_t)N * d.num_per;
  const size_t zi = (size_t)plane * 4 * rc + (size_t)z * d.num_per + (size_t)chunk * 128 + 2 * lane;
#pragma unroll
  for (int b = 0; b < B; b++) {
    u32* o = d.out[b] + zi;
    *reinterpret_cast<uint2*>(o + 0 * rc) = make_uint2((u32)acc[b][0], (u32)acc[b][4]);
    *reinterpret_cast<uint2*>(o + 1 * rc) = make_uint2((u32)acc[b][2], (u32)acc[b][6]);
    *reinterpret_cast<uint2*>(o + 2 * rc) = make_uint2((u32)acc[b][1], (u32)acc[b][5]);
    *reinterpret_cast<uint2*>(o + 3 * rc) = make_uint2((u32)acc[b][3], (u32)acc[b][7]);
  }
}
static bool mfma_shape_ok(int num_per, int nj) {
  return tunable("batch_mfma", 1) != 0 && nj > 0 && (nj % 32) == 0 && nj <= 512 && num_per >= 128 && (num_per % 128) == 0;
}
bool sweep_batch_wants_mfma(const SweepBatchDesc& d) {
  if (d.narrow) return false;
  return mfma_shape_ok(d.num_per, d.nj) && d.batch >= (int)tunable("batch_mfma_min", 4) && d.batch <= SWEEP_GROUP_MAX &&
         (d.batch <= SWEEP_BATCH_MAX || tunable("batch_mfma_tiles", 2) >= 2);
}
int sweep_batch_group_max(int num_per, int nj) {
  if (!mfma_shape_ok(num_per, nj) || tunable("batch_mfma_tiles", 2) < 2 || tunable("batch_mfma_min", 4) > SWEEP_BATCH_MAX + 1)
// ... 239 lines not shown
```

sdk_amd/kernel_signature.py:

```python
import hashlib
import struct

_MAGIC = b"__CLANG_OFFLOAD_BUNDLE__"


def _code_objects(blob):
    pos = 0
    while True:
        i = blob.find(_MAGIC, pos)
        if i < 0:
            return
        n, = struct.unpack_from("<Q", blob, i + len(_MAGIC))
        p = i + len(_MAGIC) + 8
        for _ in range(n):
            off, size, tl = struct.unpack_from("<QQQ", blob, p)
            triple = blob[p + 24:p + 24 + tl].decode("ascii", "replace")
            p += 24 + tl
            if "amdgcn" in triple and size:
                yield triple, blob[i + off:i + off + size]
        pos = i + len(_MAGIC)


def _elf_functions(elf):
    if elf[:4] != b"\x7fELF" or elf[4] != 2 or elf[5] != 1:
        return {}
    shoff, = struct.unpack_from("<Q", elf, 0x28)
    shentsize, shnum, _ = struct.unpack_from("<HHH", elf, 0x3A)
    secs = [struct.unpack_from("<IIQQQQIIQQ", elf, shoff + k * shentsize) for k in range(shnum)]
    out = {}
    for (_, typ, _, _, off, size, link, _, _, entsize) in secs:
        if typ != 2 or not entsize:
            continue
        stroff = secs[link][4]
        for k in range(size // entsize):
            name_i, info, _, shndx, value, sz = struct.unpack_from("<IBBHQQ", elf, off + k * entsize)
            if (info & 0xF) != 2 or not sz or shndx == 0 or shndx >= shnum:
                continue
            end = elf.index(b"\0", stroff + name_i)
            name = elf[stroff + name_i:end].decode("ascii", "replace")
            _, _, _, saddr, soff, _, _, _, _, _ = secs[shndx]
            start = soff + (value - saddr)
            out[name] = elf[start:start + sz]
    return out


def kernel_signature(so_path, name_fragment):
    blob = open(so_path, "rb").read()
    found = {}
    for triple, elf in _code_objects(blob):
        if "gfx950" not in triple:
            continue
        for name, body in _elf_functions(elf).items():
            if name_fragment in name:
                found[name] = hashlib.sha256(body).hexdigest()[:32]
    if len(found) != 1:
        raise LookupError("%d gfx950 kernels match %r in %s: %s" % (len(found), name_fragment, so_path, sorted(found)))
    (name, sig), = found.items()
    return sig, name


def compiler_version():
    import subprocess
    try:
        out = subprocess.run(["/opt/rocm/bin/hipcc", "--version"], capture_output=True, text=True, timeout=60).stdout
        return " | ".join(line.strip() for line in out.splitlines()[:2])
    except Exception:
        return ""


SWEEP_C2 = "k_sweep_packed_ringILi8E"


if __name__ == "__main__":
    import os
    import sys
    so = sys.argv[1] if len(sys.argv) > 1 else os.path.join(os.path.dirname(os.path.abspath(__file__)), "libspiral_hip.so")
    print(*kernel_signature(so, sys.argv[2] if len(sys.argv) > 2 else SWEEP_C2))
```

Before: 93.83 queries/s.

## Write tiled sweep output via LDS-staged z-runs and read it tiled in from_sweep4

The persistent packed ring sweep now gives each wave a run of R=8 consecutive z rows per 128-column chunk. It stages the per-row results in LDS and writes them out as contiguous 16-byte tiles instead of strided pair stores. k_from_sweep4 gains a tiled read path that matches this layout, and an untile kernel restores the reference layout when the partial buffer is exposed. This is meant to make sweep-output writes and fold-input reads coalesced. The cost is 64 KiB of dynamic LDS per workgroup, a changed unit schedule, and an extra untile pass for consumers that need the old layout.

```diff
diff --git a/include/spiral_hip.h b/include/spiral_hip.h
--- a/include/spiral_hip.h
+++ b/include/spiral_hip.h
@@ -166,6 +166,9 @@
 int sp_debug_resident_check(const sp_params_t* params, const sp_pp_t* pp, uint64_t* out, int cap);
 int sp_debug_chacha20_u64(const uint8_t seed[32], uint64_t* out, size_t count);
 int sp_debug_chacha20_u64_device(const sp_params_t*, const uint8_t seed[32], size_t first_word, uint64_t* out, size_t count);
+int sp_debug_sweep_tiled_map(int num_per, int R, uint32_t* map, size_t cap_words);
+int sp_debug_plane_sweep(sp_query_t* q, const sp_db_t* db, int plane, int tiled, uint32_t* out, size_t cap_words);
+int sp_debug_from_sweep4(const sp_params_t*, const uint32_t* plane_words, int num_per, int tiled, uint64_t* cts);
 
 int sp_bench_ntt(const sp_params_t*, int M, int blocks, int reps, float* ns_per_ntt);
 
diff --git a/rust/src/hip.rs b/rust/src/hip.rs
--- a/rust/src/hip.rs
+++ b/rust/src/hip.rs
@@ -183,6 +183,11 @@
         pub fn sp_debug_chacha20_u64(seed: *const u8, out: *mut u64, count: usize) -> c_int;
         pub fn sp_debug_chacha20_u64_device(p: *const sp_params_t, seed: *const u8, first_word: usize, out: *mut u64,
                                             count: usize) -> c_int;
+        pub fn sp_debug_sweep_tiled_map(num_per: c_int, r: c_int, map: *mut u32, cap_words: usize) -> c_int;
+        pub fn sp_debug_plane_sweep(q: *mut sp_query_t, db: *const sp_db_t, plane: c_int, tiled: c_int, out: *mut u32,
+                                    cap_words: usize) -> c_int;
+        pub fn sp_debug_from_sweep4(p: *const sp_params_t, plane_words: *const u32, num_per: c_int, tiled: c_int,
+                                    cts: *mut u64) -> c_int;
         pub fn sp_bench_ntt(p: *const sp_params_t, m: c_int, blocks: c_int, reps: c_int, ns_per_ntt: *mut f32) -> c_int;
         pub fn sp_ntt_forward(p: *const sp_params_t, data: *mut u64, count: usize) -> c_int;
         pub fn sp_ntt_inverse(p: *const sp_params_t, data: *mut u64, count: usize) -> c_int;
diff --git a/sdk_amd/csrc/capi.cpp b/sdk_amd/csrc/capi.cpp
--- a/sdk_amd/csrc/capi.cpp
+++ b/sdk_amd/csrc/capi.cpp
@@ -1435,7 +1435,7 @@
 
 void* sp_query_partial_ptr(sp_query_t* q) {
   if (!q || !q->ws) return nullptr;
-  if (guarded([&] { q->ws->ensure_sweep(); }) != SP_OK) return nullptr;
+  if (guarded([&] { q->ws->ensure_sweep(); sweep_out_untile(*q->ws); }) != SP_OK) return nullptr;
   return (void*)q->ws->sweep_out.p;
 }
 size_t sp_query_partial_words(const sp_query_t* q) {
diff --git a/sdk_amd/csrc/capi_internal.hpp b/sdk_amd/csrc/capi_internal.hpp
--- a/sdk_amd/csrc/capi_internal.hpp
+++ b/sdk_amd/csrc/capi_internal.hpp
@@ -26,6 +26,7 @@
         (void)hipStreamSynchronize(ws->stream2);
       }
       ws->pipelined = false;
+      ws->sweep_tiled = 0;
       ws->have_sweep_span = false;
       ws->zero_shortcuts = false;
       ws->out_G = 1;
diff --git a/sdk_amd/csrc/capi_stage.cpp b/sdk_amd/csrc/capi_stage.cpp
--- a/sdk_amd/csrc/capi_stage.cpp
+++ b/sdk_amd/csrc/capi_stage.cpp
@@ -78,7 +78,9 @@
     auto sweep_once = [&] {
       if (!per_plane) return run_sweep(W, *db);
       W.ensure_sweep();
-      for (size_t pl = 0; pl < p.planes(); pl++) launch_plane_sweep(W, *db, pl);
+      const int tiled = sweep_is_pipelined(p, *db) ? plane_sweep_tiles(W, *db) : 0;
+      W.sweep_tiled = tiled;
+      for (size_t pl = 0; pl < p.planes(); pl++) launch_plane_sweep(W, *db, pl, tiled);
     };
     *ms_per_launch = timed_reps(W.stream, iters, sweep_once, per_plane ? (float)p.planes() : 1.0f);
   });
@@ -214,6 +216,49 @@
   }
   chacha20_keystream_u64(seed, out, count);
   return SP_OK;
+}
+
+int sp_debug_sweep_tiled_map(int num_per, int R, uint32_t* map, size_t cap_words) {
+  return guarded([&] {
+    need(map && sweep_tiled_shape_ok(num_per, R), "bad argument");
+    need(cap_words >= (size_t)4 * N * num_per, "map buffer smaller than 4 * 2048 * num_per words");
+    for (int rc = 0; rc < 4; rc++)
+      for (int z = 0; z < N; z++)
+        for (int ii = 0; ii < num_per; ii++) map[((size_t)rc * N + z) * num_per + ii] = (uint32_t)sweep_tiled_index(num_per, R, rc, z, ii);
+  });
+}
+
+int sp_debug_plane_sweep(sp_query_t* q, const sp_db_t* db, int plane, int tiled, uint32_t* out, size_t cap_words) {
+  return guarded([&] {
+    need(q && db && out, "null argument");
+    refuse_planar_resident(db, "sp_debug_plane_sweep");
+    need(db->params == q->params, "db was created for different params");
+    need(q->state >= 1, "query not begun");
+    need(db->col_G == 1 && db->num_shards == 1, "sp_debug_plane_sweep: an unsharded db");
+    const Params& p = q->params->p;
+    need(plane >= 0 && (size_t)plane < p.planes(), "plane out of range");
+    const size_t words = (size_t)4 * POLY_LEN * db->np_local;
+    need(cap_words >= words, "output buffer smaller than one plane");
+    check_device(db->device);
+    Workspace& W = *q->ws;
+    W.ensure_sweep();
+    launch_plane_sweep(W, *db, (size_t)plane, tiled);
+    HIP_CHECK(hipMemcpyAsync(out, W.sweep_out.p + (size_t)plane * words, words * sizeof(u32), hipMemcpyDeviceToHost, W.stream));
+    HIP_CHECK(hipStreamSynchronize(W.stream));
+  });
+}
+
+int sp_debug_from_sweep4(const sp_params_t* h, const uint32_t* plane_words, int num_per, int tiled, uint64_t* cts) {
+  return guarded([&] {
+    need(h && plane_words && cts && num_per >= 4 && num_per % 4 == 0 && num_per <= 65536, "bad argument");
+    Scoped W(h);
+    const size_t words = (size_t)4 * POLY_LEN * num_per;
+    DevBuf<u32> src(words);
+    DevBuf<u64> dst((size_t)num_per * 2 * POLY_LEN);
+    HIP_CHECK(hipMemcpyAsync(src.p, plane_words, words * sizeof(u32), hipMemcpyHostToDevice, W->stream));
+    launch_from_sweep4(W->D->T, src.p, num_per, 1, 0, dst.p, W->stream, tiled);
+    download_raw(*W, dst.p, (size_t)num_per * 2 * POLY_LEN, cts);
+  });
 }
 
 int sp_debug_resident_check(const sp_params_t* h, const sp_pp_t* pp, uint64_t* out, int cap) {
diff --git a/sdk_amd/csrc/db.hip b/sdk_amd/csrc/db.hip
--- a/sdk_amd/csrc/db.hip
+++ b/sdk_amd/csrc/db.hip
@@ -360,6 +360,18 @@
   launched(0, "k_sweep_out_to_ref");
 }
 
+__global__ __launch_bounds__(256) void k_sweep_out_untile(u32* out, const u32* in, int num_per, int R) {
+  const size_t i = (size_t)blockIdx.x * 256 + threadIdx.x;
+  if (i >= (size_t)4 * N * num_per) return;
+  const int ii = (int)(i % num_per), z = (int)((i / num_per) & (N - 1)), rc = (int)(i / num_per) >> POLY_LEN_LOG2;
+  out[i] = in[sweep_tiled_index(num_per, R, rc, z, ii)];
+}
+void launch_sweep_out_untile(u32* out, const u32* in, int num_per, int R, hipStream_t s) {
+  const size_t total = (size_t)4 * N * num_per;
+  hipLaunchKernelGGL(k_sweep_out_untile, dim3((unsigned)((total + 255) / 256)), dim3(256), 0, s, out, in, num_per, R);
+  launched(0, "k_sweep_out_untile");
+}
+
 }
 
 #include "item_readback.hpp"
diff --git a/sdk_amd/csrc/kernels.hpp b/sdk_amd/csrc/kernels.hpp
--- a/sdk_amd/csrc/kernels.hpp
+++ b/sdk_amd/csrc/kernels.hpp
@@ -109,7 +109,7 @@
   int add_inner2, add_outer_stride;
 };
 void launch_ntt_inv(const DevTables& T, const InvDesc& d, hipStream_t s);
-void launch_from_sweep4(const DevTables& T, const u32* src, int np, int n_planes, int premod, u64* dst, hipStream_t s);
+void launch_from_sweep4(const DevTables& T, const u32* src, int np, int n_planes, int premod, u64* dst, hipStream_t s, int tiled = 0);
 
 struct MacDesc {
   const u32* A;
@@ -268,7 +268,18 @@
   int packed;
   int out_G;
   int nt_store;
-};
+  int out_tiled;
+};
+constexpr int SWEEP_TILE_R = 8;
+__host__ __device__ inline size_t sweep_tiled_index(int num_per, int R, int rc, int z, int ii) {
+  const int gpc = num_per >= 128 ? 32 : num_per / 4;
+  const int chunks = num_per / (4 * gpc);
+  const int zrun = z / R, zr = z % R, chunk = ii / (4 * gpc), g = (ii / 4) % gpc, c = ii % 4;
+  return ((((size_t)(zrun * chunks + chunk) * 4 + rc) * gpc + g) * R + zr) * 4 + c;
+}
+inline bool sweep_tiled_shape_ok(int num_per, int R) {
+  return (R == 4 || R == 8) && num_per >= 4 && num_per % 4 == 0 && (num_per < 128 || num_per % 128 == 0);
+}
 struct ColMap {
   int off = 0, stride = 1, np_global = 0;
 };
@@ -278,6 +289,7 @@
 }
 void launch_sweep(const DevTables& T, const SweepDesc& d, hipStream_t s);
 void launch_sweep_persist(const DevTables& T, const SweepDesc& d, int wgs_per_cu, hipStream_t s, int n_cus = 256);
+int sweep_ring_rows(int npairs);
 constexpr int SWEEP_BATCH_MAX = 8;
 constexpr int SWEEP_GROUP_MAX = 16;
 struct SweepBatchDesc {
@@ -428,6 +440,7 @@
                                        hipStream_t s);
 
 void launch_sweep_out_to_ref(u64* out, const u32* in, int num_per, hipStream_t s);
+void launch_sweep_out_untile(u32* out, const u32* in, int num_per, int R, hipStream_t s);
 
 __host__ __device__ inline u64 synth_word(u64 seed, u64 idx) {
   u64 z = seed + 0x9E3779B97F4A7C15ULL * (idx + 1);
diff --git a/sdk_amd/csrc/ntt.hip b/sdk_amd/csrc/ntt.hip
--- a/sdk_amd/csrc/ntt.hip
+++ b/sdk_amd/csrc/ntt.hip
@@ -1,5 +1,6 @@
 #include "device_common.hpp"
 #include "bodies.hpp"
+#include "server.hpp"
 
 namespace spiral {
 
@@ -256,7 +257,7 @@
   launched(d.sweep_np > 0 ? PATH_FROM_SWEEP1 : 0, "k_ntt_inv");
 }
 
-__global__ __launch_bounds__(256, 2) void k_from_sweep4(DevTables T, const u32* src, int np, int premod, u64* dst, int xcd_map) {
+__global__ __launch_bounds__(256, 2) void k_from_sweep4(DevTables T, const u32* src, int np, int premod, u64* dst, int xcd_map, int tiled) {
   __shared__ u32 lds0[4 * LDS_WORDS];
   __shared__ u32 lds1[4 * LDS_WORDS];
   const int tau = threadIdx.x;
@@ -273,11 +274,23 @@
   const size_t base = ((size_t)plane * 4 + r * 2) * N * np + ii0;
   u32 res0[4][8];
   uint4 xin[2][8];
-#pragma unroll
-  for (int c = 0; c < 2; c++)
-#pragma unroll
-    for (int k = 0; k < 8; k++)
-      xin[c][k] = *reinterpret_cast<const uint4*>(src + base + (size_t)c * N * np + (size_t)(8 * tau + k) * np);
+  if (tiled) {
+    const u32* pl = src + (size_t)plane * 4 * N * np;
+#pragma unroll
+    for (int c = 0; c < 2; c++)
+#pragma unroll
+      for (int h = 0; h < 2; h++) {
+        const uint4* e = reinterpret_cast<const uint4*>(pl + sweep_tiled_index(np, tiled, r * 2 + c, 8 * tau + 4 * h, ii0));
+#pragma unroll
+        for (int k = 0; k < 4; k++) xin[c][4 * h + k] = e[k];
+      }
+  } else {
+#pragma unroll
+    for (int c = 0; c < 2; c++)
+#pragma unroll
+      for (int k = 0; k < 8; k++)
+        xin[c][k] = *reinterpret_cast<const uint4*>(src + base + (size_t)c * N * np + (size_t)(8 * tau + k) * np);
+  }
 #pragma unroll
   for (int c = 0; c < 2; c++) {
     const ModConst m = T.c.mod[c];
@@ -318,11 +331,12 @@
     }
   }
 }
-void launch_from_sweep4(const DevTables& T, const u32* src, int np, int n_planes, int premod, u64* dst, hipStream_t s) {
+void launch_from_sweep4(const DevTables& T, const u32* src, int np, int n_planes, int premod, u64* dst, hipStream_t s, int tiled) {
   if (n_planes <= 0) return;
+  if (tiled && !sweep_tiled_shape_ok(np, tiled)) throw ArgError("launch_from_sweep4: no tiled layout for this column count");
   const unsigned groups = (unsigned)((np / 4) * 2 * n_planes);
   const int xcd_map = tunable("from_sweep_xcd", 1) != 0 && (np % 32) == 0 && (groups % 64) == 0;
-  hipLaunchKernelGGL(k_from_sweep4, dim3(groups), dim3(256), 0, s, T, src, np, premod, dst, xcd_map);
+  hipLaunchKernelGGL(k_from_sweep4, dim3(groups), dim3(256), 0, s, T, src, np, premod, dst, xcd_map, tiled);
   launched(PATH_FROM_SWEEP4 | (xcd_map ? PATH_SWEEP_XCD_FROM : 0), "k_from_sweep4");
 }
 
diff --git a/sdk_amd/csrc/pipeline.hpp b/sdk_amd/csrc/pipeline.hpp
--- a/sdk_amd/csrc/pipeline.hpp
+++ b/sdk_amd/csrc/pipeline.hpp
@@ -34,6 +34,7 @@
   DevBuf<u64> gsw_raw;
   DevBuf<u32> gsw_dig;
   DevBuf<u32> sweep_out;
+  int sweep_tiled = 0;
   DevBuf<u64> fold_tail;
   DevBuf<u32> batch_rq;
   DevBuf<u64> foldX, foldY, final_cts, pack_raw;
@@ -84,7 +85,9 @@
 void run_sweep(Workspace& W, const sp_db& db);
 void run_sweep_pipelined(Workspace& W, const sp_db& db);
 bool sweep_is_pipelined(const Params& p, const sp_db& db);
-void launch_plane_sweep(Workspace& W, const sp_db& db, size_t plane);
+void launch_plane_sweep(Workspace& W, const sp_db& db, size_t plane, int tiled = 0);
+int plane_sweep_tiles(const Workspace& W, const sp_db& db);
+void sweep_out_untile(Workspace& W);
 bool fused_fold_supported(const Params& p);
 struct FoldOpts {
   long fused_min_pairs;
diff --git a/sdk_amd/csrc/server.cpp b/sdk_amd/csrc/server.cpp
--- a/sdk_amd/csrc/server.cpp
+++ b/sdk_amd/csrc/server.cpp
@@ -1144,6 +1144,7 @@
   if (db.planar_resident) throw ArgError("the single-query sweep kernels do not read a planar-resident database (sp_db_create_planar)");
   const Params& p = *W.P;
   W.ensure_sweep();
+  W.sweep_tiled = 0;
   SweepDesc d{db.words.p, W.qv.p, W.sweep_out.p, (int)p.planes(), db.np_local, (int)p.dim0(), db.j0, db.nj, db.packed, W.out_G};
   d.nt_store = (int)tunable("sweep_nt_store", 1);
   launch_sweep(W.D->T, d, W.stream);
@@ -1193,14 +1194,15 @@
   return FoldOpts{std::min(W.fused_min_pairs, tunable("fused_min_pairs_cap", 1L << 62)), true, below_q};
 }
 
-static void fold_planes(Workspace& W, size_t pg0, int np, bool premod) {
+static void fold_planes(Workspace& W, size_t pg0, int np, bool premod, int tiled = 0) {
   const Params& p = *W.P;
   DeviceState& D = *W.D;
   hipStream_t s = W.stream;
   if (p.num_per() % 4 == 0 && !tunable("from_sweep1", 0)) {
     launch_from_sweep4(D.T, W.sweep_out.p + pg0 * 4 * POLY_LEN * p.num_per(), (int)p.num_per(), np, premod ? 1 : 0,
-                       W.foldX.p, s);
+                       W.foldX.p, s, tiled);
   } else {
+    if (tiled) throw ArgError("fold_planes: only k_from_sweep4 reads the tiled sweep output");
     InvDesc inv{};
     inv.src = W.sweep_out.p + pg0 * 4 * POLY_LEN * p.num_per();
     inv.sweep_np = (int)p.num_per();
@@ -1220,9 +1222,9 @@
   while (cur > (size_t)stop && cur / 2 >= 1 && (cur & 1) == 0) { cur >>= 1; lv++; }
   return cur == (size_t)stop && lv > 0 && stop >= 2 ? lv : 0;
 }
-static void fold_plane_head(Workspace& W, size_t pl, int levels) {
-  const Params& p = *W.P;
-  launch_from_sweep4(W.D->T, W.sweep_out.p + pl * 4 * POLY_LEN * p.num_per(), (int)p.num_per(), 1, 0, W.foldX.p, W.stream);
+static void fold_plane_head(Workspace& W, size_t pl, int levels, int tiled) {
+  const Params& p = *W.P;
+  launch_from_sweep4(W.D->T, W.sweep_out.p + pl * 4 * POLY_LEN * p.num_per(), (int)p.num_per(), 1, 0, W.foldX.p, W.stream, tiled);
   u64* res = run_fold(W, query_fold_opts(W, true), W.foldX.p, W.foldY.p, 1, (int)p.num_per(), -1, 0, levels);
   const size_t cts = p.num_per() >> levels;
   HIP_CHECK(hipMemcpyAsync(W.fold_tail.p + pl * cts * 2 * POLY_LEN, res, cts * 2 * POLY_LEN * sizeof(u64), hipMemcpyDeviceToDevice, W.stream));
@@ -1240,7 +1242,15 @@
   return enabled && db.packed && db.num_shards == 1 && db.col_G == 1 && p.planes() > 1 && p.num_per() >= 1024;
 }
 
-void launch_plane_sweep(Workspace& W, const sp_db& db, size_t pl) {
+int plane_sweep_tiles(const Workspace& W, const sp_db& db) {
+  if (tunable("sweep_out_tiled", 1) == 0) return 0;
+  const int R = SWEEP_TILE_R;
+  const bool ring = db.packed && tunable("pipe_wgs", 4) > 0 && sweep_ring_rows(db.nj >> 1) >= 2;
+  const bool from4 = db.np_local % 4 == 0 && !tunable("from_sweep1", 0);
+  return ring && from4 && W.out_G <= 1 && db.np_local >= 128 && sweep_tiled_shape_ok(db.np_local, R) ? R : 0;
+}
+
+void launch_plane_sweep(Workspace& W, const sp_db& db, size_t pl, int tiled) {
   if (db.planar_resident) throw ArgError("the single-query sweep kernels do not read a planar-resident database (sp_db_create_planar)");
   const Params& p = *W.P;
   const size_t np_ = (size_t)db.np_local;
@@ -1248,11 +1258,27 @@
   SweepDesc d{db.words.p + pl * plane_db_words, W.qv.p, W.sweep_out.p + pl * 4 * POLY_LEN * np_, 1, db.np_local,
               (int)p.dim0(), db.j0, db.nj, db.packed, W.out_G};
   d.nt_store = (int)tunable("sweep_nt_store", 1);
+  d.out_tiled = tiled;
   const int wgs = (int)tunable("pipe_wgs", 4);
+  if (tiled && !(db.packed && wgs > 0)) throw ArgError("launch_plane_sweep: only the persistent PACKED sweep writes the tiled output");
   if (db.packed && wgs > 0)
     launch_sweep_persist(W.D->T, d, wgs, W.stream);
   else
     launch_sweep(W.D->T, d, W.stream);
+}
+
+void sweep_out_untile(Workspace& W) {
+  if (!W.sweep_tiled) return;
+  const Params& p = *W.P;
+  const size_t words = (size_t)4 * POLY_LEN * p.num_per();
+  DevBuf<u32> plane(words);
+  if (W.pipelined) HIP_CHECK(hipStreamWaitEvent(W.stream, W.ev_fold, 0));
+  for (size_t pl = 0; pl < p.planes(); pl++) {
+    launch_sweep_out_untile(plane.p, W.sweep_out.p + pl * words, (int)p.num_per(), W.sweep_tiled, W.stream);
+    HIP_CHECK(hipMemcpyAsync(W.sweep_out.p + pl * words, plane.p, words * sizeof(u32), hipMemcpyDeviceToDevice, W.stream));
+  }
+  HIP_CHECK(hipStreamSynchronize(W.stream));
+  W.sweep_tiled = 0;
 }
 
 void run_sweep_pipelined(Workspace& W, const sp_db& db) {
@@ -1266,18 +1292,20 @@
     W.fold_tail.ensure(2 * planes * (p.num_per() >> defer_levels) * 2 * POLY_LEN);
     note_path(PATH_FOLD_TAIL_BATCHED);
   }
+  const int tiled = plane_sweep_tiles(W, db);
+  W.sweep_tiled = tiled;
   for (size_t pl = 0; pl < planes; pl++) {
-    launch_plane_sweep(W, db, pl);
+    launch_plane_sweep(W, db, pl, tiled);
     HIP_CHECK(hipEventRecord(W.ev_plane[pl], W.stream));
     HIP_CHECK(hipStreamWaitEvent(W.stream2, W.ev_plane[pl], 0));
     if (defer_levels > 0) {
       on_stream(W, W.stream2, [&] {
-        fold_plane_head(W, pl, defer_levels);
+        fold_plane_head(W, pl, defer_levels, tiled);
         if (pl + 1 == planes) fold_tails(W, defer_levels);
       });
       continue;
     }
-    on_stream(W, W.stream2, [&] { fold_planes(W, pl, 1, false); });
+    on_stream(W, W.stream2, [&] { fold_planes(W, pl, 1, false, tiled); });
   }
   HIP_CHECK(hipEventRecord(W.ev_sw[1], W.stream));
   HIP_CHECK(hipEventRecord(W.ev_fold, W.stream2));
diff --git a/sdk_amd/csrc/sweep.hip b/sdk_amd/csrc/sweep.hip
--- a/sdk_amd/csrc/sweep.hip
+++ b/sdk_amd/csrc/sweep.hip
@@ -152,8 +152,9 @@
   }
 }
 typedef __attribute__((address_space(4))) const u32x4_t sweep_const_uint4;
-template <int U>
-__global__ __launch_bounds__(256) void k_sweep_packed_ring(DevTables T, SweepDesc d, int units, int hi_prio) {
+template <int U, int ZR>
+__device__ __forceinline__ void sweep_packed_ring(const DevTables& T, const SweepDesc& d, int units, int hi_prio) {
+  extern __shared__ __attribute__((aligned(16))) unsigned char smem_q[];
   if (hi_prio) __builtin_amdgcn_s_setprio(3);
   const int lane = threadIdx.x & 63;
   const int wave0 = __builtin_amdgcn_readfirstlane(blockIdx.x * 4 + (threadIdx.x >> 6));
@@ -166,8 +167,8 @@
   if (wave0 >= units) return;
   u32x4_t va[U], na[U];
   u32x3_t vb[U], nb[U];
-#define SPR_BASE(UNIT) \
-  (reinterpret_cast<const u32*>(d.db) + packed_unit_offset((size_t)((UNIT) / chunks), 0, (UNIT) % chunks, npairs, chunks))
+#define SPR_BASE2(ZP, CHUNK) (reinterpret_cast<const u32*>(d.db) + packed_unit_offset((size_t)(ZP), 0, (CHUNK), npairs, chunks))
+#define SPR_BASE(UNIT) SPR_BASE2((UNIT) / chunks * (ZR > 0 ? ZR : 1), (UNIT) % chunks)
 #define SPR_LOAD(VA, VB, BASE, JP0)                                                                       \
   _Pragma("unroll") for (int uu = 0; uu < U; uu++) {                                                      \
     const u32* u = (BASE) + (size_t)((JP0) + uu) * ustride;                                               \
@@ -198,9 +199,10 @@
   a10 = reduce64(a10, m0); a11 = reduce64(a11, m0); a12 = reduce64(a12, m1); a13 = reduce64(a13, m1);
   const u32* base = SPR_BASE(wave0);
   SPR_LOAD(va, vb, base, 0)
+  int zr = 0;
   for (int unit = wave0; unit < units;) {
     const int chunk = unit % chunks;
-    const int zp = unit / chunks;
+    const int zp = ZR > 0 ? unit / chunks * ZR + zr : unit / chunks;
     const int z = zp & (N - 1);
     const int plane = zp >> POLY_LEN_LOG2;
     const sweep_const_uint4* qrow =
@@ -223,8 +225,13 @@
       __builtin_amdgcn_sched_barrier(0);
       SPR_MAC(va, vb, j)
       const bool more = jb + 128 < npairs;
-      next_unit = unit + nwaves;
-      next_base = next_unit < units ? SPR_BASE(next_unit) : base;
+      if (ZR > 0 && zr + 1 < ZR) {
+        next_unit = unit;
+        next_base = SPR_BASE2(zp + 1, chunk);
+      } else {
+        next_unit = unit + nwaves;
+        next_base = next_unit < units ? SPR_BASE(next_unit) : base;
+      }
       const u32* nb_base = more ? base : next_base;
       const int nb_jp = more ? jb + 128 : 0;
       SPR_LOAD(va, vb, nb_base, nb_jp)
@@ -232,22 +239,72 @@
       SPR_MAC(na, nb, j + U)
       SPR_FOLD
     }
-    sweep_store_pair(d, plane, z, chunk * 128 + 2 * lane, (u32)a00, (u32)a10, (u32)a02, (u32)a12, (u32)a01, (u32)a11,
-                     (u32)a03, (u32)a13);
+    if (ZR > 0) {
+      constexpr int R = ZR > 0 ? ZR : 1;
+      u32* region = reinterpret_cast<u32*>(smem_q) + (threadIdx.x >> 6) * (512 * R);
+      u32* w = region + ((lane >> 1) * R + zr) * 4 + (lane & 1) * 2;
+      *reinterpret_cast<mf_u32x2_t*>(w + 0 * 32 * R * 4) = mf_u32x2_t{(u32)a00, (u32)a10};
+      *reinterpret_cast<mf_u32x2_t*>(w + 1 * 32 * R * 4) = mf_u32x2_t{(u32)a02, (u32)a12};
+      *reinterpret_cast<mf_u32x2_t*>(w + 2 * 32 * R * 4) = mf_u32x2_t{(u32)a01, (u32)a11};
+      *reinterpret_cast<mf_u32x2_t*>(w + 3 * 32 * R * 4) = mf_u32x2_t{(u32)a03, (u32)a13};
+      if (++zr == R) {
+        zr = 0;
+        __builtin_amdgcn_wave_barrier();
+        u32* o = d.out + (size_t)plane * 4 * N * d.num_per + ((size_t)(z / R) * chunks + chunk) * (512 * R) + lane * 4;
+        const u32* rd = region + lane * 4;
+#pragma unroll
+        for (int i = 0; i < 2 * R; i++) {
+          const u32x4_t v = *reinterpret_cast<const u32x4_t*>(rd + i * 256);
+          if (d.nt_store) __builtin_nontemporal_store(v, reinterpret_cast<u32x4_t*>(o + i * 256));
+          else *reinterpret_cast<u32x4_t*>(o + i * 256) = v;
+        }
+        __builtin_amdgcn_wave_barrier();
+      }
+    } else {
+      sweep_store_pair(d, plane, z, chunk * 128 + 2 * lane, (u32)a00, (u32)a10, (u32)a02, (u32)a12, (u32)a01, (u32)a11,
+                       (u32)a03, (u32)a13);
+    }
     base = next_base;
     unit = next_unit;
   }
+#undef SPR_BASE2
 #undef SPR_BASE
 #undef SPR_LOAD
 #undef SPR_MAC
 #undef SPR_FOLD
 }
+template <int U>
+__global__ __launch_bounds__(256) void k_sweep_packed_ring(DevTables T, SweepDesc d, int units, int hi_prio) {
+  sweep_packed_ring<U, 0>(T, d, units, hi_prio);
+}
+template <int U, int R>
+__global__ __launch_bounds__(256) void k_sweep_packed_ring_zrun(DevTables T, SweepDesc d, int units, int hi_prio) {
+  sweep_packed_ring<U, R>(T, d, units, hi_prio);
+}
+int sweep_ring_rows(int npairs) {
+  long ring = tunable("pipe_ring", 8);
+  while (ring > 1 && (npairs % (2 * ring) != 0 || (ring != 2 && ring != 4 && ring != 8))) ring >>= 1;
+  return ring >= 2 ? (int)ring : 0;
+}
 void launch_sweep_persist(const DevTables& T, const SweepDesc& d, int wgs_per_cu, hipStream_t s, int n_cus) {
   const int units = d.planes * N * (d.num_per >> 7);
   const int prio = (int)tunable("sweep_prio", 1);
-  const int npairs = d.nj >> 1;
-  long ring = tunable("pipe_ring", 8);
-  while (ring > 1 && (npairs % (2 * ring) != 0 || (ring != 2 && ring != 4 && ring != 8))) ring >>= 1;
+  const int ring = sweep_ring_rows(d.nj >> 1);
+  if (d.out_tiled && !(ring >= 2 && d.out_G <= 1 && d.out_tiled == SWEEP_TILE_R && d.num_per >= 128 && sweep_tiled_shape_ok(d.num_per, SWEEP_TILE_R)))
+    throw ArgError("launch_sweep_persist: the tiled output needs the ring form, one output chunk, whole 128-column chunks and R = 8");
+  if (d.out_tiled) {
+    constexpr int R = SWEEP_TILE_R;
+    const int runs = d.planes * (N / R) * (d.num_per >> 7);
+    const dim3 rgrid((unsigned)std::min(n_cus, (runs + 3) / 4));
+    const size_t lds = (size_t)4 * 512 * R * sizeof(u32);
+    switch (ring) {
+      case 2: hipLaunchKernelGGL((k_sweep_packed_ring_zrun<2, R>), rgrid, dim3(256), lds, s, T, d, runs, prio); break;
+      case 8: hipLaunchKernelGGL((k_sweep_packed_ring_zrun<8, R>), rgrid, dim3(256), lds, s, T, d, runs, prio); break;
+      default: hipLaunchKernelGGL((k_sweep_packed_ring_zrun<4, R>), rgrid, dim3(256), lds, s, T, d, runs, prio); break;
+    }
+    launched(PATH_SWEEP_PERSIST | PATH_SWEEP_RING, "k_sweep_packed_ring_zrun");
+    return;
+  }
   if (ring >= 2) {
     const int ring_wgs = (int)std::max(1L, tunable("pipe_ring_wgs", 1));
     const dim3 rgrid((unsigned)std::min(n_cus * ring_wgs, (units + 3) / 4));
diff --git a/sdk_amd/kernel_signature.py b/sdk_amd/kernel_signature.py
--- a/sdk_amd/kernel_signature.py
+++ b/sdk_amd/kernel_signature.py
@@ -68,7 +68,7 @@
         return ""
 
 
-SWEEP_C2 = "k_sweep_packed_ringILi8E"
+SWEEP_C2 = "k_sweep_packed_ring_zrunILi8ELi8E"
 
 
 if __name__ == "__main__":
```

New measurement: 95.79 queries/s, median of 6. 2.1% higher.
